# zju3dv/RelightableAvatar

Hardware: AMD Instinct MI355X
Metric: rays_per_sec (higher is better)
Workload: dtype f16

## Files before the change

### include/relightableavatar.h

```cpp
#ifndef RELIGHTABLEAVATAR_H
#define RELIGHTABLEAVATAR_H

#include <stddef.h>
#include <stdint.h>

#ifdef __cplusplus
extern "C" {
#endif

#define RA_ABI_VERSION 9
#define RA_N_LIGHTS_MAX 512

typedef struct ra_ctx ra_ctx;

const char* ra_last_error(void);
int ra_abi_version(void);

int ra_ctx_create(ra_ctx** out, int device);
int ra_ctx_destroy(ra_ctx* ctx);

typedef struct ra_config {
    int   xyz_res, sdf_res, view_res;
    int   n_bones;
    int   relight;
    float resd_limit;
    float blend_radius;
    float albedo_slope, albedo_bias;
    float roughness_slope, roughness_bias;
    float fresnel_f0;
    float shading_albedo;
    float albedo_multiplier;
    int   lambert_only, glossy_only;
    int   tonemapping;
    float bg_brightness;
    int   mlp_f16;
    int   query_skip;
    int   k4_batch_slots;
    int   trace_precision;
    float clip_near, clip_far;
    int   only_visibility;
    int   vis_shade_map;
    int   use_geodesic_filter;
    float key_light_share;
} ra_config;
int ra_default_config(ra_config* out);
int ra_set_config(ra_ctx* ctx, const ra_config* cfg);

int ra_set_weight(ra_ctx* ctx, const char* name, const float* host_data, size_t numel);
int ra_finalize_weights(ra_ctx* ctx, void* stream);
int ra_k3cc_enabled(const ra_ctx* ctx);

typedef struct ra_frame {
    const float* R;
    const float* Th;
    const float* poses;
    const float* cond_fix;
    const float* A;
    const float* big_A;
    const float* pverts;
    const float* pnorm;
    const float* tverts;
    const float* weights;
    int n_verts;
} ra_frame;
int ra_set_frame(ra_ctx* ctx, const ra_frame* frame, void* stream);

int ra_hdq_sdf(ra_ctx* ctx, const float* x_dev, int n, float dist_th, int smooth_transition,
               float* sdf_dev, void* stream);

int ra_observed_sdf(ra_ctx* ctx, const float* bpts_dev, int n, float* sdf_dev, void* stream);

int ra_bigpose_transform(ra_ctx* ctx, const float* x_dev, int n, const float* R_dev, const float* Th_dev, int invert,
                         float* out_dev, void* stream);

int ra_raw_channels(const ra_ctx* ctx);
int ra_forward(ra_ctx* ctx, const float* x_dev, const float* v_dev, int n, float dist_th,
               float* raw_dev, void* stream);

typedef struct ra_trace_params {
    int   iters;
    float tan_i;
    float tan_i_multiplier;
    float relax, offset, eps;
    int   shadow_skip_iter;
    int   clay_book;
    int   soft_shadow;
    float dist_th;
} ra_trace_params;
int ra_sphere_trace(ra_ctx* ctx, const float* ray_o, const float* ray_d, const float* near_,
                    const float* far_, const float* tan_i_dev, int n, const ra_trace_params* p,
                    float* surf, float* occ, float* st, float* ot, void* stream);

typedef struct ra_render_out {
    float* rgb;
    float* acc;
    float* depth;
    float* surf;
    float* norm;
    float* albedo;
    float* roughness;
    float* shade;
    float* spec;
    float* cpts;
    float* bpts;
    float* resd;
    float* ray_o;
    float* lvis;
    float* ldot;
    float* raw;
    float* volume_albedo;
    float* volume_roughness;
} ra_render_out;

typedef struct ra_sphere_params {
    ra_trace_params surface;
    ra_trace_params shadow;
    float shadow_near_offset;
    float dist_th;
    float surf_sample_range;
    int   n_samples;
    int   relighting;
    int   no_visibility, local_visibility;
    int   premultiply;
    int   n_boxes;
    const float* boxes;
    const int*   box_start;
} ra_sphere_params;

int ra_render_sphere_chunk(ra_ctx* ctx, const float* ray_o, const float* ray_d, const float* near_,
                           const float* far_, int P, const float* bbox_host6,
                           const float* probe_dev, int probe_h, int probe_w,
                           const ra_sphere_params* p, const ra_render_out* out, void* stream);

int ra_gather_rays(int device, const long long* idx_dev, int n, const float* ray_o, const float* ray_d, const float* near_, const float* far_,
                   float* out_o, float* out_d, float* out_near, float* out_far, void* stream);

int ra_scatter_rows(int device, const float* src_dev, const long long* src_idx_dev, const long long* dst_idx_dev, long long n, int C,
                    float* dst_dev, void* stream);

int ra_begin_render(ra_ctx* ctx);

int ra_set_key_probes(ra_ctx* ctx, const float* probes_dev, int n, int probe_h, int probe_w, int accumulate, void* stream);

int ra_set_light_xyz(ra_ctx* ctx, const float* xyz_dev, void* stream);

int ra_light_visibility(ra_ctx* ctx, const float* surf, const float* norm, const float* acc, int n, const int* rows_dev, int n_rows,
                        const float* bbox_host6, const float* probe_dev, int probe_h, int probe_w, const ra_sphere_params* params,
                        float* lvis, float* ldot, void* stream);

int ra_render_volume_chunk(ra_ctx* ctx, const float* ray_o, const float* ray_d, const float* near_,
                           const float* far_, int P, int n_samples, float dist_th,
                           const ra_render_out* out, void* stream);

int ra_reshade(ra_ctx* ctx, const float* ray_o, const float* surf, const float* norm,
               const float* albedo, const float* roughness, const float* lvis, const float* ldot,
               int P, const float* probes_dev, int n_probes, int probe_h, int probe_w,
               float* rgb, float* shade, float* spec, void* stream);

int ra_reshade_backward(ra_ctx* ctx, const float* ray_o, const float* surf, const float* norm,
                        const float* albedo, const float* roughness, const float* lvis, const float* ldot, int P,
                        const float* probes_dev, int n_probes, int probe_h, int probe_w,
                        const float* d_rgb, float* d_albedo, float* d_roughness, float* d_probes, void* stream);

size_t ra_heads_param_count(const ra_ctx* ctx);
int ra_heads_get_params(ra_ctx* ctx, float* theta_dev, void* stream);
int ra_heads_forward(ra_ctx* ctx, const float* theta_dev, const float* feat_dev, int n, float* albedo_dev, float* rough_dev, void* stream);
int ra_heads_backward(ra_ctx* ctx, const float* theta_dev, const float* feat_dev, int n,
                      const float* d_albedo_dev, const float* d_rough_dev, float* d_theta_dev, void* stream);
int ra_bigpose_features(ra_ctx* ctx, const float* bpts_dev, int n, float* feat_dev, void* stream);

int ra_canonical_features(ra_ctx* ctx, const float* cpts_dev, int n, float* feat_dev, void* stream);
int ra_gaussian_entropy(ra_ctx* ctx, const float* x_dev, int n, const float* d_value_dev, float* value_dev, float* d_x_dev, void* stream);

int ra_reshade_ground(ra_ctx* ctx, const float* ray_d, const float* albedo_map, const float* lvis, const float* ldot, int P,
                      const float* probes_dev, int n_probes, int probe_h, int probe_w, const float* images_dev, int image_h, int image_w,
                      int attach_envmap, float* rgb, float* albedo, float* shade, float* spec, void* stream);

typedef struct ra_counters {
    uint64_t n_coarse;
    uint64_t n_fine_sdf;
    uint64_t n_fine_full;
    uint64_t n_shadow_rays;
    uint64_t n_hit_pixels;
    uint64_t n_shaded;
    uint64_t n_fine_sdf_wide;
    uint64_t n_fine_sdf_comp;
} ra_counters;
int ra_get_counters(ra_ctx* ctx, ra_counters* out, void* stream);
int ra_reset_counters(ra_ctx* ctx, void* stream);

int ra_get_mlp_time(ra_ctx* ctx, float* ms, int* n_launches, void* stream);
int ra_get_kernel_time(ra_ctx* ctx, int kind, float* ms, int* n_launches, void* stream);
int ra_enable_timing(ra_ctx* ctx, int on);
typedef struct ra_gate ra_gate;
int ra_gate_create(ra_gate** out, int device);
int ra_gate_destroy(ra_gate* gate);
// ... 196 lines not shown
```

### relightableavatar_amd/_lib.py

```python
import ctypes as C
import os
import subprocess

_HERE = os.path.dirname(os.path.abspath(__file__))
LIB_PATH = os.environ.get('RA_LIB_PATH') or os.path.join(_HERE, 'librelightableavatar_hip.so')
_lib = None
ABI_VERSION = 9
RA_MESH_BRUTE, RA_MESH_UNSORTED = 1, 2
RA_WINDING_ONE_PASS, RA_WINDING_SPLIT = 1, 2
RA_RAYCAST_BRUTE, RA_RAYCAST_UNSORTED = 1, 2
RA_TOPO_ARRAYS = ('vert', 'twin', 'edge', 'edges', 'edge_counts', 'edge_he_start', 'edge_he', 'nbr_start', 'nbr', 'out_start', 'out_he')
RA_CLOTH_STRETCH, RA_CLOTH_BENDING, RA_CLOTH_GRAVITY = 1, 2, 4
CLOTH_MATERIAL_DEFAULTS = (('density', 426 * 0.00047), ('thickness', 0.00047), ('young_modulus', 0.7e5), ('poisson_ratio', 0.485),
                           ('bending_multiplier', 50.0), ('stretch_multiplier', 1.0), ('material_multiplier', 1.0))
RA_VOLUME_MODES = {'canonical': 0, 'tpose': 1, 'posed': 2}


class RaError(RuntimeError):
    pass


class ra_config(C.Structure):
    _fields_ = [('xyz_res', C.c_int), ('sdf_res', C.c_int), ('view_res', C.c_int), ('n_bones', C.c_int), ('relight', C.c_int),
                ('resd_limit', C.c_float), ('blend_radius', C.c_float), ('albedo_slope', C.c_float), ('albedo_bias', C.c_float),
                ('roughness_slope', C.c_float), ('roughness_bias', C.c_float), ('fresnel_f0', C.c_float),
                ('shading_albedo', C.c_float), ('albedo_multiplier', C.c_float), ('lambert_only', C.c_int),
                ('glossy_only', C.c_int), ('tonemapping', C.c_int), ('bg_brightness', C.c_float), ('mlp_f16', C.c_int), ('query_skip', C.c_int),
                ('k4_batch_slots', C.c_int), ('trace_precision', C.c_int), ('clip_near', C.c_float), ('clip_far', C.c_float),
                ('only_visibility', C.c_int), ('vis_shade_map', C.c_int), ('use_geodesic_filter', C.c_int), ('key_light_share', C.c_float)]


class ra_frame(C.Structure):
    _fields_ = [(k, C.c_void_p) for k in ('R', 'Th', 'poses', 'cond_fix', 'A', 'big_A', 'pverts', 'pnorm', 'tverts', 'weights')] + \
               [('n_verts', C.c_int)]


class ra_trace_params(C.Structure):
    _fields_ = [('iters', C.c_int), ('tan_i', C.c_float), ('tan_i_multiplier', C.c_float), ('relax', C.c_float),
                ('offset', C.c_float), ('eps', C.c_float), ('shadow_skip_iter', C.c_int), ('clay_book', C.c_int),
                ('soft_shadow', C.c_int), ('dist_th', C.c_float)]


RENDER_OUT_KEYS = ('rgb', 'acc', 'depth', 'surf', 'norm', 'albedo', 'roughness', 'shade', 'spec', 'cpts', 'bpts', 'resd',
                   'ray_o', 'lvis', 'ldot', 'raw', 'volume_albedo', 'volume_roughness')


class ra_render_out(C.Structure):
    _fields_ = [(k, C.c_void_p) for k in RENDER_OUT_KEYS]


class ra_sphere_params(C.Structure):
    _fields_ = [('surface', ra_trace_params), ('shadow', ra_trace_params), ('shadow_near_offset', C.c_float),
                ('dist_th', C.c_float), ('surf_sample_range', C.c_float), ('n_samples', C.c_int), ('relighting', C.c_int),
                ('no_visibility', C.c_int), ('local_visibility', C.c_int), ('premultiply', C.c_int),
                ('n_boxes', C.c_int), ('boxes', C.POINTER(C.c_float)), ('box_start', C.POINTER(C.c_int))]


class ra_ground_params(C.Structure):
    _fields_ = [('normal', C.c_float * 3), ('origin', C.c_float * 3), ('albedo', C.c_float * 3), ('attach_envmap', C.c_int),
                ('env_r', C.c_float), ('shading_multiplier', C.c_float), ('shadow', ra_trace_params), ('shadow_near_offset', C.c_float),
                ('no_visibility', C.c_int), ('local_visibility', C.c_int), ('n_boxes', C.c_int), ('boxes', C.POINTER(C.c_float)),
                ('box_start', C.POINTER(C.c_int))]


GROUND_OUT_KEYS = ('rgb', 'surf', 'albedo', 'shade', 'spec', 'depth', 'lvis', 'ldot')


class ra_ground_out(C.Structure):
    _fields_ = [(k, C.c_void_p) for k in GROUND_OUT_KEYS]


class ra_pose_in(C.Structure):
    _fields_ = [(k, C.POINTER(C.c_float)) for k in ('poses', 'tjoints', 'big_A', 'Rh', 'Th')] + \
               [('parents', C.POINTER(C.c_int)), ('faces', C.POINTER(C.c_int)), ('n_bones', C.c_int), ('n_faces', C.c_int), ('n_verts', C.c_int),
                ('tverts', C.c_void_p), ('weights', C.c_void_p), ('bounds_padding', C.c_float)]


POSE_OUT_KEYS = ('A', 'joints', 'tpose', 'pverts', 'wverts', 'pnorm', 'R', 'pbounds', 'wbounds', 'poses', 'Th')


class ra_pose_out(C.Structure):
    _fields_ = [(k, C.c_void_p) for k in POSE_OUT_KEYS]


class ra_image_params(C.Structure):
    _fields_ = [('type', C.c_int), ('H', C.c_int), ('W', C.c_int), ('bg_brightness', C.c_float), ('normalize', C.c_int), ('tonemap', C.c_int),
                ('min_clip', C.c_float), ('cam_R', C.c_float * 9), ('tbounds', C.c_float * 6)]


class ra_metrics_params(C.Structure):
    _fields_ = [('H', C.c_int), ('W', C.c_int), ('bg_brightness', C.c_float), ('data_range', C.c_float), ('mse_over_rays', C.c_int),
                ('crop_to_mask', C.c_int)]


class ra_lpips_weights(C.Structure):
    _fields_ = [('conv_w', C.c_void_p * 5), ('conv_b', C.c_void_p * 5), ('lin', C.c_void_p * 5), ('shift', C.c_float * 3), ('scale', C.c_float * 3)]


class ra_cloth_material(C.Structure):
    _fields_ = [(k, C.c_double) for k, _ in CLOTH_MATERIAL_DEFAULTS]


class ra_counters(C.Structure):
    _fields_ = [(k, C.c_uint64) for k in ('n_coarse', 'n_fine_sdf', 'n_fine_full', 'n_shadow_rays', 'n_hit_pixels', 'n_shaded', 'n_fine_sdf_wide', 'n_fine_sdf_comp')]


SYMBOLS = {
    'ra_last_error': (C.c_char_p, []),
    'ra_abi_version': (C.c_int, []),
    'ra_default_config': (C.c_int, [C.POINTER(ra_config)]),
    'ra_shard_plan': (C.c_int, [C.c_void_p, C.c_int, C.c_int, C.c_int, C.c_int, C.c_longlong] + [C.c_void_p] * 2 + [C.c_int] + [C.c_void_p] * 7),
    'ra_ctx_create': (C.c_int, [C.POINTER(C.c_void_p), C.c_int]),
    'ra_ctx_destroy': (C.c_int, [C.c_void_p]),
    'ra_set_config': (C.c_int, [C.c_void_p, C.POINTER(ra_config)]),
    'ra_set_weight': (C.c_int, [C.c_void_p, C.c_char_p, C.c_void_p, C.c_size_t]),
    'ra_finalize_weights': (C.c_int, [C.c_void_p, C.c_void_p]),
    'ra_set_frame': (C.c_int, [C.c_void_p, C.POINTER(ra_frame), C.c_void_p]),
    'ra_hdq_sdf': (C.c_int, [C.c_void_p, C.c_void_p, C.c_int, C.c_float, C.c_int, C.c_void_p, C.c_void_p]),
    'ra_observed_sdf': (C.c_int, [C.c_void_p, C.c_void_p, C.c_int, C.c_void_p, C.c_void_p]),
    'ra_bigpose_transform': (C.c_int, [C.c_void_p, C.c_void_p, C.c_int, C.c_void_p, C.c_void_p, C.c_int, C.c_void_p, C.c_void_p]),
    'ra_raw_channels': (C.c_int, [C.c_void_p]),
    'ra_forward': (C.c_int, [C.c_void_p, C.c_void_p, C.c_void_p, C.c_int, C.c_float, C.c_void_p, C.c_void_p]),
    'ra_sphere_trace': (C.c_int, [C.c_void_p] + [C.c_void_p] * 5 + [C.c_int, C.POINTER(ra_trace_params)] + [C.c_void_p] * 5),
    'ra_render_sphere_chunk': (C.c_int, [C.c_void_p] + [C.c_void_p] * 4 + [C.c_int, C.POINTER(C.c_float), C.c_void_p, C.c_int, C.c_int,
                                         C.POINTER(ra_sphere_params), C.POINTER(ra_render_out), C.c_void_p]),
    'ra_render_volume_chunk': (C.c_int, [C.c_void_p] + [C.c_void_p] * 4 + [C.c_int, C.c_int, C.c_float, C.POINTER(ra_render_out), C.c_void_p]),
    'ra_render_ground_chunk': (C.c_int, [C.c_void_p] + [C.c_void_p] * 3 + [C.c_int, C.POINTER(C.c_float), C.c_void_p, C.c_int, C.c_int,
                                         C.POINTER(ra_ground_params), C.POINTER(ra_ground_out), C.c_void_p]),
    'ra_blend_ground': (C.c_int, [C.c_void_p] + [C.c_void_p] * 4 + [C.c_int, C.c_int, C.c_int, C.c_void_p, C.c_void_p]),
    'ra_reshade': (C.c_int, [C.c_void_p] + [C.c_void_p] * 7 + [C.c_int, C.c_void_p, C.c_int, C.c_int, C.c_int] + [C.c_void_p] * 4),
    'ra_reshade_backward': (C.c_int, [C.c_void_p] + [C.c_void_p] * 7 + [C.c_int, C.c_void_p, C.c_int, C.c_int, C.c_int] + [C.c_void_p] * 5),
    'ra_heads_get_params': (C.c_int, [C.c_void_p, C.c_void_p, C.c_void_p]),
    'ra_heads_forward': (C.c_int, [C.c_void_p, C.c_void_p, C.c_void_p, C.c_int, C.c_void_p, C.c_void_p, C.c_void_p]),
    'ra_heads_backward': (C.c_int, [C.c_void_p, C.c_void_p, C.c_void_p, C.c_int, C.c_void_p, C.c_void_p, C.c_void_p, C.c_void_p]),
    'ra_bigpose_features': (C.c_int, [C.c_void_p, C.c_void_p, C.c_int, C.c_void_p, C.c_void_p]),
    'ra_canonical_features': (C.c_int, [C.c_void_p, C.c_void_p, C.c_int, C.c_void_p, C.c_void_p]),
    'ra_gaussian_entropy': (C.c_int, [C.c_void_p, C.c_void_p, C.c_int, C.c_void_p, C.c_void_p, C.c_void_p, C.c_void_p]),
    'ra_k3cc_enabled': (C.c_int, [C.c_void_p]),
    'ra_begin_render': (C.c_int, [C.c_void_p]),
    'ra_debug_key_lights': (C.c_int, [C.c_void_p, C.c_void_p, C.c_void_p, C.c_void_p]),
    'ra_scatter_rows': (C.c_int, [C.c_int, C.c_void_p, C.c_void_p, C.c_void_p, C.c_longlong, C.c_int, C.c_void_p, C.c_void_p]),
    'ra_gather_rays': (C.c_int, [C.c_int, C.c_void_p, C.c_int] + [C.c_void_p] * 9),
    'ra_set_key_probes': (C.c_int, [C.c_void_p, C.c_void_p, C.c_int, C.c_int, C.c_int, C.c_int, C.c_void_p]),
    'ra_set_light_xyz': (C.c_int, [C.c_void_p, C.c_void_p, C.c_void_p]),
    'ra_light_visibility': (C.c_int, [C.c_void_p, C.c_void_p, C.c_void_p, C.c_void_p, C.c_int, C.c_void_p, C.c_int, C.POINTER(C.c_float), C.c_void_p,
                                      C.c_int, C.c_int, C.POINTER(ra_sphere_params), C.c_void_p, C.c_void_p, C.c_void_p]),
    'ra_reshade_ground': (C.c_int, [C.c_void_p] + [C.c_void_p] * 4 + [C.c_int, C.c_void_p, C.c_int, C.c_int, C.c_int, C.c_void_p, C.c_int, C.c_int, C.c_int] +
                          [C.c_void_p] * 5),
    'ra_get_counters': (C.c_int, [C.c_void_p, C.POINTER(ra_counters), C.c_void_p]),
    'ra_reset_counters': (C.c_int, [C.c_void_p, C.c_void_p]),
    'ra_get_mlp_time': (C.c_int, [C.c_void_p, C.POINTER(C.c_float), C.POINTER(C.c_int), C.c_void_p]),
    'ra_get_kernel_time': (C.c_int, [C.c_void_p, C.c_int, C.POINTER(C.c_float), C.POINTER(C.c_int), C.c_void_p]),
    'ra_enable_timing': (C.c_int, [C.c_void_p, C.c_int]),
    'ra_set_knn_mode': (C.c_int, [C.c_void_p, C.c_int]),
    'ra_gate_create': (C.c_int, [C.POINTER(C.c_void_p), C.c_int]),
    'ra_gate_destroy': (C.c_int, [C.c_void_p]),
    'ra_set_gate': (C.c_int, [C.c_void_p, C.c_void_p]),
    'ra_pose_frame': (C.c_int, [C.c_void_p, C.POINTER(ra_pose_in), C.POINTER(ra_pose_out), C.c_void_p]),
    'ra_grow_bounds': (C.c_int, [C.c_void_p, C.c_void_p, C.c_float, C.c_void_p]),
    'ra_shift_envmap': (C.c_int, [C.c_void_p, C.c_void_p, C.c_int, C.c_int, C.c_int, C.c_float, C.c_void_p, C.c_void_p]),
    'ra_add_light_probe': (C.c_int, [C.c_void_p, C.c_void_p, C.c_int, C.c_int, C.c_void_p, C.c_int, C.c_int, C.POINTER(C.c_float), C.c_int, C.c_int, C.c_void_p]),
    'ra_map_to_image': (C.c_int, [C.c_void_p, C.POINTER(ra_image_params)] + [C.c_void_p] * 4 + [C.c_int, C.c_void_p, C.c_void_p, C.c_void_p]),
    'ra_image_metrics': (C.c_int, [C.c_void_p, C.POINTER(ra_metrics_params), C.c_void_p, C.c_void_p, C.c_void_p, C.c_int, C.c_void_p, C.c_void_p,
                                   C.c_void_p]),
    'ra_lpips_load': (C.c_int, [C.c_void_p, C.POINTER(ra_lpips_weights), C.c_void_p]),
    'ra_lpips_loaded': (C.c_int, [C.c_void_p]),
    'ra_lpips': (C.c_int, [C.c_void_p, C.POINTER(ra_metrics_params), C.c_void_p, C.c_void_p, C.c_void_p, C.c_int, C.c_void_p, C.c_void_p, C.c_void_p]),
    'ra_lpips_features': (C.c_int, [C.c_void_p, C.c_void_p, C.c_int, C.c_int, C.c_int, C.c_void_p, C.c_void_p]),
    'ra_lpips_tile_m': (C.c_int, []),
    'ra_mesh_create': (C.c_int, [C.c_void_p, C.c_void_p, C.c_int, C.c_void_p, C.c_int, C.POINTER(C.c_void_p), C.c_void_p]),
    'ra_mesh_destroy': (C.c_int, [C.c_void_p, C.c_void_p]),
    'ra_mesh_closest': (C.c_int, [C.c_void_p, C.c_void_p, C.c_void_p, C.c_int, C.c_int] + [C.c_void_p] * 5),
    'ra_mesh_tile': (C.c_int, [C.c_int]),
    'ra_mesh_winding': (C.c_int, [C.c_void_p, C.c_void_p, C.c_void_p, C.c_int, C.c_int, C.c_void_p, C.c_void_p]),
    'ra_winding_tile': (C.c_int, [C.c_int]),
    'ra_mesh_winding_grad': (C.c_int, [C.c_void_p, C.c_void_p, C.c_void_p, C.c_int, C.c_int, C.c_void_p, C.c_void_p, C.c_void_p]),
    'ra_mesh_raycast': (C.c_int, [C.c_void_p, C.c_void_p, C.c_void_p, C.c_void_p, C.c_int, C.c_int] + [C.c_void_p] * 5),
    'ra_raycast_tile': (C.c_int, [C.c_int]),
    'ra_topo_create': (C.c_int, [C.c_void_p, C.c_void_p, C.c_int, C.c_int, C.POINTER(C.c_void_p), C.c_void_p]),
    'ra_topo_destroy': (C.c_int, [C.c_void_p, C.c_void_p]),
    'ra_topo_sizes': (C.c_int, [C.c_void_p, C.c_void_p, C.POINTER(C.c_int)]),
    'ra_topo_array': (C.c_int, [C.c_void_p, C.c_void_p, C.c_int, C.c_void_p, C.c_void_p]),
# ... 80 lines not shown
```

### relightableavatar_amd/config.py

```python
from .base_utils import dotdict

_ACTIVE = None


def set_active_cfg(cfg):
    global _ACTIVE
    _ACTIVE = cfg


def active_cfg():
    global _ACTIVE
    if _ACTIVE is None:
        _ACTIVE = default_cfg()
    return _ACTIVE


UNSUPPORTED = {
    'bruteforce_st': (False, 'render_bruteforce_human (sphere_tracing_renderer.py:787-940) needs lib/networks/relight/nerfactor_network.py, '
                             'which the reference release does not contain'),
    'smpl_distance': (False, 'the SMPL mesh distance (base_network.py:417-427) needs the bvh_distance_queries CUDA extension'),
    'ablate_hdq_mode': ('hdq', "the world / can / curve tracing modes (sphere_tracing_renderer.py:141-151) call world_to_bigpose_transform, "
                               "which raises on the dataset's Th of shape (B, 1, 3); the operators exist: ra_observed_sdf, ra_bigpose_transform"),
    'check_bound_sdf': (False, 'debug colour map of |sdf| at termination (sphere_tracing_renderer.py:577-587, needs easyvolcap)'),
    'geometry_normal': (False, 'part of render_bruteforce_human'),
    'geometry_visibility': (False, 'part of render_bruteforce_human'),
    'zero_roughness': (False, 'part of render_bruteforce_human'),
    'mesh_simp_face': (-1, 'quadric decimation of the extracted mesh (mesh_renderer.py:95-96) needs open3d / trimesh'),
    'track_tpose_mesh': (False, 'mesh tracking (lib/networks/renderer/mesh_tracker.py) is not mirrored'),
}


def check_supported(cfg):
    for k, (default, why) in UNSUPPORTED.items():
        if k in cfg and cfg[k] != default:
            raise NotImplementedError(f'cfg.{k} = {cfg[k]!r} is not supported: {why}')


def default_cfg() -> dotdict:
    c = dotdict()
    c.network_module = 'relightableavatar_amd.networks.deform.base_network'
    c.renderer_module = 'relightableavatar_amd.renderer.base_renderer'
    c.n_bones = 52
    c.cond_dim = 156
    c.xyz_res = 10
    c.sdf_res = 8
    c.view_res = 4
    c.feat_dim = 256
    c.resd_limit = 0.05
    c.sdf_beta_init_value = 0.1
    c.blend_radius = 0.075
    c.sample_vert_cnt = 3
    c.use_geodesic_filter = True
    c.lambertian = False
    c.dist_th = 0.1
    c.n_samples = 128
    c.perturb = 1.0
    c.clip_near = 0.02
    c.clip_far = 10.0
    c.bg_brightness = 0.0
    c.render_chunk_size = 8192
    c.volume_chunk_rays = 65536
    c.sphere_chunk_rays = 262144
    c.ground_chunk_rays = 262144
    c.network_chunk_size = 262144
    c.fix_material = 0
    c.always_fix_material = True
    c.sphere_tracing = dotdict(iter=16, tan_i=1000.0, relax=0.0, offset=0.02, eps=1e-8,
                               near_offset=0.01, shadow_skip_iter=1, tan_i_multiplier=1.0)
    c.obj_lvis = dotdict(iter=4, offset=0.01, relax=0.0, near_offset=0.02, dist_th=0.05)
    c.env_lvis = dotdict(iter=16, offset=0.01, relax=0.0, near_offset=0.02, bbox_margin=0.25, dist_th=0.005)
    c.no_claybook = False
    c.no_dfss = False
    c.no_visibility = False
    c.local_visibility = False
    c.surf_sample_range = 0.005
    c.relighting = False
    c.achro_light = False
    c.envmap_upscale = 2
    c.envmap_init_intensity = 0.2
    c.env_h = 16
    c.env_w = 32
    c.env_r = 10.0
    c.fresnel_f0 = 0.02
    c.lambert_only = False
    c.glossy_only = False
    c.albedo_slope = 1.0
    c.albedo_bias = 0.0
    c.roughness_slope = 0.90
    c.roughness_bias = 0.09
    c.relight_network_width = 128
    c.relight_network_depth = 2
    c.albedo_multiplier = 1.0
    c.shading_albedo = 0.8
    c.tonemapping_rendering = True
    c.only_visibility = False
    c.rgb_as_albedo = False
    c.img_loss_weight = 1.0
    c.albedo_sparsity = 5e-4
    c.albedo_smooth_weight = 5e-3
    c.roughness_smooth_weight = 5e-3
    c.xyz_noise_std = 0.02
    c.light_xyz_noise_std = 1.0
    c.vis_rendering_map = True
    c.vis_shading_map = False
    c.vis_specular_map = False
    c.vis_novel_light = False
    c.vis_ground_shading = False
    c.voxel_size = [0.005, 0.005, 0.005]
    c.mesh_th = 0.5
    c.mesh_th_to_sdf = False
    c.mesh_simp_face = -1
    c.surface_blend_weight = False
    c.vis_tpose_mesh = False
    c.vis_posed_mesh = False
    c.vis_can_mesh = False
    c.track_tpose_mesh = False
    c.ground_normal = [0.0, 0.0, 1.0]
    c.ground_origin = [0.0, 0.0, 0.0]
    c.ground_albedo = [0.05, 0.05, 0.05]
    c.ground_attach_envmap = True
    c.ground_shading_multiplier = 1.0
    c.vis_lvis_map = False
    c.vis_ldot_map = False
    c.replace_light = ''
    c.test_light = ['main']
    c.vis_rotate_light = False
    c.rotate_ratio = 4
    c.probe_size_ratio = 0.2
    c.env_image_w = 2048
    c.normalize_shading = False
    c.normalize_specular = True
    c.min_clip = 1.0
    c.vis_median_depth = False
    c.store_alpha_channel = True
    c.tonemapping_albedo = True
    c.mlp_dtype = 'f16'
    c.ret_raw = True
    c.novel_light_timing = True
    c.query_skip = True
    c.trace_precision = 1
    c.key_light_share = 0.0078
    c.k4_batch_slots = 0
    return c


def make_cfg(mode: str = 'anisdf', **overrides) -> dotdict:
    c = default_cfg()
    if mode in ('sphere_tracing', 'relight', 'novel_light'):
        c.n_samples = 3
        c.render_chunk_size = 65536
        c.network_chunk_size = 1048576
        c.renderer_module = 'relightableavatar_amd.renderer.sphere_tracing_renderer'
    if mode in ('relight', 'novel_light'):
        c.relighting = True
        c.dist_th = 0.125
        c.obj_lvis.dist_th = 0.125
        c.achro_light = True
        c.network_module = 'relightableavatar_amd.networks.relight.relight_network'
    if mode == 'novel_light':
        c.vis_novel_light = True
        c.renderer_module = 'relightableavatar_amd.renderer.novel_light_sphere_tracing'
    elif mode not in ('anisdf', 'sphere_tracing', 'relight'):
        raise ValueError(f'unknown mode {mode}')
    for k, v in overrides.items():
        if isinstance(v, dict) and isinstance(c.get(k), dict):
            c[k].update(v)
        else:
            c[k] = v
    return c
```

### relightableavatar_amd/csrc/ra_api.cpp

```cpp
#include "ra_api_impl.hpp"
#include <cmath>

int check_ready(ra_ctx* c, const char* who) {
    if (!c) { ra_set_error(std::string(who) + ": null ctx"); return 1; }
    if (!c->have_weights) { ra_set_error(std::string(who) + ": weights not finalized"); return 1; }
    if (!c->have_frame) { ra_set_error(std::string(who) + ": no frame set (ra_set_frame)"); return 1; }
    if (hipSetDevice(c->device) != hipSuccess) { ra_set_error(std::string(who) + ": hipSetDevice failed"); return 1; }
    return 0;
}

static void zero_chunk_counters(ra_ctx* c, hipStream_t s) {
    hipMemsetAsync(icnt(c, 0), 0, CNT_ALL * sizeof(int), s);
    c->fc_next = 0;
    c->fc_wrapped = false;
    c->cnt_zero = true;
}
int* next_fine_counter(ra_ctx* c, hipStream_t s) {
    if (c->fc_next >= CNT_FC_SLOTS) {
        hipMemsetAsync(icnt(c, CNT_FC0), 0, CNT_FC_SLOTS * sizeof(int), s);
        c->fc_next = 0;
        c->fc_wrapped = true;
    }
    return icnt(c, CNT_FC0 + c->fc_next++);
}

namespace {

struct Timer {
    ra_ctx* c; hipStream_t s; TimerKind kind; hipEvent_t a = nullptr, b = nullptr;
    Timer(ra_ctx* c_, hipStream_t s_, TimerKind kind_) : c(c_), s(s_), kind(kind_) {
        if (!c->timing) return;
        if (c->ev_used == c->ev_pool.size()) {
            hipEvent_t x, y;
            hipEventCreate(&x); hipEventCreate(&y);
            c->ev_pool.push_back({x, y});
            c->ev_kind.push_back(kind);
        }
        c->ev_kind[c->ev_used] = kind;
        a = c->ev_pool[c->ev_used].first; b = c->ev_pool[c->ev_used].second;
        c->ev_used++;
        hipEventRecord(a, s);
    }
    ~Timer() { if (a) hipEventRecord(b, s); }
};

struct HintScope {
    ra_ctx* c; hipStream_t s;
    HintScope(ra_ctx* c_, hipStream_t s_) : c(c_), s(s_) {
        const int k = c->call_no++;
        if (k >= 64) { c->cur_hint = nullptr; return; }
        if ((int)c->hints.size() <= k) c->hints.resize(k + 1);
        HintSlot& h = c->hints[k];
        if (!h.ev) {
            if (hipEventCreateWithFlags(&h.ev, hipEventDisableTiming) != hipSuccess || hipHostMalloc((void**)&h.host, CNT_FC_SLOTS * sizeof(int)) != hipSuccess) {
                h.ev = nullptr; h.host = nullptr; c->cur_hint = nullptr; (void)hipGetLastError(); return;
            }
        }
        if (h.pending && hipEventQuery(h.ev) == hipSuccess) {
            h.vals.assign(h.host, h.host + h.n_pending);
            h.n_valid = h.n_pending;
            h.pending = false;
        }
        (void)hipGetLastError();
        c->cur_hint = &h;
    }
    ~HintScope() {
        HintSlot* h = c->cur_hint;
        c->cur_hint = nullptr;
        if (!h || h->pending || c->fc_next <= 0 || c->fc_wrapped) return;
        if (hipMemcpyAsync(h->host, icnt(c, CNT_FC0), (size_t)c->fc_next * sizeof(int), hipMemcpyDeviceToHost, s) != hipSuccess) return;
        if (hipEventRecord(h->ev, s) != hipSuccess) return;
        h->n_pending = c->fc_next;
        h->pending = true;
    }
};

int fine_hint(const ra_ctx* c, int k) {
    const HintSlot* h = c->cur_hint;
    return (h && !c->fc_wrapped && k < h->n_valid) ? h->vals[k] : -1;
}
int variant_size(int n, int hint) {
    if (hint < 0) return n;
    const long long v = (long long)hint + hint / 4 + 1024;
    return v < n ? (int)v : n;
}
int grid_size(int n, int nv) { return nv > n / 8 ? nv : n / 8; }

void k3_launch(ra_ctx* c, const MlpIO& io, int n, hipStream_t s, int grid_slots = 0) {
    if (c->cfg.mlp_f16) launch_mlp_sdf_stream_f16(c->host.geo, c->sarena.p, c->sarena_pairs.p, c->barena.as<float>(), c->fr, io, n, s, grid_slots);
    else launch_mlp_sdf_stream_bf16(c->host.geo, c->sarena.p, c->sarena_pairs.p, c->barena.as<float>(), c->fr, io, n, s, grid_slots);
}

}

void k4_fwd_launch(ra_ctx* c, const FullIO& io, char* tape, hipStream_t s) {
    if (c->cfg.mlp_f16) launch_mlp_fwd_tape_f16(c->host.geo, c->fwd_arena.p, c->barena.as<float>(), c->fr, io, tape, s);
    else launch_mlp_fwd_tape_bf16(c->host.geo, c->fwd_arena.p, c->barena.as<float>(), c->fr, io, tape, s);
}

FullIO full_io(ra_ctx* c) {
    FullIO io{};
    io.C = raw_channels(c);
    io.beta = c->host.beta; io.resd_limit = c->cfg.resd_limit;
    io.albedo_slope = c->cfg.albedo_slope; io.albedo_bias = c->cfg.albedo_bias;
    io.rough_slope = c->cfg.roughness_slope; io.rough_bias = c->cfg.roughness_bias;
    io.relight = c->cfg.relight;
    io.counters = dcnt(c);
    return io;
}

enum { Q_OTHER = 0, Q_SURFACE = 1, Q_PRECISE = 2 };
static bool precise(const ra_ctx* c, int what) { return what == Q_PRECISE || c->cfg.trace_precision >= 2 || (c->cfg.trace_precision == 1 && what == Q_SURFACE); }
static constexpr int KEY_LIGHTS_MAX = 48;
static bool key_tier(const ra_ctx* c) { return c->cfg.trace_precision == 1 && c->cfg.key_light_share > 0.f && c->n_lights > 0; }
static int key_mask_from(ra_ctx* c, const float* probe, int ph, int pw, hipStream_t s) {
    if (c->key_external) return 0;
    c->key_valid = false;
    if (!key_tier(c) || !probe) return 0;
    if (c->key_mask.ensure((size_t)c->n_lights) || c->key_share.ensure((size_t)c->n_lights * sizeof(float))) return 1;
    launch_key_lights(probe, 1, ph, pw, c->light_dir.as<float>(), c->light_area.as<float>(), c->n_lights, c->cfg.key_light_share, KEY_LIGHTS_MAX, 0,
                      c->key_share.as<float>(), c->key_mask.as<unsigned char>(), s);
    c->key_valid = true;
    return 0;
}

static void fine_level(ra_ctx* c, const MlpIO& io, int n, bool comp, hipStream_t s, int hint = -1) {
    const int nv = variant_size(n, hint);
    if (comp) {
        Timer t(c, s, T_K3C);
        launch_mlp_sdf_comp(c->host.geo, c->sarena_c.p, c->barena.as<float>(), c->fr, io, nv, s, c->k3cc_ok, grid_size(n, nv));
    } else {
        Timer t(c, s, k3_waves(nv) == 8 ? T_K3_WIDE : T_K3_NARROW);
        k3_launch(c, io, nv, s, grid_size(n, nv));
    }
}

static int hdq_pass(ra_ctx* c, const RaySet& rs, int n, float th, int smooth, float* sdf, hipStream_t s, int what = Q_OTHER,
                    const unsigned char* key = nullptr, int n_key = 0) {
    if (n <= 0) return 0;
    int err = 0;
    int* fine_idx = c->buf<int>("fine_idx", n, &err);
    float* bpts = c->buf<float>("fine_bpts", (size_t)n * 3, &err);
    if (err) return 1;
    HdqOut out{};
    out.sdf = sdf; out.fine_count = next_fine_counter(c, s); out.fine_idx = fine_idx; out.bpts = bpts;
    const int hint = fine_hint(c, c->fc_next - 1);
    int hint2 = -1;
    if (key && n_key > 0) {
        out.key = key;
        out.fine_idx2 = c->buf<int>("fine_idx_k", n_key, &err);
        out.bpts2 = c->buf<float>("fine_bpts_k", (size_t)n_key * 3, &err);
        if (err) return 1;
        out.fine_count2 = next_fine_counter(c, s);
        hint2 = fine_hint(c, c->fc_next - 1);
    }
    out.counters = dcnt(c);
    launch_hdq_coarse(c->fr, rs, n, th, c->cfg.blend_radius, out, s, c->cfg.use_geodesic_filter != 0);
    MlpIO io{};
    io.bpts = bpts; io.idx = fine_idx; io.count = out.fine_count; io.sdf = sdf; io.dist_th = th; io.smooth = smooth;
    io.resd_limit = c->cfg.resd_limit; io.counters = dcnt(c);
    fine_level(c, io, n, precise(c, what), s, hint);
    if (out.key) {
        io.bpts = out.bpts2; io.idx = out.fine_idx2; io.count = out.fine_count2;
        fine_level(c, io, n_key, true, s, hint2);
    }
    return 0;
}

int full_query(ra_ctx* c, FullIO io, int n, hipStream_t s) {
    const bool gated = c->gate && n > 65536;
    if (gated && c->gate->armed) RA_HIP(hipStreamWaitEvent(s, c->gate->done, 0));
    struct Release {
        ra_ctx* c; hipStream_t s; bool on;
        ~Release() { if (on) { hipEventRecord(c->gate->done, s); c->gate->armed = true; } }
    } release{c, s, gated};
    Timer t(c, s, T_K4);
    const int batch = c->cfg.k4_batch_slots > 0 ? c->cfg.k4_batch_slots : (1 << 20);
    const int cap = n < batch ? n : batch;
    int err = 0;
    char* tape = c->buf<char>("k4_tape", mlp_full_rev_tape_bytes(cap), &err);
    if (err) {
        ra_set_error("full query: no device memory for the activation tape (" + std::to_string(mlp_full_rev_tape_bytes(cap) >> 20) +
                     " MB): lower cfg.k4_batch_slots / cfg.volume_chunk_rays");
        return 1;
    }
    for (int s0 = 0; s0 < n; s0 += cap) {
        io.slot0 = s0;
        io.slot_cap = n - s0 < cap ? n - s0 : cap;
        k4_fwd_launch(c, io, tape, s);
        if (c->cfg.mlp_f16) launch_mlp_bwd_heads_f16(c->host.mat, c->host.col, c->bwd_arena.p, c->barena.as<float>(), c->shead_row.as<float>(), c->fr, io, tape, s);
        else launch_mlp_bwd_heads_bf16(c->host.mat, c->host.col, c->bwd_arena.p, c->barena.as<float>(), c->shead_row.as<float>(), c->fr, io, tape, s);
    }
    return 0;
}

static int forward_pass(ra_ctx* c, const float* x, const float* v, int n, const int* n_dev, float th, float* raw, hipStream_t s) {
    if (n <= 0) return 0;
    int err = 0;
    const int C = raw_channels(c);
    int* fine_idx = c->buf<int>("fine_idx", n, &err);
    float* bpts = c->buf<float>("fine_bpts", (size_t)n * 3, &err);
    float* mats = c->buf<float>("fine_mats", (size_t)n * 24, &err);
    float* sdf = c->buf<float>("fwd_sdf", n, &err);
    if (err) return 1;
    RaySet rs{};
    rs.mode = 0; rs.x = x; rs.n_dev = n_dev;
    HdqOut out{};
    out.sdf = sdf; out.fine_count = next_fine_counter(c, s); out.fine_idx = fine_idx; out.bpts = bpts; out.mats = mats;
    out.raw_zero = raw; out.raw_C = C;
    out.counters = dcnt(c);
    launch_hdq_coarse(c->fr, rs, n, th, c->cfg.blend_radius, out, s, c->cfg.use_geodesic_filter != 0);
    FullIO io = full_io(c);
    io.bpts = bpts; io.mats = mats; io.view = v; io.idx = fine_idx; io.count = out.fine_count; io.raw = raw;
    return full_query(c, io, n, s);
}

static TraceState alloc_trace(ra_ctx* c, const std::string& p, int n, bool soft, int* err) {
    TraceState ts{};
    ts.t = c->buf<float>(p + "t", n, err);
    ts.d0 = c->buf<float>(p + "d0", n, err);
    ts.occ = c->buf<float>(p + "occ", n, err);
    ts.ot = c->buf<float>(p + "ot", n, err);
    ts.stuck = c->buf<unsigned char>(p + "stuck", n, err);
    if (!soft) {
        ts.dt = c->buf<float>(p + "dt", n, err);
        ts.st = c->buf<float>(p + "st", n, err);
        ts.cd = c->buf<float>(p + "cd", n, err);
        ts.off = c->buf<float>(p + "off", n, err);
        ts.rlx = c->buf<float>(p + "rlx", n, err);
    }
    return ts;
}

int sdf_points_precise(ra_ctx* c, int mode, const float* pts, int n, float dist_th, float* sdf, hipStream_t s) {
    if (n <= 0) return 0;
    if (mode == 2) {
        RaySet rs{};
        rs.mode = 0; rs.x = pts;
        return hdq_pass(c, rs, n, dist_th, 0, sdf, s, Q_PRECISE);
    }
    int err = 0;
    int* idx = c->buf<int>("fine_idx", n, &err);
    if (err) return 1;
    int* cnt = next_fine_counter(c, s);
    launch_iota(idx, n, cnt, s);
    MlpIO io{};
    io.bpts = pts; io.idx = idx; io.count = cnt; io.sdf = sdf; io.dist_th = 1.f; io.smooth = 0;
    io.resd_limit = mode == 0 ? 0.f : c->cfg.resd_limit; io.counters = dcnt(c);
    fine_level(c, io, n, true, s);
    return 0;
}

extern "C" {

int ra_raw_channels(const ra_ctx* c) { return c ? raw_channels(c) : 16; }

int ra_hdq_sdf(ra_ctx* c, const float* x, int n, float dist_th, int smooth, float* sdf, void* stream) {
    if (check_ready(c, "ra_hdq_sdf")) return 1;
    RA_CHECK(n >= 0 && (n == 0 || (x && sdf)), "ra_hdq_sdf: bad arguments");
    RaySet rs{};
    rs.mode = 0; rs.x = x;
    if (hdq_pass(c, rs, n, dist_th, smooth, sdf, (hipStream_t)stream)) return 1;
    RA_HIP(hipGetLastError());
    return 0;
}

int ra_observed_sdf(ra_ctx* c, const float* bpts, int n, float* sdf, void* stream) {
    if (check_ready(c, "ra_observed_sdf")) return 1;
    RA_CHECK(n >= 0 && (n == 0 || (bpts && sdf)), "ra_observed_sdf: bad arguments");
    if (n == 0) return 0;
    hipStream_t s = (hipStream_t)stream;
    int err = 0;
    int* idx = c->buf<int>("fine_idx", n, &err);
    if (err) return 1;
    int* cnt = next_fine_counter(c, s);
    launch_iota(idx, n, cnt, s);
    MlpIO io{};
    io.bpts = bpts; io.idx = idx; io.count = cnt; io.sdf = sdf; io.dist_th = 1.f; io.smooth = 0;
    io.resd_limit = c->cfg.resd_limit; io.counters = dcnt(c);
    fine_level(c, io, n, precise(c, Q_OTHER), s);
    RA_HIP(hipGetLastError());
    return 0;
}

int ra_bigpose_transform(ra_ctx* c, const float* x, int n, const float* R, const float* Th, int invert, float* out, void* stream) {
    if (check_ready(c, "ra_bigpose_transform")) return 1;
    RA_CHECK(n >= 0 && (n == 0 || (x && out && R && Th)), "ra_bigpose_transform: bad arguments");
    if (n == 0) return 0;
    hipStream_t s = (hipStream_t)stream;
    int err = 0;
    int* fine_idx = c->buf<int>("fine_idx", n, &err);
    float* fb = c->buf<float>("fine_bpts", (size_t)n * 3, &err);
    float* sdfc = c->buf<float>("bt_sdf", n, &err);
    float* sb = c->buf<float>("bt_sdf_batch", (size_t)n * 3, &err);
    int* nb = c->buf<int>("bt_nn", (size_t)n * 3, &err);
    float* d2 = c->buf<float>("bt_d2", (size_t)n * 3, &err);
    float* bp = c->buf<float>("bt_bpts", (size_t)n * 3, &err);
    float* tp = c->buf<float>("bt_tpts", (size_t)n * 3, &err);
    float* mats = c->buf<float>("bt_mats", (size_t)n * 24, &err);
    if (err) return 1;
    RaySet rs{};
    rs.mode = 0; rs.x = x;
    HdqOut o{};
    o.sdf = sdfc; o.fine_count = next_fine_counter(c, s); o.fine_idx = fine_idx; o.bpts = fb;
    o.dbg_sdf_batch = sb; o.dbg_nn_batch = nb; o.dbg_d2 = d2; o.dbg_bpts = bp; o.dbg_tpts = tp; o.dbg_mats = mats;
    o.counters = dcnt(c);
    launch_hdq_coarse(c->fr, rs, n, 1e9f, c->cfg.blend_radius, o, s, c->cfg.use_geodesic_filter != 0);
    launch_bigpose_compose(mats, d2, n, c->cfg.blend_radius, R, Th, invert, out, s);
    RA_HIP(hipGetLastError());
    return 0;
}

int ra_forward(ra_ctx* c, const float* x, const float* v, int n, float dist_th, float* raw, void* stream) {
    if (check_ready(c, "ra_forward")) return 1;
    RA_CHECK(n >= 0 && (n == 0 || (x && raw)), "ra_forward: bad arguments");
    RA_CHECK(c->cfg.relight || v || n == 0, "ra_forward: the AniSDF colour net needs view directions");
    if (forward_pass(c, x, v, n, nullptr, dist_th, raw, (hipStream_t)stream)) return 1;
    RA_HIP(hipGetLastError());
    return 0;
}

int ra_sphere_trace(ra_ctx* c, const float* ray_o, const float* ray_d, const float* near_, const float* far_, const float* tan_i,
                    int n, const ra_trace_params* p, float* surf, float* occ, float* st, float* ot, void* stream) {
    if (check_ready(c, "ra_sphere_trace")) return 1;
    RA_CHECK(p && n >= 0 && (n == 0 || (ray_o && ray_d && near_ && far_)), "ra_sphere_trace: bad arguments");
    if (n == 0) return 0;
    hipStream_t s = (hipStream_t)stream;
    int err = 0;
    TraceState ts = alloc_trace(c, "tr_", n, false, &err);
    float* sdf = c->buf<float>("tr_sdf", n, &err);
    if (err) return 1;
    ts.near_ = near_; ts.far_ = far_; ts.tan_i = tan_i; ts.light = nullptr;
    launch_trace_init(ts, n, nullptr, *p, s);
    RaySet rs{};
    rs.mode = 1; rs.o = ray_o; rs.d = ray_d; rs.t = ts.t;
    rs.nn_hint = c->buf<int>("tr_nn", (size_t)n * 3, &err);
    if (err) return 1;
    for (int it = 0; it < p->iters; ++it) {
        rs.hint_valid = it > 0;
        if (hdq_pass(c, rs, n, p->dist_th, 1, sdf, s, p->soft_shadow ? Q_OTHER : Q_SURFACE)) return 1;
        launch_trace_update(ts, sdf, n, nullptr, it, *p, s);
    }
    if (occ) RA_HIP(hipMemcpyAsync(occ, ts.occ, (size_t)n * 4, hipMemcpyDeviceToDevice, s));
    if (st) RA_HIP(hipMemcpyAsync(st, ts.st, (size_t)n * 4, hipMemcpyDeviceToDevice, s));
    if (ot) RA_HIP(hipMemcpyAsync(ot, ts.ot, (size_t)n * 4, hipMemcpyDeviceToDevice, s));
    if (surf) {
        float* depth = c->buf<float>("tr_depth", n, &err);
        float* acc = c->buf<float>("tr_acc", n, &err);
        int* hidx = c->buf<int>("tr_hidx", n, &err);
        if (err) return 1;
        launch_surface_finish(ray_o, ray_d, ts.st, ts.occ, n, surf, depth, acc, hidx, icnt(c, CNT_HIT), s);
    }
    RA_HIP(hipGetLastError());
    return 0;
}

struct LvisStage {
    const float *surf, *norm_slots, *acc, *bbox;
    const int *hit_idx, *hit_count;
    int P, no_visibility, local_visibility;
    float near_offset;
    const ra_trace_params* shadow;
    int n_boxes;
    const float* boxes;
    const int *box_start, *pix_nn, *perm;
    bool split_wide_groups;
    float *lvis, *ldot;
};
static int light_visibility_stage(ra_ctx* c, LvisStage& st, hipStream_t s) {
    const int P = st.P;
    const ra_trace_params& shadow = *st.shadow;
    int err = 0;
    const int L = c->n_lights;
    const size_t NR = (size_t)P * L;
    st.lvis = c->buf<float>("lv_lvis", NR, &err);
    st.ldot = c->buf<float>("lv_ldot", NR, &err);
    ShadowGen g{};
    g.surf = st.surf; g.norm = st.norm_slots; g.acc = st.acc; g.hit_idx = st.hit_idx; g.hit_count = st.hit_count; g.ldir = c->light_dir.as<float>();
    for (int k = 0; k < 6; ++k) g.bbox[k] = st.bbox[k];
    g.n_boxes = st.n_boxes > 1 ? st.n_boxes : 0;
    for (int j = 0; j < g.n_boxes; ++j) {
        for (int k = 0; k < 6; ++k) g.boxes[j][k] = st.boxes[6 * j + k];
        g.box_start[j] = st.box_start[j];
    }
    if (g.n_boxes) g.box_start[g.n_boxes] = st.box_start[g.n_boxes];
    g.perm = g.n_boxes ? st.perm : nullptr;
    g.near_offset = st.near_offset; g.L = L; g.no_visibility = st.no_visibility; g.local_visibility = st.local_visibility;
    g.split_wide_groups = st.split_wide_groups ? 1 : 0;
    g.lvis = st.lvis; g.ldot = st.ldot;
    g.ray_count = icnt(c, CNT_RAYS);
    const bool traced = !(st.no_visibility || st.local_visibility);
    TraceState sh{};
    float* ssdf = nullptr;
    if (traced) {
        g.ray_pix = c->buf<int>("lv_pix", NR, &err);
        g.ray_light = c->buf<int>("lv_light", NR, &err);
        g.ray_slot = c->buf<int>("lv_slot", NR, &err);
        g.near_ = c->buf<float>("lv_near", NR, &err);
        g.far_ = c->buf<float>("lv_far", NR, &err);
        sh = alloc_trace(c, "sh_", (int)NR, shadow.soft_shadow != 0, &err);
        ssdf = c->buf<float>("sh_sdf", NR, &err);
    }
    const bool keyed = traced && key_tier(c) && c->key_valid;
    const size_t NK = keyed ? (size_t)P * (size_t)(L < KEY_LIGHTS_MAX ? L : KEY_LIGHTS_MAX) : 0;
    if (err) return 1;
    if (c->gate && c->gate->armed) RA_HIP(hipStreamWaitEvent(s, c->gate->done, 0));
    launch_shadow_gen(g, P, s, c->cnt_zero);
    c->cnt_zero = false;
    if (traced) {
        sh.near_ = g.near_; sh.far_ = g.far_; sh.tan_i = c->light_sharp.as<float>(); sh.light = g.ray_light;
        launch_trace_init(sh, (int)NR, g.ray_count, shadow, s);
        RaySet r2{};
        r2.mode = 2; r2.o = st.surf; r2.t = sh.t; r2.pix = g.ray_pix; r2.light = g.ray_light; r2.ldir = c->light_dir.as<float>();
        r2.n_dev = g.ray_count;
        r2.skip = c->cfg.query_skip ? sh.stuck : nullptr;
        r2.nn_hint = c->buf<int>("lv_nn", NR * 3, &err);
        if (err) return 1;
        for (int it = 0; it < shadow.iters; ++it) {
            r2.hint_valid = it > 0;
            r2.hint_src = it == 0 ? st.pix_nn : nullptr;
            r2.hint_src_index = it == 0 ? g.ray_pix : nullptr;
            if (hdq_pass(c, r2, (int)NR, shadow.dist_th, 1, ssdf, s, Q_OTHER, keyed ? c->key_mask.as<unsigned char>() : nullptr, (int)NK)) return 1;
            launch_trace_update(sh, ssdf, (int)NR, g.ray_count, it, shadow, s);
        }
        launch_shadow_scatter(sh.occ, g.ray_slot, g.ray_count, (int)NR, st.lvis, s);
        launch_accumulate(g.ray_count, &dcnt(c)->n_shadow_rays, s);
    }
    if (c->gate) { RA_HIP(hipEventRecord(c->gate->done, s)); c->gate->armed = true; }
    return 0;
}

int ra_begin_render(ra_ctx* c) {
    RA_CHECK(c, "ra_begin_render: null ctx");
    c->call_no = 0;
    return 0;
}

int ra_set_key_probes(ra_ctx* c, const float* probes, int n, int ph, int pw, int accumulate, void* stream) {
    RA_CHECK(c && n >= 0 && (n == 0 || (probes && ph > 0 && pw > 0)), "ra_set_key_probes: bad arguments");
    if (n == 0) { c->key_external = false; c->key_valid = false; return 0; }
    RA_CHECK(c->have_weights && c->n_lights > 0, "ra_set_key_probes: needs the relight network's light set (ra_finalize_weights)");
    RA_HIP(hipSetDevice(c->device));
    const bool acc = accumulate && c->key_external && c->key_valid;
    c->key_external = true;
    if (!key_tier(c)) { c->key_valid = false; return 0; }
    if (c->key_mask.ensure((size_t)c->n_lights) || c->key_share.ensure((size_t)c->n_lights * sizeof(float))) return 1;
    launch_key_lights(probes, n, ph, pw, c->light_dir.as<float>(), c->light_area.as<float>(), c->n_lights, c->cfg.key_light_share, KEY_LIGHTS_MAX,
                      acc ? 1 : 0, c->key_share.as<float>(), c->key_mask.as<unsigned char>(), (hipStream_t)stream);
    c->key_valid = true;
    RA_HIP(hipGetLastError());
    return 0;
}

static int sort_hits(ra_ctx* c, const char* who, const float* surf, const float* acc, int P, const float* bbox, int* hit_idx, hipStream_t s) {
    int err = 0;
    const size_t tb = sort_hits_temp_bytes(P);
    unsigned* k0 = c->buf<unsigned>("hs_k0", P, &err);
    unsigned* k1 = c->buf<unsigned>("hs_k1", P, &err);
    int* v0 = c->buf<int>("hs_v0", P, &err);
    char* tmp = c->buf<char>("hs_tmp", tb + 16, &err);
    if (err) return 1;
    if (launch_sort_hits(surf, acc, P, bbox, k0, k1, v0, hit_idx, tmp, tb, s)) { ra_set_error(std::string(who) + ": radix sort failed"); return 1; }
    return 0;
}
static int sort_rays(ra_ctx* c, const char* who, const float** ray_o, const float** ray_d, const float** near_, const float** far_, int P,
                     const float* bbox, const int** perm, hipStream_t s) {
    int err = 0;
    const size_t tb = sort_hits_temp_bytes(P);
    unsigned* k0 = c->buf<unsigned>("hs_k0", P, &err);
    unsigned* k1 = c->buf<unsigned>("hs_k1", P, &err);
    int* v0 = c->buf<int>("hs_v0", P, &err);
    int* pm = c->buf<int>("rs_perm", P, &err);
    char* tmp = c->buf<char>("hs_tmp", tb + 16, &err);
    float* so = c->buf<float>("rs_o", (size_t)P * 3, &err);
    float* sd = c->buf<float>("rs_d", (size_t)P * 3, &err);
    float* sn = c->buf<float>("rs_n", P, &err);
    float* sf = c->buf<float>("rs_f", P, &err);
    if (err) return 1;
    const int rc = bbox ? launch_sort_rays(*ray_o, *ray_d, *near_, *far_, P, bbox, k0, k1, v0, pm, tmp, tb, so, sd, sn, sf, s)
                        : launch_sort_rays(*ray_o, *ray_d, *near_, *far_, P, nullptr, k0, k1, v0, pm, tmp, tb, so, sd, sn, sf, s, c->cfg.clip_near, c->cfg.clip_far);
    if (rc) { ra_set_error(std::string(who) + ": radix sort failed"); return 1; }
    *ray_o = so; *ray_d = sd; *near_ = sn; *far_ = sf; *perm = pm;
    return 0;
}

static int check_box_table(const std::string& w, int n_boxes, const float* boxes, const int* box_start, const float* bbox, int P) {
    if (n_boxes <= 1) return 0;
    RA_CHECK(n_boxes <= RA_MAX_BOXES && boxes && box_start && bbox, w + ": at most 32 boxes per call, with their tables");
    RA_CHECK(box_start[0] == 0 && box_start[n_boxes] == P, w + ": box_start must run from 0 to P");
    for (int j = 0; j < n_boxes; ++j) RA_CHECK(box_start[j] <= box_start[j + 1], w + ": box_start must ascend");
    return 0;
}

int ra_render_sphere_chunk(ra_ctx* c, const float* ray_o, const float* ray_d, const float* near_, const float* far_, int P,
                           const float* bbox, const float* probe, int ph, int pw, const ra_sphere_params* p,
                           const ra_render_out* out, void* stream) {
    if (check_ready(c, "ra_render_sphere_chunk")) return 1;
    RA_CHECK(p && out && P >= 0, "ra_render_sphere_chunk: bad arguments");
    if (P == 0) return 0;
    RA_CHECK(ray_o && ray_d && near_ && far_, "ra_render_sphere_chunk: null ray arrays");
    const bool relit = p->relighting != 0;
    RA_CHECK(!relit || (c->cfg.relight && probe && bbox && c->n_lights > 0), "ra_render_sphere_chunk: relighting needs the relight network, a probe and a bbox");
    RA_CHECK(p->n_samples >= 1 && p->n_samples <= 16, "ra_render_sphere_chunk: n_samples out of range");
    RA_CHECK(!relit || (long long)P * c->n_lights < (1ll << 31), "ra_render_sphere_chunk: chunk too large (rays x lights must fit an int): lower cfg.render_chunk_size / cfg.sphere_chunk_rays");
    if (check_box_table("ra_render_sphere_chunk", p->n_boxes, p->boxes, p->box_start, bbox, P)) return 1;
    hipStream_t s = (hipStream_t)stream;
    int err = 0;
    const int S = p->n_samples, C = raw_channels(c), L = c->n_lights;
    zero_chunk_counters(c, s);
    HintScope hints(c, s);
    const int* perm = nullptr;
    if (bbox && sort_rays(c, "ra_render_sphere_chunk", &ray_o, &ray_d, &near_, &far_, P, bbox, &perm, s)) return 1;
    TraceState ts = alloc_trace(c, "sf_", P, false, &err);
    float* sdf = c->buf<float>("sf_sdf", P, &err);
    float* surf = c->buf<float>("sf_surf", (size_t)P * 3, &err);
    float* depth = c->buf<float>("sf_depth", P, &err);
    float* acc = c->buf<float>("sf_acc", P, &err);
    int* hit_idx = c->buf<int>("sf_hit", P, &err);
    int* slot_of_ray = c->buf<int>("sf_slot", P, &err);
    if (err) return 1;
    ts.near_ = near_; ts.far_ = far_;
    launch_trace_init(ts, P, nullptr, p->surface, s);
    RaySet rs{};
    rs.mode = 1; rs.o = ray_o; rs.d = ray_d; rs.t = ts.t; rs.skip = c->cfg.query_skip ? ts.stuck : nullptr;
    rs.nn_hint = c->buf<int>("sf_nn", (size_t)P * 3, &err);
    if (err) return 1;
    for (int it = 0; it < p->surface.iters; ++it) {
        rs.hint_valid = it > 0;
        if (hdq_pass(c, rs, P, p->surface.dist_th, 1, sdf, s, Q_SURFACE)) return 1;
        launch_trace_update(ts, sdf, P, nullptr, it, p->surface, s);
    }
    int* hit_count = icnt(c, CNT_HIT);
    launch_surface_finish(ray_o, ray_d, ts.st, ts.occ, P, surf, depth, acc, hit_idx, hit_count, s, slot_of_ray, true);
    launch_accumulate(hit_count, &dcnt(c)->n_hit_pixels, s);
    if (relit && sort_hits(c, "ra_render_sphere_chunk", surf, acc, P, bbox, hit_idx, s)) return 1;
    launch_slot_index(hit_idx, hit_count, P, slot_of_ray, s);
    float* xs = c->buf<float>("mt_x", (size_t)P * S * 3, &err);
    float* vs = c->buf<float>("mt_v", (size_t)P * S * 3, &err);
    float* raw = c->buf<float>("mt_raw", (size_t)P * S * C, &err);
    SurfaceMaps m{};
    m.cpts = c->buf<float>("mp_cpts", (size_t)P * 3, &err);
    m.bpts = c->buf<float>("mp_bpts", (size_t)P * 3, &err);
    m.resd = c->buf<float>("mp_resd", (size_t)P * 3, &err);
    m.norm = c->buf<float>("mp_norm", (size_t)P * 3, &err);
    m.albedo = c->buf<float>("mp_albedo", (size_t)P * 3, &err);
    m.rough = c->buf<float>("mp_rough", P, &err);
    m.rgb = c->buf<float>("mp_rgb", (size_t)P * 3, &err);
    m.valbedo = (out->volume_albedo && c->cfg.relight) ? c->buf<float>("mp_valbedo", (size_t)P * 3, &err) : nullptr;
    if (err) return 1;
    launch_surface_samples(surf, ray_d, hit_idx, hit_count, P, S, p->surf_sample_range, xs, vs, icnt(c, CNT_SAMP), s);
    if (forward_pass(c, xs, vs, P * S, icnt(c, CNT_SAMP), p->dist_th, raw, s)) return 1;
    launch_surface_composite(raw, C, S, hit_count, P, c->cfg.relight, c->cfg, m, s);
    float *shade = nullptr, *spec = nullptr;
    LvisStage st{};
    if (relit) {
        if (key_mask_from(c, probe, ph, pw, s)) return 1;
        st.surf = surf; st.norm_slots = m.norm; st.acc = acc; st.hit_idx = hit_idx; st.hit_count = hit_count; st.P = P; st.bbox = bbox;
        st.near_offset = p->shadow_near_offset; st.shadow = &p->shadow; st.no_visibility = p->no_visibility; st.local_visibility = p->local_visibility;
        st.n_boxes = p->n_boxes; st.boxes = p->boxes; st.box_start = p->box_start; st.pix_nn = rs.nn_hint; st.perm = perm; st.split_wide_groups = true;
        if (light_visibility_stage(c, st, s)) return 1;
        m.rgb = c->buf<float>("mp_rgb", (size_t)P * 3, &err);
        shade = c->buf<float>("mp_shade", (size_t)P * 3, &err);
        spec = c->buf<float>("mp_spec", (size_t)P * 3, &err);
        if (err) return 1;
        ShadeIn in{};
        in.ray_o = ray_o; in.surf = surf; in.idx = hit_idx; in.count = hit_count; in.n = P;
        in.norm = m.norm; in.albedo = m.albedo; in.rough = m.rough; in.lvis = st.lvis; in.ldot = st.ldot;
        in.light_xyz = c->light_xyz.as<float>(); in.light_area = c->light_area.as<float>(); in.L = L;
        in.probes = probe; in.n_probes = 1; in.ph = ph; in.pw = pw; in.want_spec = out->spec != nullptr;
        in.rgb = m.rgb; in.shade = shade; in.spec = spec;
        launch_shade(in, c->cfg, s);
    }
    const int pm = p->premultiply;
    EmitMaps em{};
    em.slot_of_ray = slot_of_ray; em.acc = acc; em.perm = perm; em.P = P;
    long long total = 0;
    auto scat = [&](float* dst, const float* src, int Cc, bool premul, bool src_full) {
        if (!dst) return;
        if (em.n_jobs == RA_MAX_MAP_JOBS) { launch_emit_maps(em, s); em.n_jobs = 0; total = 0; }
// ... 161 lines not shown
```

### relightableavatar_amd/csrc/ra_api_ctx.cpp

```cpp
#include "ra_api_impl.hpp"
#include <cstdio>
#include <memory>
#include <mutex>

static thread_local std::string g_err;
void ra_set_error(const std::string& msg) { g_err = msg; }

int DevBuf::ensure(size_t need) {
    if (need <= bytes && p) return 0;
    if (need == 0) need = 16;
    if (p) { hipDeviceSynchronize(); hipFree(p); p = nullptr; bytes = 0; }
    size_t want = need + need / 8 + 256;
    hipError_t e = hipMalloc(&p, want);
    if (e != hipSuccess) { ra_set_error(std::string("hipMalloc(") + std::to_string(want) + "): " + hipGetErrorString(e)); p = nullptr; return 1; }
    bytes = want;
    return 0;
}
void DevBuf::release() { if (p) hipFree(p); p = nullptr; bytes = 0; }

ra_ctx::~ra_ctx() {
    for (auto& e : ev_pool) { hipEventDestroy(e.first); hipEventDestroy(e.second); }
    for (int k = 0; k < PinRing::n; ++k) if (pin.ev[k]) hipEventDestroy(pin.ev[k]);
    for (HintSlot& h : hints) { if (h.ev) hipEventDestroy(h.ev); if (h.host) hipHostFree(h.host); }
    if (pin.base) hipHostFree(pin.base);
}

extern "C" {

const char* ra_last_error(void) { return g_err.c_str(); }
int ra_abi_version(void) { return RA_ABI_VERSION; }

int ra_ctx_create(ra_ctx** out, int device) {
    RA_CHECK(out, "ra_ctx_create: null out");
    int n = 0;
    RA_HIP(hipGetDeviceCount(&n));
    RA_CHECK(n > 0, "ra_ctx_create: no HIP device visible (the render path has no CPU fallback)");
    RA_CHECK(device >= 0 && device < n, "ra_ctx_create: bad device index");
    RA_HIP(hipSetDevice(device));
    std::unique_ptr<ra_ctx> c(new ra_ctx());
    c->device = device;
    if (c->dcounters.ensure(1024)) return 1;
    RA_HIP(hipMemset(c->dcounters.p, 0, 1024));
    *out = c.release();
    return 0;
}

int ra_gate_create(ra_gate** out, int device) {
    RA_CHECK(out, "ra_gate_create: null out");
    RA_HIP(hipSetDevice(device));
    std::unique_ptr<ra_gate> g(new ra_gate());
    g->device = device;
    if (hipEventCreateWithFlags(&g->done, hipEventDisableTiming) != hipSuccess) { g->done = nullptr; ra_set_error("ra_gate_create: hipEventCreate failed"); return 1; }
    *out = g.release();
    return 0;
}
int ra_gate_destroy(ra_gate* g) {
    if (!g) return 0;
    hipSetDevice(g->device);
    hipDeviceSynchronize();
    delete g;
    return 0;
}
int ra_set_gate(ra_ctx* c, ra_gate* g) {
    RA_CHECK(c, "ra_set_gate: null context");
    RA_CHECK(!g || g->device == c->device, "ra_set_gate: gate and context live on different devices");
    c->gate = g;
    return 0;
}

int ra_ctx_destroy(ra_ctx* c) {
    if (!c) return 0;
    hipSetDevice(c->device);
    hipDeviceSynchronize();
    delete c;
    return 0;
}

int ra_default_config(ra_config* o) {
    RA_CHECK(o, "ra_default_config: null argument");
    *o = ra_config{};
    o->xyz_res = 10; o->sdf_res = 8; o->view_res = 4; o->n_bones = 52; o->relight = 1;
    o->resd_limit = 0.05f; o->blend_radius = 0.075f;
    o->albedo_slope = 1.f; o->albedo_bias = 0.f; o->roughness_slope = 0.9f; o->roughness_bias = 0.09f;
    o->fresnel_f0 = 0.02f; o->shading_albedo = 0.8f; o->albedo_multiplier = 1.f;
    o->tonemapping = 1; o->bg_brightness = 0.f; o->mlp_f16 = 1; o->query_skip = 1; o->k4_batch_slots = 0;
    o->trace_precision = 1; o->clip_near = 0.02f; o->clip_far = 10.f;
    o->only_visibility = 0; o->vis_shade_map = 0; o->use_geodesic_filter = 1;
    o->key_light_share = 0.0078f;
    return 0;
}

int ra_set_config(ra_ctx* c, const ra_config* cfg) {
    RA_CHECK(c && cfg, "ra_set_config: null argument");
    RA_CHECK(cfg->n_bones > 0 && cfg->n_bones <= 256, "ra_set_config: bad n_bones");
    RA_CHECK(cfg->trace_precision >= 0 && cfg->trace_precision <= 2, "ra_set_config: trace_precision must be 0, 1 or 2 (a zero-initialised ra_config is not the default: ra_default_config)");
    RA_CHECK(cfg->clip_far > cfg->clip_near, "ra_set_config: clip_far must exceed clip_near (a zero-initialised ra_config is not the default: ra_default_config)");
    RA_CHECK(cfg->vis_shade_map >= 0 && cfg->vis_shade_map <= 2, "ra_set_config: vis_shade_map must be 0, 1 or 2");
    RA_CHECK(cfg->key_light_share >= 0.f && cfg->key_light_share <= 1.f, "ra_set_config: key_light_share must be a fraction in [0, 1] (0 = no key-light tier)");
    c->cfg = *cfg;
    c->have_cfg = true;
    return 0;
}

int ra_set_weight(ra_ctx* c, const char* name, const float* data, size_t numel) {
    RA_CHECK(c && name && (data || numel == 0), "ra_set_weight: null argument");
    c->state_dict[name] = std::vector<float>(data, data + numel);
    c->have_weights = false;
    return 0;
}

static int upload(DevBuf& b, const void* src, size_t bytes, hipStream_t s) {
    if (b.ensure(bytes)) return 1;
    if (bytes) RA_HIP(hipMemcpyAsync(b.p, src, bytes, hipMemcpyHostToDevice, s));
    return 0;
}

static std::mutex k3cc_mu;
static std::map<int, bool> k3cc_result;
static int k3cc_self_test(ra_ctx* c, hipStream_t s) {
    {
        std::lock_guard<std::mutex> lk(k3cc_mu);
        auto it = k3cc_result.find(c->device);
        if (it != k3cc_result.end()) { c->k3cc_ok = it->second; return 0; }
    }
    constexpr int N = 400;
    std::vector<float> x(3 * N);
    unsigned u = 12345u;
    for (float& v : x) { u = u * 1664525u + 1013904223u; v = ((u >> 8) * (1.f / 16777216.f) - 0.5f) * 0.9f; }
    std::vector<int> idx(N);
    for (int i = 0; i < N; ++i) idx[i] = i;
    DevBuf bx, bi, bc, ba, bb, bz;
    if (bx.ensure(x.size() * 4) || bi.ensure(N * 4) || bc.ensure(4) || ba.ensure(N * 4) || bb.ensure(N * 4) || bz.ensure(2048)) return 1;
    RA_HIP(hipMemcpyAsync(bx.p, x.data(), x.size() * 4, hipMemcpyHostToDevice, s));
    RA_HIP(hipMemcpyAsync(bi.p, idx.data(), N * 4, hipMemcpyHostToDevice, s));
    const int n = N;
    RA_HIP(hipMemcpyAsync(bc.p, &n, 4, hipMemcpyHostToDevice, s));
    RA_HIP(hipMemsetAsync(ba.p, 0xff, N * 4, s));
    RA_HIP(hipMemsetAsync(bb.p, 0, N * 4, s));
    RA_HIP(hipMemsetAsync(bz.p, 0, 2048, s));
    FrameState f{};
    f.bias_r0 = bz.as<float>(); f.bias_r4 = bz.as<float>() + 256;
    MlpIO io{};
    io.bpts = bx.as<float>(); io.idx = bi.as<int>(); io.count = bc.as<int>(); io.dist_th = 1.f; io.smooth = 0; io.resd_limit = c->cfg.resd_limit;
    io.sdf = ba.as<float>();
    launch_mlp_sdf_comp(c->host.geo, c->sarena_c.p, c->barena.as<float>(), f, io, N, s, true);
    io.sdf = bb.as<float>();
    launch_mlp_sdf_comp(c->host.geo, c->sarena_c.p, c->barena.as<float>(), f, io, N, s, false);
    std::vector<unsigned> a(N), b(N);
    RA_HIP(hipMemcpyAsync(a.data(), ba.p, N * 4, hipMemcpyDeviceToHost, s));
    RA_HIP(hipMemcpyAsync(b.data(), bb.p, N * 4, hipMemcpyDeviceToHost, s));
    RA_HIP(hipStreamSynchronize(s));
    RA_HIP(hipGetLastError());
    c->k3cc_ok = a == b;
    if (!c->k3cc_ok)
        fprintf(stderr, "relightableavatar: K3CC self-test failed (its distances differ from K3C's): the cooperative small-launch kernel is disabled on device %d (ra_k3cc_enabled)\n", c->device);
    std::lock_guard<std::mutex> lk(k3cc_mu);
    k3cc_result[c->device] = c->k3cc_ok;
    return 0;
}

int ra_k3cc_enabled(const ra_ctx* c) { return c && c->have_weights && c->k3cc_ok ? 1 : 0; }

int ra_finalize_weights(ra_ctx* c, void* stream) {
    RA_CHECK(c && c->have_cfg, "ra_finalize_weights: call ra_set_config first");
    hipStream_t s = (hipStream_t)stream;
    RA_HIP(hipSetDevice(c->device));
    std::string err;
    if (ra_pack_weights(c, err)) { ra_set_error("ra_finalize_weights: " + err); return 1; }
    HostNets& H = c->host;
    if (upload(c->sarena, H.sarena_trim.data(), H.sarena_trim.size() * 2, s)) return 1;
    if (upload(c->sarena_pairs, H.sarena_pairs.data(), H.sarena_pairs.size() * 2, s)) return 1;
    if (upload(c->sarena_c, H.sarena_c.data(), H.sarena_c.size() * 2, s)) return 1;
    if (upload(c->fwd_arena, H.fwd_arena.data(), H.fwd_arena.size() * 2, s)) return 1;
    if (upload(c->bwd_arena, H.bwd_arena.data(), H.bwd_arena.size() * 2, s)) return 1;
    if (upload(c->shead_row, H.shead_row.data(), H.shead_row.size() * 4, s)) return 1;
    if (upload(c->barena, H.barena.data(), H.barena.size() * 4, s)) return 1;
    if (upload(c->cond_r0, H.cond_r0.data(), H.cond_r0.size() * 4, s)) return 1;
    if (upload(c->cond_r4, H.cond_r4.data(), H.cond_r4.size() * 4, s)) return 1;
    if (upload(c->b_r0, H.b_r0.data(), H.b_r0.size() * 4, s)) return 1;
    if (upload(c->b_r4, H.b_r4.data(), H.b_r4.size() * 4, s)) return 1;
    if (H.has_color) {
        if (upload(c->cond_c3, H.cond_c3.data(), H.cond_c3.size() * 4, s)) return 1;
        if (upload(c->b_c3, H.b_c3.data(), H.b_c3.size() * 4, s)) return 1;
    }
    if (c->cfg.relight) {
        c->n_lights = (int)H.light_area.size();
        if (upload(c->light_xyz, H.light_xyz.data(), H.light_xyz.size() * 4, s)) return 1;
        if (upload(c->light_xyz_loaded, H.light_xyz.data(), H.light_xyz.size() * 4, s)) return 1;
        if (upload(c->light_area, H.light_area.data(), H.light_area.size() * 4, s)) return 1;
        if (upload(c->light_sharp, H.light_sharp.data(), H.light_sharp.size() * 4, s)) return 1;
        if (c->light_dir.ensure(H.light_xyz.size() * 4)) return 1;
        launch_light_dirs(c->light_xyz.as<float>(), c->n_lights, c->light_dir.as<float>(), s);
    }
    RA_HIP(hipStreamSynchronize(s));
    if (k3cc_self_test(c, s)) return 1;
    c->have_weights = true;
    return 0;
}

int ra_set_frame(ra_ctx* c, const ra_frame* f, void* stream) {
    RA_CHECK(c && f, "ra_set_frame: null argument");
    RA_CHECK(c->have_weights, "ra_set_frame: weights not finalized");
    RA_CHECK(f->R && f->Th && f->poses && f->A && f->big_A && f->pverts && f->pnorm && f->tverts && f->weights, "ra_set_frame: null frame array");
    RA_CHECK(f->n_verts >= 3, "ra_set_frame: need at least 3 vertices (K=3 neighbours)");
    hipStream_t s = (hipStream_t)stream;
    RA_HIP(hipSetDevice(c->device));
    const int nv = f->n_verts, nb = c->cfg.n_bones, cond = nb * 3;
    if (c->fvertA.ensure((size_t)nv * 24 * 4) || c->fpverts4.ensure((size_t)nv * 16) || c->fbias_r0.ensure(1024) || c->fbias_r4.ensure(1024) ||
        c->fbias_c3.ensure(1024))
        return 1;
    launch_pack_verts(f->pverts, nv, c->fpverts4.as<float4>(), s);
    launch_vert_blend(f->weights, f->A, f->big_A, nv, nb, c->fvertA.as<float>(), s);
    const int nleaf = c->use_bvh ? bvh_leaf_count(nv) : 0;
    const int nsuper = bvh_super_count(nleaf);
    if (nleaf > 0) {
        if (c->fbvh_pts.ensure((size_t)nleaf * 32 * 16) || c->fbvh_pairs.ensure((size_t)nsuper * (32 + 192)) || c->fbvh_order.ensure((size_t)nv * 4)) return 1;
        launch_bvh_build(c->fpverts4.as<float4>(), nv, c->fbvh_order.as<int>(), c->fbvh_pts.as<float>(), c->fbvh_pairs.as<float4>(), nleaf, nsuper, s);
        RA_HIP(hipGetLastError());
    }
    launch_fold_bias(c->cond_r0.as<float>(), cond, 0, cond, f->poses, c->b_r0.as<float>(), c->fbias_r0.as<float>(), s);
    launch_fold_bias(c->cond_r4.as<float>(), cond, 0, cond, f->poses, c->b_r4.as<float>(), c->fbias_r4.as<float>(), s);
    if (c->host.has_color && f->cond_fix)
        launch_fold_bias(c->cond_c3.as<float>(), cond, 0, cond, f->cond_fix, c->b_c3.as<float>(), c->fbias_c3.as<float>(), s);
    FrameState& fr = c->fr;
    fr.R = (float*)f->R; fr.Th = (float*)f->Th; fr.vertA = c->fvertA.as<float>(); fr.pverts4 = c->fpverts4.as<float4>();
    fr.pnorm = (float*)f->pnorm; fr.tverts = (float*)f->tverts; fr.bias_r0 = c->fbias_r0.as<float>();
    fr.bias_r4 = c->fbias_r4.as<float>(); fr.bias_c3 = c->fbias_c3.as<float>(); fr.n_verts = nv;
    fr.bvh_soa = c->fbvh_pts.as<float>();
    fr.bvh_sbox = c->fbvh_pairs.as<float4>(); fr.bvh_lpair = reinterpret_cast<const float*>(fr.bvh_sbox + (size_t)2 * nsuper); fr.bvh_leaves = nleaf; fr.bvh_supers = nsuper;
    c->have_frame = true;
    c->call_no = 0;
    RA_HIP(hipGetLastError());
    return 0;
}

int ra_get_counters(ra_ctx* c, ra_counters* out, void* stream) {
    RA_CHECK(c && out, "ra_get_counters: null argument");
    RA_HIP(hipSetDevice(c->device));
    RA_HIP(hipStreamSynchronize((hipStream_t)stream));
    unsigned long long h[8];
    RA_HIP(hipMemcpy(h, c->dcounters.p, sizeof(h), hipMemcpyDeviceToHost));
// ... 60 lines not shown
```

### relightableavatar_amd/csrc/ra_hdq.hip

```cpp
#include "ra_kernels.hpp"
#include <type_traits>
#include <cstdlib>

namespace {

constexpr int KNN_THREADS = 256;

#ifdef RA_COARSE_TS
__device__ long long ra_coarse_ts[64 * 64 * 16 * 8];
extern "C" int ra_coarse_read_timestamps(long long* out) { return (int)hipMemcpyFromSymbol(out, HIP_SYMBOL(ra_coarse_ts), sizeof(ra_coarse_ts)); }
#define RA_CSTAMP(k) do { if (tsp) { __builtin_amdgcn_sched_barrier(0); if ((threadIdx.x & 63) == 0) tsp[k] = __builtin_readcyclecounter(); __builtin_amdgcn_sched_barrier(0); } } while (0)
#else
#define RA_CSTAMP(k) do { } while (0)
#endif
constexpr int VT = 2048;

__device__ __forceinline__ void inv3d(const float R[9], float M[9]) {
    M[0] = R[4] * R[8] - R[7] * R[5];
    M[3] = -R[3] * R[8] + R[6] * R[5];
    M[6] = R[3] * R[7] - R[6] * R[4];
    M[1] = -R[1] * R[8] + R[7] * R[2];
    M[4] = R[0] * R[8] - R[6] * R[2];
    M[7] = -R[0] * R[7] + R[6] * R[1];
    M[2] = R[1] * R[5] - R[4] * R[2];
    M[5] = -R[0] * R[5] + R[3] * R[2];
    M[8] = R[0] * R[4] - R[3] * R[1];
    const float D = R[0] * M[0] + R[1] * M[3] + R[2] * M[6];
    const float inv = 1.f / (D + 1e-8f);
#pragma unroll
    for (int i = 0; i < 9; ++i) M[i] *= inv;
}

__device__ __forceinline__ float sgn(float x) { return (x > 0.f) ? 1.f : ((x < 0.f) ? -1.f : 0.f); }

__global__ void vert_blend_kernel(const float* __restrict__ weights, const float* __restrict__ A, const float* __restrict__ big_A,
                                  int n_verts, int n_bones, float* __restrict__ vertA) {
    const int v = blockIdx.x * blockDim.x + threadIdx.x;
    if (v >= n_verts) return;
    float acc[24];
#pragma unroll
    for (int e = 0; e < 24; ++e) acc[e] = 0.f;
    for (int j = 0; j < n_bones; ++j) {
        const float w = weights[(size_t)v * n_bones + j];
#pragma unroll
        for (int e = 0; e < 12; ++e) {
            acc[e] += w * A[j * 16 + e];
            acc[12 + e] += w * big_A[j * 16 + e];
        }
    }
#pragma unroll
    for (int e = 0; e < 24; ++e) vertA[(size_t)v * 24 + e] = acc[e];
}

__global__ void pack_verts_kernel(const float* __restrict__ pv, int n, float4* __restrict__ out) {
    const int v = blockIdx.x * blockDim.x + threadIdx.x;
    if (v < n) out[v] = make_float4(pv[3 * v], pv[3 * v + 1], pv[3 * v + 2], 0.f);
}

__global__ __launch_bounds__(256) void fold_bias_kernel(const float* __restrict__ W, int ld, int col0, int ncond, const float* __restrict__ cond,
                                                        const float* __restrict__ bias, float* __restrict__ out) {
    const int r = blockIdx.x * 4 + (threadIdx.x >> 6), lane = threadIdx.x & 63;
    if (r >= 256) return;
    const float* row = W + (size_t)r * ld + col0;
    float a = 0.f;
    for (int c = lane; c < ncond; c += 64) a = fmaf(row[c], cond[c], a);
#pragma unroll
    for (int o = 32; o > 0; o >>= 1) a += __shfl_xor(a, o);
    if (lane == 0) out[r] = bias[r] + a;
}

constexpr int BVH_THREADS = 1024;
constexpr int BVH_LEAF = 32;
constexpr int BVH_FAN = 8;
constexpr int BVH_MAXN = 16384;
constexpr int BVH_MAXL = BVH_MAXN / BVH_LEAF;
constexpr int BVH_MAXS = BVH_MAXL / BVH_FAN;

__device__ __forceinline__ unsigned expand10(unsigned v) {
    v = (v * 0x00010001u) & 0xFF0000FFu;
    v = (v * 0x00000101u) & 0x0F00F00Fu;
    v = (v * 0x00000011u) & 0xC30C30C3u;
    v = (v * 0x00000005u) & 0x49249249u;
    return v;
}

constexpr int RANK_WAVES = BVH_THREADS / 64;

__global__ __launch_bounds__(BVH_THREADS) void bvh_rank_kernel(const float4* __restrict__ pv, int n, int* __restrict__ order) {
    __shared__ unsigned long long keys[BVH_MAXN];
    __shared__ float red[6][BVH_THREADS / 64];
    __shared__ float bb[6];
    __shared__ int cnt[RANK_WAVES][64];
    const int tid = threadIdx.x;
    float mn[3] = {3e38f, 3e38f, 3e38f}, mx[3] = {-3e38f, -3e38f, -3e38f};
    for (int i = tid; i < n; i += BVH_THREADS) {
        const float4 v = pv[i];
        mn[0] = fminf(mn[0], v.x); mn[1] = fminf(mn[1], v.y); mn[2] = fminf(mn[2], v.z);
        mx[0] = fmaxf(mx[0], v.x); mx[1] = fmaxf(mx[1], v.y); mx[2] = fmaxf(mx[2], v.z);
    }
#pragma unroll
    for (int c = 0; c < 3; ++c)
#pragma unroll
        for (int o = 32; o > 0; o >>= 1) { mn[c] = fminf(mn[c], __shfl_xor(mn[c], o)); mx[c] = fmaxf(mx[c], __shfl_xor(mx[c], o)); }
    if ((tid & 63) == 0) for (int c = 0; c < 3; ++c) { red[c][tid >> 6] = mn[c]; red[3 + c][tid >> 6] = mx[c]; }
    __syncthreads();
    if (tid < 6) {
        float a = red[tid][0];
        for (int w = 1; w < BVH_THREADS / 64; ++w) a = tid < 3 ? fminf(a, red[tid][w]) : fmaxf(a, red[tid][w]);
        bb[tid] = a;
    }
    __syncthreads();
    const int n4 = (n + 3) & ~3;
    for (int i = tid; i < n4; i += BVH_THREADS) {
        unsigned long long k = ~0ull;
        if (i < n) {
            const float4 v = pv[i];
            const float p[3] = {v.x, v.y, v.z};
            unsigned q[3];
#pragma unroll
            for (int c = 0; c < 3; ++c) {
                const float e = fmaxf(bb[3 + c] - bb[c], 1e-12f);
                q[c] = (unsigned)fminf(fmaxf((p[c] - bb[c]) / e * 1023.f, 0.f), 1023.f);
            }
            const unsigned code = (expand10(q[0]) << 2) | (expand10(q[1]) << 1) | expand10(q[2]);
            k = ((unsigned long long)code << 32) | (unsigned)i;
        }
        keys[i] = k;
    }
    __syncthreads();
    const int lane = tid & 63, g = tid >> 6;
    const int e = blockIdx.x * 64 + lane;
    const unsigned long long mine = e < n ? keys[e] : 0ull;
    const int chunk = ((n4 / 4 + RANK_WAVES - 1) / RANK_WAVES) * 4;
    const int j0 = g * chunk, j1 = min(n4, j0 + chunk);
    int c = 0;
    for (int j = j0; j < j1; j += 4) {
        const ulonglong2 a = *reinterpret_cast<const ulonglong2*>(&keys[j]);
        const ulonglong2 b = *reinterpret_cast<const ulonglong2*>(&keys[j + 2]);
        c += (a.x < mine) + (a.y < mine) + (b.x < mine) + (b.y < mine);
    }
    cnt[g][lane] = c;
    __syncthreads();
    if (g == 0 && e < n) {
        int r = 0;
#pragma unroll
        for (int w = 0; w < RANK_WAVES; ++w) r += cnt[w][lane];
        order[r] = e;
    }
}

__global__ __launch_bounds__(BVH_THREADS) void bvh_boxes_kernel(const float4* __restrict__ pv, const int* __restrict__ order, int n,
                                                                float* __restrict__ leaves, float4* __restrict__ sbox, int nl, int ns) {
    __shared__ float lb[BVH_MAXL][6];
    const int tid = threadIdx.x, e = tid & 31;
    for (int l = tid >> 5; l < nl; l += BVH_THREADS / 32) {
        const int i = l * BVH_LEAF + e;
        float4 v = make_float4(__int_as_float(0x7f800000), __int_as_float(0x7f800000), __int_as_float(0x7f800000), __int_as_float(0x7fffffff));
        float lo[3] = {3e38f, 3e38f, 3e38f}, hi[3] = {-3e38f, -3e38f, -3e38f};
        if (i < n) {
            const int id = order[i];
            v = pv[id];
            v.w = __int_as_float(id);
            lo[0] = hi[0] = v.x; lo[1] = hi[1] = v.y; lo[2] = hi[2] = v.z;
        }
        float* soa = leaves + (size_t)l * (4 * BVH_LEAF) + e;
        soa[0] = v.x; soa[BVH_LEAF] = v.y; soa[2 * BVH_LEAF] = v.z; soa[3 * BVH_LEAF] = v.w;
#pragma unroll
        for (int c = 0; c < 3; ++c)
#pragma unroll
            for (int o = 16; o > 0; o >>= 1) { lo[c] = fminf(lo[c], __shfl_xor(lo[c], o)); hi[c] = fmaxf(hi[c], __shfl_xor(hi[c], o)); }
        if (e == 0) {
#pragma unroll
            for (int c = 0; c < 3; ++c) { lb[l][c] = lo[c]; lb[l][3 + c] = hi[c]; }
        }
    }
    __syncthreads();
    for (int sidx = tid; sidx < ns; sidx += BVH_THREADS) {
        float lo[3] = {3e38f, 3e38f, 3e38f}, hi[3] = {-3e38f, -3e38f, -3e38f};
        for (int k = 0; k < BVH_FAN; ++k) {
            const int l = sidx * BVH_FAN + k;
            if (l < nl)
#pragma unroll
                for (int c = 0; c < 3; ++c) { lo[c] = fminf(lo[c], lb[l][c]); hi[c] = fmaxf(hi[c], lb[l][3 + c]); }
        }
        sbox[2 * sidx] = make_float4(lo[0], lo[1], lo[2], 0.f);
        sbox[2 * sidx + 1] = make_float4(hi[0], hi[1], hi[2], 0.f);
        float* rec = reinterpret_cast<float*>(sbox + 2 * (size_t)ns) + (size_t)sidx * (6 * BVH_FAN);
        for (int k = 0; k < BVH_FAN; ++k) {
            const int l = sidx * BVH_FAN + k;
#pragma unroll
            for (int c = 0; c < 6; ++c) rec[12 * (k >> 1) + 2 * c + (k & 1)] = l < nl ? lb[l][c] : (c < 3 ? 3e38f : -3e38f);
        }
    }
}

template <int I, int N, typename F>
__device__ __forceinline__ void static_for(F&& f) {
    if constexpr (I < N) {
        f(std::integral_constant<int, I>{});
        static_for<I + 1, N>(f);
    }
}

template <int K>
__device__ __forceinline__ float row_bcast(float v) {
    return __int_as_float(__builtin_amdgcn_update_dpp(0, __float_as_int(v), 0x150 + K, 0xf, 0xf, false));
}

__device__ __forceinline__ float box_dist2(const float p[3], float lx, float ly, float lz, float hx, float hy, float hz) {
    const float dx = fmaxf(fmaxf(lx - p[0], p[0] - hx), 0.f);
    const float dy = fmaxf(fmaxf(ly - p[1], p[1] - hy), 0.f);
    const float dz = fmaxf(fmaxf(lz - p[2], p[2] - hz), 0.f);
    return dx * dx + dy * dy + dz * dz;
}

__device__ __forceinline__ float dist2(float dx, float dy, float dz) { return __fmaf_rn(dz, dz, __fmaf_rn(dx, dx, dy * dy)); }

__device__ __forceinline__ void knn_insert(float d, int id, float& d0, float& d1, float& d2, int& i0, int& i1, int& i2, bool dedup = false) {
    if (__builtin_expect(__ballot(d <= d2) == 0ull, 1)) return;
    bool fresh = true;
    if (dedup) fresh = (id != i0) & (id != i1) & (id != i2);
    const bool c2 = fresh && (d < d2 || (d == d2 && id < i2));
    const bool c1 = fresh && (d < d1 || (d == d1 && id < i1));
    const bool c0 = fresh && (d < d0 || (d == d0 && id < i0));
    const float nd2 = c1 ? d1 : (c2 ? d : d2);
    const int ni2 = c1 ? i1 : (c2 ? id : i2);
    const float nd1 = c0 ? d0 : (c1 ? d : d1);
    const int ni1 = c0 ? i0 : (c1 ? id : i1);
    d0 = c0 ? d : d0;
    i0 = c0 ? id : i0;
    d1 = nd1; i1 = ni1; d2 = nd2; i2 = ni2;
}

__device__ __forceinline__ void ray_point(const RaySet& rs, int i, float x[3]) {
    if (rs.mode == 0) {
        x[0] = rs.x[3 * i]; x[1] = rs.x[3 * i + 1]; x[2] = rs.x[3 * i + 2];
    } else if (rs.mode == 1) {
        const float t = rs.t[i];
        x[0] = rs.o[3 * i] + t * rs.d[3 * i];
        x[1] = rs.o[3 * i + 1] + t * rs.d[3 * i + 1];
        x[2] = rs.o[3 * i + 2] + t * rs.d[3 * i + 2];
    } else {
        const float t = rs.t[i];
        const int p = rs.pix[i], l = rs.light[i];
        x[0] = rs.o[3 * p] + t * rs.ldir[3 * l];
        x[1] = rs.o[3 * p + 1] + t * rs.ldir[3 * l + 1];
        x[2] = rs.o[3 * p + 2] + t * rs.ldir[3 * l + 2];
    }
}

template <bool BVH, int SPLIT, bool HINT = false>
__global__ __launch_bounds__(SPLIT == 1 ? KNN_THREADS : 64 * SPLIT) void hdq_coarse_kernel(FrameState fr, RaySet rs, int n_launch, float th, float inv2r2,
                                                                  HdqOut out, int dbg) {
    static_assert(SPLIT == 1 || (BVH && SPLIT >= 2 && SPLIT <= 16), "SPLIT > 1: the workgroup is SPLIT waves on the same 64 queries");
    constexpr int NT = SPLIT == 1 ? KNN_THREADS : 64 * SPLIT;
    __shared__ __attribute__((aligned(16))) unsigned char smem[BVH ? 16 : VT * 16];
#ifdef RA_COARSE_TS
    long long* tsp = blockIdx.x < 64 ? ra_coarse_ts + ((((dbg >> 8) & 63) * 64 + blockIdx.x) * 16 + (threadIdx.x >> 6)) * 8 : nullptr;
    dbg &= 255;
    if (tsp && (threadIdx.x & 63) == 0) { tsp[1] = tsp[2] = tsp[3] = tsp[4] = tsp[5] = tsp[6] = tsp[7] = 0; }
    RA_CSTAMP(0);
#endif
    const int n = rs.n_dev ? min(*rs.n_dev, n_launch) : n_launch;
    const int base = blockIdx.x * (SPLIT == 1 ? KNN_THREADS : 64);
    if (base >= n) return;
    if (blockIdx.x == 0 && threadIdx.x == 0 && out.counters) atomicAdd(&out.counters->n_coarse, (unsigned long long)n);
    const int i = base + (SPLIT == 1 ? threadIdx.x : (threadIdx.x & 63));
    const bool live_q = i < n && !(rs.skip && rs.skip[i < n ? i : 0]);
    bool live = live_q;
    if (__syncthreads_count(live_q) == 0) return;
    float x[3] = {0.f, 0.f, 0.f};
    if (live) ray_point(rs, i, x);
    const float xt[3] = {x[0] - fr.Th[0], x[1] - fr.Th[1], x[2] - fr.Th[2]};
    float p[3];
#pragma unroll
    for (int c = 0; c < 3; ++c) p[c] = xt[0] * fr.R[c] + xt[1] * fr.R[3 + c] + xt[2] * fr.R[6 + c];

    RA_CSTAMP(1);
    float d0 = 3.0e38f, d1 = 3.0e38f, d2 = 3.0e38f;
    int i0 = 0, i1 = 0, i2 = 0;
    if (dbg & 1) { d0 = 1e-4f; d1 = 2e-4f; d2 = 3e-4f; i0 = 0; i1 = 1; i2 = 2; }
    else if (BVH) {
        const int nl = fr.bvh_leaves, ns = fr.bvh_supers;
        if (!live) { d0 = d1 = d2 = -1.f; }
        const unsigned long long lm = __ballot(live);
        const int first = lm ? __ffsll((long long)lm) - 1 : 0;
        const int lane = threadIdx.x & 63;
        typedef float f2 __attribute__((ext_vector_type(2)));
        const f2 px2 = {p[0], p[0]}, py2 = {p[1], p[1]}, pz2 = {p[2], p[2]};
        constexpr bool hinted = HINT;
#ifdef RA_COARSE_TS
        int n_rare = 0;
#endif
        typedef float f8 __attribute__((ext_vector_type(8)));
        typedef float f4 __attribute__((ext_vector_type(4)));
        typedef int i4 __attribute__((ext_vector_type(4)));
        auto soa8 = [&](int off) __attribute__((always_inline)) { return *(const f8 __attribute__((address_space(4)))*)(fr.bvh_soa + off); };
        auto soa_id4 = [&](int off) __attribute__((always_inline)) { return *(const i4 __attribute__((address_space(4)))*)(fr.bvh_soa + off); };
        auto box4 = [&](int off) __attribute__((always_inline)) {
            return *(const f4 __attribute__((address_space(4)))*)(reinterpret_cast<const float*>(fr.bvh_sbox) + off);
        };
        auto box1 = [&](int off) __attribute__((always_inline)) { return reinterpret_cast<const float*>(fr.bvh_sbox)[off]; };
        auto scan_leaf = [&](int l) __attribute__((always_inline)) {
            const int L = l * (4 * BVH_LEAF);
            f8 cx = soa8(L), cy = soa8(L + BVH_LEAF), cz = soa8(L + 2 * BVH_LEAF), nx = cx, ny = cy, nz = cz;
            static_for<0, 4>([&](auto q_) {
                constexpr int q = decltype(q_)::value;
                static_for<0, 2>([&](auto g_) {
                    constexpr int g = decltype(g_)::value;
                    const f2 ax = {cx[4 * g], cx[4 * g + 1]}, ay = {cy[4 * g], cy[4 * g + 1]}, az = {cz[4 * g], cz[4 * g + 1]};
                    const f2 bx = {cx[4 * g + 2], cx[4 * g + 3]}, by = {cy[4 * g + 2], cy[4 * g + 3]}, bz = {cz[4 * g + 2], cz[4 * g + 3]};
                    const f2 dxa = px2 - ax, dya = py2 - ay, dza = pz2 - az, dxb = px2 - bx, dyb = py2 - by, dzb = pz2 - bz;
                    f2 da = dya * dya, db = dyb * dyb;
                    da = __builtin_elementwise_fma(dxa, dxa, da);
                    db = __builtin_elementwise_fma(dxb, dxb, db);
                    da = __builtin_elementwise_fma(dza, dza, da);
                    db = __builtin_elementwise_fma(dzb, dzb, db);
                    if (__builtin_expect(__ballot(fminf(fminf(da.x, da.y), fminf(db.x, db.y)) <= d2) != 0ull, 0)) {
#ifdef RA_COARSE_TS
                        ++n_rare;
#endif
                        const i4 id = soa_id4(L + 3 * BVH_LEAF + 8 * q + 4 * g);
                        knn_insert(da.x, id.x, d0, d1, d2, i0, i1, i2, hinted);
                        knn_insert(da.y, id.y, d0, d1, d2, i0, i1, i2, hinted);
                        knn_insert(db.x, id.z, d0, d1, d2, i0, i1, i2, hinted);
                        knn_insert(db.y, id.w, d0, d1, d2, i0, i1, i2, hinted);
                    }
                    if constexpr (g == 0 && q < 3) { nx = soa8(L + 8 * (q + 1)); ny = soa8(L + BVH_LEAF + 8 * (q + 1)); nz = soa8(L + 2 * BVH_LEAF + 8 * (q + 1)); }
                });
                cx = nx; cy = ny; cz = nz;
            });
        };
        int n_scan = 0, n_open = 0;
        if (lm != 0ull) {
            int seed = -1;
            if (hinted) {
                if (live) {
                    float e[3]; int h[3];
#pragma unroll
                    for (int k = 0; k < 3; ++k) {
                        h[k] = rs.hint_src ? rs.hint_src[3 * (size_t)rs.hint_src_index[i] + k] : rs.nn_hint[3 * (size_t)i + k];
                        const float4 v = fr.pverts4[h[k]];
                        e[k] = dist2(p[0] - v.x, p[1] - v.y, p[2] - v.z);
                    }
                    auto before = [&](int a, int b) { return e[a] < e[b] || (e[a] == e[b] && h[a] < h[b]); };
                    auto swap = [&](int a, int b) { const float te = e[a]; e[a] = e[b]; e[b] = te; const int th_ = h[a]; h[a] = h[b]; h[b] = th_; };
                    if (before(1, 0)) swap(0, 1);
                    if (before(2, 1)) swap(1, 2);
                    if (before(1, 0)) swap(0, 1);
                    d0 = e[0]; d1 = e[1]; d2 = e[2]; i0 = h[0]; i1 = h[1]; i2 = h[2];
                }
            } else {
                auto bc = [&](float v) __attribute__((always_inline)) { return __int_as_float(__builtin_amdgcn_readlane(__float_as_int(v), first)); };
                const float q[3] = {bc(p[0]), bc(p[1]), bc(p[2])};
                auto wave_argmin = [&](float d) __attribute__((always_inline)) {
                    float m = d;
#pragma unroll
                    for (int o = 32; o > 0; o >>= 1) m = fminf(m, __shfl_xor(m, o));
                    return __ffsll((long long)__ballot(d == m)) - 1;
                };
                float d = 3.4e38f;
                if (lane < ns) { const int o = 8 * lane; d = box_dist2(q, box1(o), box1(o + 1), box1(o + 2), box1(o + 4), box1(o + 5), box1(o + 6)); }
                const int bi = wave_argmin(d);
                d = 3.4e38f;
                if (lane < BVH_FAN) { const int o = 8 * ns + bi * (6 * BVH_FAN) + 12 * (lane >> 1) + (lane & 1); d = box_dist2(q, box1(o), box1(o + 2), box1(o + 4), box1(o + 6), box1(o + 8), box1(o + 10)); }
                seed = bi * BVH_FAN + wave_argmin(d);
            }
            RA_CSTAMP(2);
            if (!hinted) {
                n_scan = 1;
                scan_leaf(seed);
            }
            RA_CSTAMP(3);
#pragma unroll 1
            for (int j = SPLIT > 1 ? (int)(threadIdx.x >> 6) : 0; j < ns; j += SPLIT) {
                const f4 slo = box4(8 * j), shi = box4(8 * j + 4);
                if (__ballot(box_dist2(p, slo.x, slo.y, slo.z, shi.x, shi.y, shi.z) * 0.99999f <= d2) == 0ull) continue;
                ++n_open;
#pragma unroll 1
                for (int pr = 0; pr < BVH_FAN / 2; ++pr) {
                    const int ro = 8 * ns + j * (6 * BVH_FAN) + 12 * pr;
                    const f4 ra = box4(ro), rb = box4(ro + 4), rc = box4(ro + 8);
                    const f2 ax = f2{ra.x, ra.y} - px2, ay = f2{ra.z, ra.w} - py2, az = f2{rb.x, rb.y} - pz2;
                    const f2 bx = px2 - f2{rb.z, rb.w}, by = py2 - f2{rc.x, rc.y}, bz = pz2 - f2{rc.z, rc.w};
                    const f2 ex = {__builtin_fmaxf(__builtin_fmaxf(ax.x, bx.x), 0.f), __builtin_fmaxf(__builtin_fmaxf(ax.y, bx.y), 0.f)};
                    const f2 ey = {__builtin_fmaxf(__builtin_fmaxf(ay.x, by.x), 0.f), __builtin_fmaxf(__builtin_fmaxf(ay.y, by.y), 0.f)};
                    const f2 ez = {__builtin_fmaxf(__builtin_fmaxf(az.x, bz.x), 0.f), __builtin_fmaxf(__builtin_fmaxf(az.y, bz.y), 0.f)};
                    f2 dd = ex * ex;
                    dd = __builtin_elementwise_fma(ey, ey, dd);
                    dd = __builtin_elementwise_fma(ez, ez, dd);
                    dd *= 0.99999f;
                    const int l = j * BVH_FAN + 2 * pr;
                    if (l != seed && __ballot(dd.x <= d2) != 0ull) { scan_leaf(l); ++n_scan; }
                    if (l + 1 != seed && __ballot(dd.y <= d2) != 0ull) { scan_leaf(l + 1); ++n_scan; }
                }
            }
        }
        RA_CSTAMP(4);
#ifdef RA_COARSE_TS
        if (tsp && (threadIdx.x & 63) == 0) tsp[7] = ((long long)n_scan << 32) | ((long long)n_rare << 12) | n_open;
#endif
        if (SPLIT > 1) {
            __shared__ float md[SPLIT > 1 ? SPLIT - 1 : 1][3][64];
            __shared__ int mi[SPLIT > 1 ? SPLIT - 1 : 1][3][64];
            const int wv = threadIdx.x >> 6;
            if (wv > 0) {
                md[wv - 1][0][lane] = d0; md[wv - 1][1][lane] = d1; md[wv - 1][2][lane] = d2;
                mi[wv - 1][0][lane] = i0; mi[wv - 1][1][lane] = i1; mi[wv - 1][2][lane] = i2;
            }
            __syncthreads();
            if (wv == 0) {
#pragma unroll
                for (int w = 0; w < SPLIT - 1; ++w)
#pragma unroll
                    for (int k = 0; k < 3; ++k) {
                        const int id = mi[w][k][lane];
                        const bool dup = id == i0 || id == i1 || id == i2;
                        knn_insert(dup ? 3.4e38f : md[w][k][lane], id, d0, d1, d2, i0, i1, i2);
                    }
            } else {
                live = false;
            }
        }
        RA_CSTAMP(5);
        if ((dbg & 4) && out.counters && lane == 0) {
// ... 2 lines not shown
        }
    } else {
        float4* sv = reinterpret_cast<float4*>(smem);
        for (int v0 = 0; v0 < fr.n_verts; v0 += VT) {
            const int nv = min(VT, fr.n_verts - v0);
            __syncthreads();
            for (int j = threadIdx.x; j < nv; j += KNN_THREADS) sv[j] = fr.pverts4[v0 + j];
            __syncthreads();
#pragma unroll 4
            for (int j = 0; j < nv; ++j) {
                const float4 v = sv[j];
                const float dx = p[0] - v.x, dy = p[1] - v.y, dz = p[2] - v.z;
                const float d = dist2(dx, dy, dz);
                knn_insert(d, v0 + j, d0, d1, d2, i0, i1, i2);
            }
        }
    }
    if (rs.nn_hint && live) {
        int* hw = rs.nn_hint + 3 * (size_t)i;
        hw[0] = i0; hw[1] = i1; hw[2] = i2;
    }
    if (dbg & 2) { if (live) out.sdf[i] = d0 + d1 + d2 + (float)(i0 + i1 + i2); return; }
    float dk[3] = {d0, d1, d2};
    int ik[3] = {i0, i1, i2};
    float sk[3];
#pragma unroll
    for (int k = 0; k < 3; ++k) {
        const float4 v = fr.pverts4[ik[k]];
        const float* nn = fr.pnorm + 3 * (size_t)ik[k];
        const float dot = (p[0] - v.x) * nn[0] + (p[1] - v.y) * nn[1] + (p[2] - v.z) * nn[2];
        sk[k] = sqrtf(dk[k]) * sgn(dot);
    }
    const float th2 = th * th;
    if (!(dbg & 32)) {
        const float* t0 = fr.tverts + 3 * (size_t)ik[0];
#pragma unroll
        for (int k = 1; k < 3; ++k) {
            const float* tk = fr.tverts + 3 * (size_t)ik[k];
            const float ex = tk[0] - t0[0], ey = tk[1] - t0[1], ez = tk[2] - t0[2];
            if (!(ex * ex + ey * ey + ez * ez < th2)) { dk[k] = dk[0]; ik[k] = ik[0]; sk[k] = sk[0]; }
        }
    }
    float smpl = (sk[0] + sk[1] + sk[2]) / 3.f;
    if (dbg & 32) {
        const float sg = fmaxf(fmaxf(sgn(sk[0]), sgn(sk[1])), sgn(sk[2]));
        smpl = sqrtf((dk[0] + dk[1] + dk[2]) / 3.f) * sg;
        sk[0] = sk[1] = sk[2] = smpl;
    }
    smpl = (smpl < -th) ? smpl : fabsf(smpl);
    const bool fine = live && (d0 < th2);
    if (live) {
        out.sdf[i] = smpl;
        if (out.raw_zero && !fine) {
            float* rz = out.raw_zero + (size_t)i * out.raw_C;
            for (int c = 0; c < out.raw_C; ++c) rz[c] = 0.f;
        }
        if (out.dbg_sdf_batch) {
#pragma unroll
            for (int k = 0; k < 3; ++k) { out.dbg_sdf_batch[3 * i + k] = sk[k]; out.dbg_nn_batch[3 * i + k] = ik[k]; out.dbg_d2[3 * i + k] = dk[k]; }
        }
    }
    __shared__ int wcount[NT / 64 + 1], wcount2[NT / 64 + 1];
    const bool fine2 = fine && out.key != nullptr && out.key[rs.light[i]] != 0;
    const unsigned long long m = __ballot(fine && !fine2), m2 = out.key ? __ballot(fine2) : 0ull;
    const int lane = threadIdx.x & 63, wv = threadIdx.x >> 6;
    if (lane == 0) { wcount[wv] = __popcll(m); wcount2[wv] = __popcll(m2); }
    __syncthreads();
    if (threadIdx.x == 0) {
        int tot = 0, tot2 = 0;
#pragma unroll
        for (int w = 0; w < NT / 64; ++w) { const int cnt = wcount[w]; wcount[w] = tot; tot += cnt; const int c2 = wcount2[w]; wcount2[w] = tot2; tot2 += c2; }
        wcount[NT / 64] = (dbg & 8) ? base : (tot ? atomicAdd(out.fine_count, tot) : 0);
        wcount2[NT / 64] = tot2 ? atomicAdd(out.fine_count2, tot2) : 0;
    }
    __syncthreads();
    RA_CSTAMP(6);
    if (!fine || (dbg & 16)) return;
    const int slot = fine2 ? wcount2[NT / 64] + wcount2[wv] + __popcll(m2 & ((1ull << lane) - 1ull))
                           : wcount[NT / 64] + wcount[wv] + __popcll(m & ((1ull << lane) - 1ull));
    float w[3], ws = 0.f;
#pragma unroll
    for (int k = 0; k < 3; ++k) { w[k] = expf(-dk[k] * inv2r2); ws += w[k]; }
    ws += 1.1920928955078125e-07f;
    float M[24];
#pragma unroll
    for (int e = 0; e < 24; ++e) M[e] = 0.f;
#pragma unroll
    for (int k = 0; k < 3; ++k) {
        const float wk = w[k] / ws;
        const float4* src = reinterpret_cast<const float4*>(fr.vertA + (size_t)ik[k] * 24);
#pragma unroll
        for (int q = 0; q < 6; ++q) {
            const float4 a = src[q];
            M[4 * q] += wk * a.x; M[4 * q + 1] += wk * a.y; M[4 * q + 2] += wk * a.z; M[4 * q + 3] += wk * a.w;
        }
    }
    const float AR[9] = {M[0], M[1], M[2], M[4], M[5], M[6], M[8], M[9], M[10]};
    float Ai[9];
    inv3d(AR, Ai);
    const float q[3] = {p[0] - M[3], p[1] - M[7], p[2] - M[11]};
    float tp[3], bp[3];
#pragma unroll
    for (int r = 0; r < 3; ++r) tp[r] = Ai[3 * r] * q[0] + Ai[3 * r + 1] * q[1] + Ai[3 * r + 2] * q[2];
#pragma unroll
    for (int r = 0; r < 3; ++r) bp[r] = M[12 + 4 * r] * tp[0] + M[12 + 4 * r + 1] * tp[1] + M[12 + 4 * r + 2] * tp[2] + M[12 + 4 * r + 3];
    if (fine2) {
        out.fine_idx2[slot] = i;
        out.bpts2[3 * slot] = bp[0]; out.bpts2[3 * slot + 1] = bp[1]; out.bpts2[3 * slot + 2] = bp[2];
        return;
    }
    out.fine_idx[slot] = i;
    out.bpts[3 * slot] = bp[0]; out.bpts[3 * slot + 1] = bp[1]; out.bpts[3 * slot + 2] = bp[2];
    if (out.mats) {
        float4* dst = reinterpret_cast<float4*>(out.mats + (size_t)slot * 24);
#pragma unroll
        for (int qd = 0; qd < 6; ++qd) dst[qd] = make_float4(M[4 * qd], M[4 * qd + 1], M[4 * qd + 2], M[4 * qd + 3]);
    }
    if (out.dbg_bpts) {
#pragma unroll
        for (int c = 0; c < 3; ++c) { out.dbg_bpts[3 * i + c] = bp[c]; out.dbg_tpts[3 * i + c] = tp[c]; }
#pragma unroll
        for (int e = 0; e < 24; ++e) out.dbg_mats[(size_t)i * 24 + e] = M[e];
    }
}

}

void launch_vert_blend(const float* weights, const float* A, const float* big_A, int n_verts, int n_bones, float* vertA,
                       hipStream_t s) {
    hipLaunchKernelGGL(vert_blend_kernel, dim3((n_verts + 255) / 256), dim3(256), 0, s, weights, A, big_A, n_verts, n_bones, vertA);
}

void launch_pack_verts(const float* pverts, int n_verts, float4* out, hipStream_t s) {
    hipLaunchKernelGGL(pack_verts_kernel, dim3((n_verts + 255) / 256), dim3(256), 0, s, pverts, n_verts, out);
}

void launch_fold_bias(const float* W, int ld, int col0, int ncond, const float* cond, const float* bias, float* out,
                      hipStream_t s) {
    hipLaunchKernelGGL(fold_bias_kernel, dim3(64), dim3(256), 0, s, W, ld, col0, ncond, cond, bias, out);
}

int bvh_leaf_count(int n_verts) {
    if (n_verts > BVH_MAXN) return 0;
    return (n_verts + BVH_LEAF - 1) / BVH_LEAF;
}
int bvh_super_count(int n_leaves) { return (n_leaves + BVH_FAN - 1) / BVH_FAN; }

void launch_bvh_build(const float4* pverts4, int n_verts, int* order, float* leaves, float4* sbox, int n_leaves, int n_supers, hipStream_t s) {
    hipLaunchKernelGGL(bvh_rank_kernel, dim3((n_verts + 63) / 64), dim3(BVH_THREADS), 0, s, pverts4, n_verts, order);
    hipLaunchKernelGGL(bvh_boxes_kernel, dim3(1), dim3(BVH_THREADS), 0, s, pverts4, order, n_verts, leaves, sbox, n_leaves, n_supers);
}

void launch_hdq_coarse(const FrameState& fr, const RaySet& rs, int n, float th, float blend_radius, const HdqOut& out,
                       hipStream_t s, bool geodesic) {
    if (n <= 0) return;
    const float inv2r2 = 1.f / (2.f * blend_radius * blend_radius);
    const dim3 grid((n + KNN_THREADS - 1) / KNN_THREADS);
    int dbg = 0, probe = 0, split_max = 196608;
#ifdef RA_TESTING
    static const int e_dbg = getenv("RA_COARSE_DBG") ? atoi(getenv("RA_COARSE_DBG")) : 0;
    static const int e_probe = getenv("RA_COARSE_PROBE") ? atoi(getenv("RA_COARSE_PROBE")) : 0;
    static const int e_split = getenv("RA_COARSE_SPLIT_MAX") ? atoi(getenv("RA_COARSE_SPLIT_MAX")) : 196608;
    dbg = e_dbg; probe = e_probe; split_max = e_split;
#endif
    if (!geodesic) dbg |= 32;
#ifdef RA_COARSE_TS
    static int launch_no = 0;
    dbg |= (launch_no++ & 63) << 8;
#endif
    const bool hint = (rs.nn_hint != nullptr && rs.hint_valid != 0) || rs.hint_src != nullptr;
    for (int pass = probe ? 0 : 1; pass < 2; ++pass) {
        const int d = pass == 0 ? probe : dbg;
        if (fr.bvh_leaves > 0 && n <= split_max)
        {
            const int groups = (n + 63) / 64;
            if (hint) {
                if (n <= split_max / 8) hipLaunchKernelGGL((hdq_coarse_kernel<true, 16, true>), dim3(groups), dim3(1024), 0, s, fr, rs, n, th, inv2r2, out, d);
                else if (n <= split_max / 2) hipLaunchKernelGGL((hdq_coarse_kernel<true, 8, true>), dim3(groups), dim3(512), 0, s, fr, rs, n, th, inv2r2, out, d);
                else hipLaunchKernelGGL((hdq_coarse_kernel<true, 4, true>), dim3(groups), dim3(256), 0, s, fr, rs, n, th, inv2r2, out, d);
            } else {
                if (n <= split_max / 8) hipLaunchKernelGGL((hdq_coarse_kernel<true, 16>), dim3(groups), dim3(1024), 0, s, fr, rs, n, th, inv2r2, out, d);
                else if (n <= split_max / 2) hipLaunchKernelGGL((hdq_coarse_kernel<true, 8>), dim3(groups), dim3(512), 0, s, fr, rs, n, th, inv2r2, out, d);
                else hipLaunchKernelGGL((hdq_coarse_kernel<true, 4>), dim3(groups), dim3(256), 0, s, fr, rs, n, th, inv2r2, out, d);
            }
        }
        else if (fr.bvh_leaves > 0 && hint) hipLaunchKernelGGL((hdq_coarse_kernel<true, 1, true>), grid, dim3(KNN_THREADS), 0, s, fr, rs, n, th, inv2r2, out, d);
        else if (fr.bvh_leaves > 0) hipLaunchKernelGGL((hdq_coarse_kernel<true, 1>), grid, dim3(KNN_THREADS), 0, s, fr, rs, n, th, inv2r2, out, d);
        else hipLaunchKernelGGL((hdq_coarse_kernel<false, 1>), grid, dim3(KNN_THREADS), 0, s, fr, rs, n, th, inv2r2, out, d);
        if (pass == 0) hipMemsetAsync(out.fine_count, 0, sizeof(int), s);
    }
}
```

### relightableavatar_amd/csrc/ra_kernels.hpp

```cpp
#pragma once
#include "ra_common.hpp"
#include "ra_lpips_pack.hpp"

struct RaySet {
    int mode;
    const float* x;
    const float* o;
    const float* d;
    const float* t;
    const int* pix;
    const int* light;
    const float* ldir;
    const int* n_dev;
    const unsigned char* skip;
    int* nn_hint;
    int hint_valid;
    const int* hint_src;
    const int* hint_src_index;
};

struct HdqOut {
    float* sdf;
    int* fine_count;
    int* fine_idx;
    float* bpts;
    float* mats;
    const unsigned char* key;
    int* fine_count2;
    int* fine_idx2;
    float* bpts2;
    float* raw_zero;
    int raw_C;
    float* dbg_sdf_batch;
    int* dbg_nn_batch;
    float* dbg_d2;
    float* dbg_tpts;
    float* dbg_bpts;
    float* dbg_mats;
    DevCounters* counters;
};

void launch_vert_blend(const float* weights, const float* A, const float* big_A, int n_verts, int n_bones, float* vertA,
                       hipStream_t s);
void launch_pack_verts(const float* pverts, int n_verts, float4* out, hipStream_t s);
void launch_fold_bias(const float* W, int ld, int col0, int ncond, const float* cond, const float* bias, float* out,
                      hipStream_t s);
void launch_bvh_build(const float4* pverts4, int n_verts, int* order, float* leaves, float4* sbox, int n_leaves, int n_supers, hipStream_t s);
int bvh_leaf_count(int n_verts);
int bvh_super_count(int n_leaves);
void launch_hdq_coarse(const FrameState& fr, const RaySet& rs, int n, float th, float blend_radius, const HdqOut& out,
                       hipStream_t s, bool geodesic = true);

struct TraceState {
    float *t, *d0, *dt, *st, *ot, *cd, *occ, *off, *rlx;
    const float *near_, *far_;
    const float* tan_i;
    const int* light;
    unsigned char* stuck;
};
void launch_trace_init(const TraceState& ts, int n, const int* n_dev, const ra_trace_params& p, hipStream_t s);

void launch_trace_update(const TraceState& ts, const float* sdf, int n, const int* n_dev, int iter,
                         const ra_trace_params& p, hipStream_t s);

void launch_surface_finish(const float* ray_o, const float* ray_d, const float* st, const float* occ, int P, float* surf,
                           float* depth, float* acc, int* hit_idx, int* hit_count, hipStream_t s, int* slot_of_ray = nullptr,
                           bool counter_is_zero = false);
void launch_slot_index(const int* hit_idx, const int* hit_count, int P, int* slot_of_ray, hipStream_t s);
struct MapJob { const float* src; float* dst; int C; int premul; int src_full; };
constexpr int RA_MAX_MAP_JOBS = 16;
struct EmitMaps { MapJob job[RA_MAX_MAP_JOBS]; long long end[RA_MAX_MAP_JOBS]; int n_jobs; const int* slot_of_ray; const float* acc; const int* perm; int P; };
void launch_emit_maps(const EmitMaps& m, hipStream_t s);
void launch_surface_samples(const float* surf, const float* ray_d, const int* hit_idx, const int* hit_count, int P, int S,
                            float range, float* x, float* v, int* n_out, hipStream_t s);
struct SurfaceMaps {
    float *cpts, *bpts, *resd, *norm, *albedo, *rough, *rgb;
    float* valbedo;
};
void launch_surface_composite(const float* raw, int C, int S, const int* hit_count, int P, int relight, const ra_config& cfg,
                              const SurfaceMaps& m, hipStream_t s);

constexpr int RA_MAX_BOXES = 32;
struct ShadowGen {
    const float* surf;
    const float* norm;
    const float* acc;
    const int* hit_idx;
    const int* hit_count;
    const float* ldir;
    float bbox[6];
    int n_boxes;
    float boxes[RA_MAX_BOXES][6];
    int box_start[RA_MAX_BOXES + 1];
    const int* perm;
    float near_offset;
    int L;
    int no_visibility, local_visibility;
    int split_wide_groups;
    float* lvis;
    float* ldot;
    int* ray_pix;
    int* ray_light;
    int* ray_slot;
    float *near_, *far_;
    int* ray_count;
};
void launch_key_lights(const float* probes, int n, int ph, int pw, const float* ldir, const float* area, int L, float share, int kmax,
                       int accumulate, float* smax, unsigned char* key, hipStream_t s);
void launch_gather_shard_rays(const long long* idx, int n, const float* ro, const float* rd, const float* nr, const float* fr, float* so, float* sd,
                              float* sn, float* sf, hipStream_t s);
void launch_scatter_rows(const float* src, const long long* src_idx, const long long* dst_idx, long long n, int C, float* dst, hipStream_t s);
void launch_shadow_gen(const ShadowGen& g, int P, hipStream_t s, bool counter_is_zero = false);
void launch_debug_aabb(const float* o, const float* d, int n, const float* bbox6, float* nr, float* fr, hipStream_t s);
void launch_debug_brdf(const float* p2l, const float* p2c, const float* nrm, const float* alb, const float* rough, int L, int N, const ra_config& cfg,
                       float* out, hipStream_t s);
size_t sort_hits_temp_bytes(int P);
int launch_sort_hits(const float* surf, const float* acc, int P, const float* bbox_min, unsigned* keys_in, unsigned* keys_out,
                     int* vals_in, int* hit_idx_out, void* temp, size_t temp_bytes, hipStream_t s);
void launch_shadow_scatter(const float* occ, const int* ray_slot, const int* ray_count, int max_rays, float* lvis, hipStream_t s);

struct ShadeIn {
    const float* ray_o;
    const float* surf;
    const int* idx;
    const int* count;
    int n;
    const float *norm, *albedo, *rough;
    const float *lvis, *ldot;
    const float *light_xyz, *light_area;
    int L;
    const float* probes;
    int n_probes, ph, pw;
    int want_spec;
    float *rgb, *shade, *spec;
};
void launch_shade(const ShadeIn& in, const ra_config& cfg, hipStream_t s);

constexpr int SHADE_BWD_MAX_GRID = 768;
constexpr size_t SHADE_BWD_LDS_BYTES = 65536;
struct ShadeBwd {
    const float *ray_o, *surf, *norm, *albedo, *rough;
    const float* lvis;
    const float *light_xyz, *light_area; int L;
    const float* probes; int n_probes, ph, pw;
    const float* d_rgb;
    int P;
    float *d_albedo, *d_rough, *d_probes;
    float* slabs;
};
int shade_bwd_grid(int P);
int shade_bwd_probes_per_launch(int ph, int pw);
void launch_shade_bwd(const ShadeBwd& a, const ra_config& cfg, hipStream_t s);

constexpr int HEADS_PARAMS = 99332;
constexpr int HEADS_MAX_GRID = 128;
constexpr int HEADS_CHUNK = 32768;
constexpr size_t HEADS_TAPE_BYTES_PER_TILE = 163840;
constexpr size_t HEADS_W16_BYTES = 2 * 66048 * 2;
struct HeadsIO {
    const float *theta, *feat;
    int n;
    float *albedo, *rough;
    const float *d_albedo, *d_rough;
    float* d_theta;
    void* w16;
    unsigned* amax;
    void* tape;
    float* slabs;
};
int heads_grid(int n);
void launch_heads_forward(const HeadsIO& io, const ra_config& cfg, hipStream_t s);
void launch_heads_backward(const HeadsIO& io, const ra_config& cfg, hipStream_t s);

constexpr int ENTROPY_MAX_GRID = 256;
int entropy_grid(int n);
size_t entropy_scratch_doubles(int n);
void launch_gaussian_entropy(const float* x, int n, const float* d_value, float* value, float* d_x, double* scratch, hipStream_t s);

struct MetricsIO {
    const float *pred, *gt;
    const long long* pix;
    int P;
    const unsigned char* mask;
    int H, W;
    float bg, data_range;
    int mse_over_rays, crop_to_mask;
    double* out;
    void* scratch;
};
size_t metrics_scratch_bytes(int H, int W, bool ray_list);
void launch_image_metrics(const MetricsIO& io, hipStream_t s);

struct LpipsIO {
    const float *pred, *gt;
    const long long* pix;
    int P;
    const unsigned char* mask;
    int H, W;
    float bg;
    int crop_to_mask;
    double* out;
    void* scratch;
    const float* arena;
    LpipsArena off;
};
size_t lpips_scratch_bytes(int H, int W, bool ray_list);
void launch_lpips(const LpipsIO& io, hipStream_t s);
void launch_lpips_features(const LpipsIO& io, int tap, float* out, hipStream_t s);
void lpips_feature_shape(int H, int W, int tap, int* C, int* h, int* w);

constexpr int MESH_LEAF = 32;
constexpr int MESH_FAN = 8;
constexpr int MESH_REC = 12;
constexpr int MESH_MAX_FACES = 1 << 24;
constexpr int MESH_SORT_MIN = 64;
struct MeshView {
    const float* recs;
    const float* lbox;
    const float* gbox;
    int n_faces, n_leaves, n_groups;
};
struct MeshBuild {
    int* faces;
    unsigned* bb;
    unsigned *keys, *keys_sorted;
    int *vals, *vals_sorted;
    void* temp;
    size_t temp_bytes;
};
struct MeshQuery {
    const float* pts;
    int n, brute;
    const int* perm;
    float *d2, *closest, *bary;
    int* face;
};
inline int mesh_leaf_count(int n_faces) { return (n_faces + MESH_LEAF - 1) / MESH_LEAF; }
inline int mesh_group_count(int n_leaves) { return (n_leaves + MESH_FAN - 1) / MESH_FAN; }
size_t mesh_sort_temp_bytes(int n);
int launch_mesh_build(const float* verts, const MeshBuild& b, const MeshView& m, float* recs, float* lbox, float* gbox, hipStream_t s);
int launch_mesh_sort_points(const float* pts, int n, const MeshBuild& b, hipStream_t s);
void launch_mesh_closest(const MeshView& m, const MeshQuery& q, hipStream_t s);

constexpr int WIND_BLOCK = 64;
constexpr int WIND_CHUNK = 1024;
constexpr int WIND_SPLIT_TILES = 2048;
constexpr long long WIND_SPLIT_MAX = 1ll << 24;
inline int wind_chunk_count(int n_leaves) { return (int)(((long long)n_leaves * MESH_LEAF + WIND_CHUNK - 1) / WIND_CHUNK); }
void launch_mesh_winding(const MeshView& m, const float* pts, int n, double* partial, float* out, hipStream_t s);
void launch_mesh_winding_grad(const MeshView& m, const float* pts, int n, double* partial, float* winding, float* grad, hipStream_t s);

constexpr int RAY_BLOCK = 64;
constexpr int RAY_PAIR_BLOCK = 256;
constexpr long long RAY_MAX_PAIRS = 1ll << 31;
struct RayQuery {
    const float *o, *d;
    int n, brute;
    const int* perm;
    float *t, *uv;
    int *face, *count;
};
void launch_mesh_raycast(const MeshView& m, const RayQuery& q, hipStream_t s);
void launch_ray_tri_pairs(const float* o, const float* d, int n, const float* tris, int f, float* u, float* v, float* t, hipStream_t s);

constexpr int TOPO_BLOCK = 256;
constexpr int TOPO_SMOOTH_BLOCK = 256;
constexpr int TOPO_MAX_FACES = (1 << 29) / 3;
constexpr int TOPO_MAX_CHANNELS = 64;
enum { TOPO_BAD = 0, TOPO_E = 1, TOPO_MAX_NBR = 2, TOPO_MAX_OUT = 3, TOPO_MAX_COUNT = 4, TOPO_STAT_INTS = 5 };
struct TopoView {
    int n_faces, n_verts, n_edges;
    const int *vert, *twin, *edge;
// ... 178 lines not shown
```

### relightableavatar_amd/csrc/ra_trace.hip

```cpp
#include "ra_kernels.hpp"
#include "ra_shade_dev.hpp"
#include <hipcub/hipcub.hpp>

namespace {

constexpr int TPB = 256;

__device__ __forceinline__ int live_count(const int* n_dev, int n) { return n_dev ? min(*n_dev, n) : n; }

__device__ __forceinline__ float linspace01(int s, int S) {
    if (S == 1) return 0.f;
    const float step = 1.f / (float)(S - 1);
    return (s < S / 2) ? (float)s * step : 1.f - (float)(S - 1 - s) * step;
}

__global__ void trace_init_kernel(TraceState ts, int n_launch, const int* n_dev, float offset, float relax) {
    const int i = blockIdx.x * TPB + threadIdx.x;
    if (i >= live_count(n_dev, n_launch)) return;
    const float nr = ts.near_[i], fr = ts.far_[i];
    ts.t[i] = nr;
    ts.d0[i] = 1e9f;
    ts.occ[i] = 1.f;
    if (ts.stuck) ts.stuck[i] = 0;
    if (ts.dt) ts.dt[i] = 1e9f;
    if (ts.st) ts.st[i] = fr;
    if (ts.ot) ts.ot[i] = fr;
    if (ts.cd) ts.cd[i] = 1e9f;
    if (ts.off) ts.off[i] = offset;
    if (ts.rlx) ts.rlx[i] = relax;
}

template <bool SOFT>
__global__ void trace_update_kernel(TraceState ts, const float* __restrict__ sdf, int n_launch, const int* n_dev, int iter,
                                    ra_trace_params p) {
    const int i = blockIdx.x * TPB + threadIdx.x;
    if (i >= live_count(n_dev, n_launch)) return;
    const float d1 = sdf[i];
    const float d0 = ts.d0[i];
    float t = ts.t[i];
    const float t_prev = t;
    float occ = ts.occ[i];
    const float nr = ts.near_[i], fr = ts.far_[i];
    float tan_i = p.tan_i;
    if (SOFT) {
        const float ti = ts.tan_i ? (ts.light ? ts.tan_i[ts.light[i]] : ts.tan_i[i]) : p.tan_i;
        tan_i = p.tan_i_multiplier * ti;
    }
    const float tan2 = (1.f / tan_i) * 2.f;
    float off = ts.off ? ts.off[i] : p.offset;
    float rlx = ts.rlx ? ts.rlx[i] : p.relax;
    float ot = ts.ot ? ts.ot[i] : 0.f;
    if (SOFT && p.clay_book && iter >= p.shadow_skip_iter) {
        const float dx0 = d0 + rlx * d0 + off;
        const float dx1 = d1 + rlx * d1 + off;
        const float dy = (dx1 * dx1) / (2.f * dx0);
        const float dx = (sqrtf(dx1 * dx1 - dy * dy) - off) / (1.f + rlx);
        const float den = fmaxf(fmaxf(t - dy, nr), p.eps);
        const float cls = fmaxf(dx, 0.f) / den / tan2;
        const bool msk = (cls < occ) && (dy < t) && (dx1 > 0.f) && (dx0 > 0.f) && (dx > 0.f) && (dy > 0.f) && (dy < dx0);
        if (msk) { ot = t - dy; occ = cls; }
    }
    if (iter >= p.shadow_skip_iter) {
        const float cls = fmaxf(d1, 0.f) / fmaxf(fmaxf(t, nr), p.eps) / tan2;
        if (cls < occ) { ot = t; occ = cls; }
    }
    if (!SOFT) {
        const float d1u = fabsf(d1), d0u = fabsf(d0);
        float st = ts.st[i], cd = ts.cd[i];
        const float dt = ts.dt[i];
        const float s0 = (d0 > 0.f) ? 1.f : ((d0 < 0.f) ? -1.f : 0.f);
        const float s1 = (d1 > 0.f) ? 1.f : ((d1 < 0.f) ? -1.f : 0.f);
        if (s0 != s1) {
            st = t - dt * fminf(fmaxf(d1u / (d0u + d1u + p.eps), 0.f), 1.f);
            off = 0.f;
            rlx = 0.f;
        }
        if (d1u < cd) { cd = d1u; st = t; }
        ts.st[i] = st;
        ts.cd[i] = cd;
        ts.off[i] = off;
        ts.rlx[i] = rlx;
    }
    const float dtn = d1 + rlx * d1 + off;
    t = t + dtn;
    t = fminf(t, fr);
    t = fmaxf(t, nr);
    if (ts.dt) ts.dt[i] = dtn;
    ts.t[i] = t;
    if (ts.stuck) ts.stuck[i] = (t == t_prev || (SOFT && occ == 0.f)) ? 1 : 0;
    ts.d0[i] = d1;
    ts.occ[i] = occ;
    if (ts.ot) ts.ot[i] = ot;
}

__global__ void surface_finish_kernel(const float* __restrict__ ro, const float* __restrict__ rd, const float* __restrict__ st,
                                      const float* __restrict__ occ, int P, float* __restrict__ surf, float* __restrict__ depth,
                                      float* __restrict__ acc, int* __restrict__ hit_idx, int* __restrict__ hit_count, int* __restrict__ slot_of_ray) {
    const int i = blockIdx.x * TPB + threadIdx.x;
    bool hit = false;
    if (i < P) {
        if (slot_of_ray) slot_of_ray[i] = -1;
        const float s = st[i];
        const float sx = ro[3 * i] + s * rd[3 * i], sy = ro[3 * i + 1] + s * rd[3 * i + 1], sz = ro[3 * i + 2] + s * rd[3 * i + 2];
        surf[3 * i] = sx; surf[3 * i + 1] = sy; surf[3 * i + 2] = sz;
        depth[i] = (sx - ro[3 * i]) / rd[3 * i];
        const float a = 1.f - occ[i];
        acc[i] = a;
        hit = a > 0.f;
    }
    const unsigned long long m = __ballot(hit);
    if (m == 0ull) return;
    const int lane = threadIdx.x & 63;
    int base = 0;
    if (lane == 0) base = atomicAdd(hit_count, __popcll(m));
    base = __shfl(base, 0);
    if (hit) hit_idx[base + __popcll(m & ((1ull << lane) - 1ull))] = i;
}

__device__ __forceinline__ unsigned expand10t(unsigned v) {
    v = (v * 0x00010001u) & 0xFF0000FFu;
    v = (v * 0x00000101u) & 0x0F00F00Fu;
    v = (v * 0x00000011u) & 0xC30C30C3u;
    v = (v * 0x00000005u) & 0x49249249u;
    return v;
}

__global__ void hit_keys_kernel(const float* __restrict__ surf, const float* __restrict__ acc, int P, float bx, float by, float bz,
                                unsigned* __restrict__ keys, int* __restrict__ vals) {
    const int i = blockIdx.x * TPB + threadIdx.x;
    if (i >= P) return;
    unsigned k = 0xffffffffu;
    if (acc[i] > 0.f) {
        const unsigned qx = (unsigned)fminf(fmaxf((surf[3 * i] - bx) * 256.f, 0.f), 1023.f);
        const unsigned qy = (unsigned)fminf(fmaxf((surf[3 * i + 1] - by) * 256.f, 0.f), 1023.f);
        const unsigned qz = (unsigned)fminf(fmaxf((surf[3 * i + 2] - bz) * 256.f, 0.f), 1023.f);
        k = (expand10t(qx) << 2) | (expand10t(qy) << 1) | expand10t(qz);
    }
    keys[i] = k;
    vals[i] = i;
}

__global__ void ray_keys_kernel(const float* __restrict__ ro, const float* __restrict__ rd, const float* __restrict__ nr, int P,
                                float bx, float by, float bz, const float* __restrict__ origin_dev, unsigned* __restrict__ keys,
                                int* __restrict__ vals) {
    const int i = blockIdx.x * TPB + threadIdx.x;
    if (i >= P) return;
    if (origin_dev) { bx = origin_dev[0]; by = origin_dev[1]; bz = origin_dev[2]; }
    const float t = nr[i];
    const unsigned qx = (unsigned)fminf(fmaxf((ro[3 * i] + t * rd[3 * i] - bx) * 256.f, 0.f), 1023.f);
    const unsigned qy = (unsigned)fminf(fmaxf((ro[3 * i + 1] + t * rd[3 * i + 1] - by) * 256.f, 0.f), 1023.f);
    const unsigned qz = (unsigned)fminf(fmaxf((ro[3 * i + 2] + t * rd[3 * i + 2] - bz) * 256.f, 0.f), 1023.f);
    keys[i] = (expand10t(qx) << 2) | (expand10t(qy) << 1) | expand10t(qz);
    vals[i] = i;
}

__global__ __launch_bounds__(1024) void entry_min_kernel(const float* __restrict__ ro, const float* __restrict__ rd, const float* __restrict__ nr,
                                                         int P, float* __restrict__ out) {
    __shared__ float sm_[16][3];
    float lo[3] = {3.4e38f, 3.4e38f, 3.4e38f};
    for (int i = threadIdx.x; i < P; i += 1024)
#pragma unroll
        for (int c = 0; c < 3; ++c) lo[c] = fminf(lo[c], ro[3 * i + c] + nr[i] * rd[3 * i + c]);
#pragma unroll
    for (int c = 0; c < 3; ++c)
#pragma unroll
        for (int o = 32; o > 0; o >>= 1) lo[c] = fminf(lo[c], __shfl_xor(lo[c], o));
    if ((threadIdx.x & 63) == 0)
#pragma unroll
        for (int c = 0; c < 3; ++c) sm_[threadIdx.x >> 6][c] = lo[c];
    __syncthreads();
    if (threadIdx.x < 3) {
        float a = sm_[0][threadIdx.x];
        for (int w = 1; w < 16; ++w) a = fminf(a, sm_[w][threadIdx.x]);
        out[threadIdx.x] = a;
    }
}

__global__ void gather_rays_kernel(const int* __restrict__ perm, int P, const float* __restrict__ ro, const float* __restrict__ rd,
                                   const float* __restrict__ nr, const float* __restrict__ fr, float* __restrict__ so, float* __restrict__ sd,
                                   float* __restrict__ sn, float* __restrict__ sf, float near_min, float far_max) {
    const int i = blockIdx.x * TPB + threadIdx.x;
    if (i >= P) return;
    const int r = perm[i];
#pragma unroll
    for (int c = 0; c < 3; ++c) { so[3 * i + c] = ro[3 * r + c]; sd[3 * i + c] = rd[3 * r + c]; }
    sn[i] = fmaxf(nr[r], near_min);
    sf[i] = fminf(fr[r], far_max);
}

__global__ void gather_shard_rays_kernel(const long long* __restrict__ idx, int n, const float* __restrict__ ro, const float* __restrict__ rd,
                                         const float* __restrict__ nr, const float* __restrict__ fr, float* __restrict__ so, float* __restrict__ sd,
                                         float* __restrict__ sn, float* __restrict__ sf) {
    const int i = blockIdx.x * TPB + threadIdx.x;
    if (i >= n) return;
    const long long r = idx[i];
#pragma unroll
    for (int c = 0; c < 3; ++c) { so[3 * i + c] = ro[3 * r + c]; sd[3 * i + c] = rd[3 * r + c]; }
    sn[i] = nr[r];
    sf[i] = fr[r];
}

__global__ void scatter_rows_kernel(const float* __restrict__ src, const long long* __restrict__ src_idx, const long long* __restrict__ dst_idx,
                                    long long n, int C, float* __restrict__ dst) {
    const long long k = (long long)blockIdx.x * TPB + threadIdx.x;
    if (k >= n * C) return;
    const long long i = k / C;
    const int c = (int)(k - i * C);
    dst[dst_idx[i] * C + c] = src[src_idx[i] * C + c];
}

__global__ void surface_samples_kernel(const float* __restrict__ surf, const float* __restrict__ rd, const int* __restrict__ hit_idx,
                                       const int* __restrict__ hit_count, int S, float range, float* __restrict__ x,
                                       float* __restrict__ v, int* __restrict__ n_out) {
    const int nh = *hit_count;
    const int k = blockIdx.x * TPB + threadIdx.x;
    if (k == 0) *n_out = nh * S;
    if (k >= nh * S) return;
    const int h = k / S, s = k - h * S;
    const int r = hit_idx[h];
    const float zv = (S == 1) ? 0.5f : linspace01(s, S);
    const float z = zv * (2.f * range) - range;
#pragma unroll
    for (int c = 0; c < 3; ++c) {
        const float d = rd[3 * r + c];
        x[3 * k + c] = surf[3 * r + c] + z * d;
        v[3 * k + c] = d;
    }
}

__global__ void surface_composite_kernel(const float* __restrict__ raw, int C, int S, const int* __restrict__ hit_count, int relight,
                                         ra_config cfg, SurfaceMaps m) {
    const int h = blockIdx.x * TPB + threadIdx.x;
    if (h >= *hit_count) return;
    float out[16];
    const int CC = C - 1;
#pragma unroll
    for (int c = 0; c < 16; ++c) out[c] = 0.f;
    float T = 1.f, accw = 0.f;
    for (int s = 0; s < S; ++s) {
        const float* r = raw + ((size_t)h * S + s) * C;
        const float a = r[CC];
        const float w = a * T;
// ... 31 lines not shown
__global__ void light_dirs_kernel(const float* __restrict__ xyz, int L, float* __restrict__ ldir) {
    const int l = blockIdx.x * TPB + threadIdx.x;
    if (l >= L) return;
    const float x = xyz[3 * l], y = xyz[3 * l + 1], z = xyz[3 * l + 2];
    const float n = sqrtf(x * x + y * y + z * z) + 1e-8f;
    ldir[3 * l] = x / n; ldir[3 * l + 1] = y / n; ldir[3 * l + 2] = z / n;
}

__device__ __forceinline__ void aabb_near_far(const float* bbox, const float o[3], const float dir[3], float& nr, float& fr) {
    float d[3] = {dir[0], dir[1], dir[2]};
    nr = -3.0e38f; fr = 3.0e38f;
#pragma unroll
    for (int c = 0; c < 3; ++c) {
        if (d[c] < 1e-8f && d[c] > -1e-16f) d[c] = 1e-8f;
        const float t0 = (bbox[c] - o[c]) / d[c], t1 = (bbox[3 + c] - o[c]) / d[c];
        nr = fmaxf(nr, fminf(t0, t1));
        fr = fminf(fr, fmaxf(t0, t1));
    }
}
struct Box6 { float v[6]; };
__global__ void debug_aabb_kernel(const float* __restrict__ o, const float* __restrict__ d, int n, Box6 b, float* __restrict__ nr, float* __restrict__ fr) {
    const int i = blockIdx.x * TPB + threadIdx.x;
    if (i >= n) return;
    const float oo[3] = {o[3 * i], o[3 * i + 1], o[3 * i + 2]}, dd[3] = {d[3 * i], d[3 * i + 1], d[3 * i + 2]};
    float a, f;
    aabb_near_far(b.v, oo, dd, a, f);
    nr[i] = a; fr[i] = f;
}

constexpr int SG_LIGHTS = 32;
constexpr float SG_SPLIT_EXTENT = 0.15f;
__global__ __launch_bounds__(TPB) void shadow_gen_kernel(ShadowGen g) {
    __shared__ float t_ldot[64][SG_LIGHTS + 1], t_lvis[64][SG_LIGHTS + 1];
    const int nh = *g.hit_count;
    const int lchunks = (g.L + SG_LIGHTS - 1) / SG_LIGHTS;
    const int grp = blockIdx.x / lchunks, lc = blockIdx.x - grp * lchunks;
    if (grp * 64 >= nh) return;
    const int lane = threadIdx.x & 63, wv = threadIdx.x >> 6;
    const int h = grp * 64 + lane;
    const bool hv = h < nh;
    int r = 0;
    float nrm[3] = {0.f, 0.f, 0.f}, o[3] = {0.f, 0.f, 0.f}, acc = 0.f;
    float box[6] = {g.bbox[0], g.bbox[1], g.bbox[2], g.bbox[3], g.bbox[4], g.bbox[5]};
    if (hv) {
        r = g.hit_idx[h];
        if (g.n_boxes > 1) {
            const int rc = g.perm ? g.perm[r] : r;
            int j = 0;
            for (int k = 1; k < g.n_boxes; ++k) j += rc >= g.box_start[k];
#pragma unroll
            for (int k = 0; k < 6; ++k) box[k] = g.boxes[j][k];
        }
        nrm[0] = g.norm[3 * h]; nrm[1] = g.norm[3 * h + 1]; nrm[2] = g.norm[3 * h + 2];
        o[0] = g.surf[3 * r]; o[1] = g.surf[3 * r + 1]; o[2] = g.surf[3 * r + 2];
        acc = g.acc[r];
    }
    constexpr int ROUNDS = SG_LIGHTS / (TPB / 64);
    constexpr int NL = ROUNDS * (TPB / 64);
    __shared__ int cnt[2][NL + 1];
    float nrv[ROUNDS], frv[ROUNDS];
    unsigned tmask = 0;
    float ext = 0.f;
    {
        float lo3[3], hi3[3];
#pragma unroll
        for (int k = 0; k < 3; ++k) { lo3[k] = hv ? o[k] : 3e38f; hi3[k] = hv ? o[k] : -3e38f; }
#pragma unroll
        for (int k = 0; k < 3; ++k)
#pragma unroll
            for (int sh = 32; sh > 0; sh >>= 1) { lo3[k] = fminf(lo3[k], __shfl_xor(lo3[k], sh)); hi3[k] = fmaxf(hi3[k], __shfl_xor(hi3[k], sh)); }
        ext = fmaxf(fmaxf(hi3[0] - lo3[0], hi3[1] - lo3[1]), hi3[2] - lo3[2]);
    }
    const bool halves = g.split_wide_groups && ext > SG_SPLIT_EXTENT;
#pragma unroll
    for (int round = 0; round < ROUNDS; ++round) {
        const int ll = round * (TPB / 64) + wv;
        const int l = lc * SG_LIGHTS + ll;
        bool trace = false;
        float nr = 0.f, fr = 0.f;
        if (hv && l < g.L) {
            const float dx = g.ldir[3 * l], dy = g.ldir[3 * l + 1], dz = g.ldir[3 * l + 2];
            const float ldot = dx * nrm[0] + dy * nrm[1] + dz * nrm[2];
            float lv;
            if (g.no_visibility) lv = 1.f;
            else if (g.local_visibility) lv = ldot > 0.f ? 1.f : 0.f;
            else {
                const bool front = (ldot > 0.f) && (acc > 0.f);
                lv = 0.f;
                if (front) {
                    const float d[3] = {dx, dy, dz};
                    aabb_near_far(box, o, d, nr, fr);
                    nr = fmaxf(nr, g.near_offset);
                    fr = fmaxf(fr, g.near_offset);
                    trace = nr < fr;
                    lv = 1.f;
                }
            }
            t_ldot[lane][ll] = ldot;
            t_lvis[lane][ll] = lv;
        }
        nrv[round] = nr; frv[round] = fr;
        if (trace) tmask |= 1u << round;
        const unsigned long long m = __ballot(trace);
        if (lane == 0) { cnt[0][ll] = __popcll(m & 0xffffffffull); cnt[1][ll] = __popcll(m >> 32); }
    }
    __syncthreads();
    if (threadIdx.x == 0) {
        int tot = 0;
        if (halves) {
            for (int hf = 0; hf < 2; ++hf)
                for (int k = 0; k < NL; ++k) { const int c = cnt[hf][k]; cnt[hf][k] = tot; tot += c; }
        } else {
            for (int k = 0; k < NL; ++k) {
                const int c0 = cnt[0][k], c1 = cnt[1][k];
                cnt[0][k] = tot; cnt[1][k] = tot + c0; tot += c0 + c1;
            }
        }
        cnt[0][NL] = tot ? atomicAdd(g.ray_count, tot) : 0;
    }
    __syncthreads();
    const int gbase = cnt[0][NL];
#pragma unroll
    for (int round = 0; round < ROUNDS; ++round) {
        const int ll = round * (TPB / 64) + wv;
        const bool trace = (tmask >> round) & 1u;
        const unsigned long long m = __ballot(trace);
        if (trace) {
            const int hf = lane >> 5;
            const unsigned mh = hf ? (unsigned)(m >> 32) : (unsigned)m;
            const int s = gbase + cnt[hf][ll] + __popc(mh & ((1u << (lane & 31)) - 1u));
            const int l = lc * SG_LIGHTS + ll;
            g.ray_pix[s] = r;
            g.ray_light[s] = l;
            g.ray_slot[s] = h * g.L + l;
            g.near_[s] = nrv[round];
            g.far_[s] = frv[round];
        }
    }
    const int col = threadIdx.x & (SG_LIGHTS - 1), l = lc * SG_LIGHTS + col;
    for (int row = threadIdx.x / SG_LIGHTS; row < 64; row += TPB / SG_LIGHTS) {
        const int hh = grp * 64 + row;
        if (hh < nh && l < g.L) {
            g.ldot[(size_t)hh * g.L + l] = t_ldot[row][col];
            g.lvis[(size_t)hh * g.L + l] = t_lvis[row][col];
        }
    }
}

__global__ void shadow_scatter_kernel(const float* __restrict__ occ, const int* __restrict__ ray_slot, const int* __restrict__ ray_count,
                                      int max_rays, float* __restrict__ lvis) {
    const int i = blockIdx.x * TPB + threadIdx.x;
    if (i >= min(*ray_count, max_rays)) return;
    lvis[ray_slot[i]] = occ[i];
}

__global__ __launch_bounds__(TPB) void key_lights_kernel(const float* __restrict__ probes, int n, int ph, int pw, const float* __restrict__ ldir,
                                                         const float* __restrict__ area, int L, float share, int kmax, int accumulate,
                                                         float* __restrict__ smax, unsigned char* __restrict__ key) {
    extern __shared__ float kl_w[];
    __shared__ float red[TPB / 64];
    for (int q = 0; q < n; ++q) {
        const float* img = probes + (size_t)q * ph * pw * 3;
        float part = 0.f;
        for (int l = threadIdx.x; l < L; l += TPB) {
            const float d[3] = {ldir[3 * l], ldir[3 * l + 1], ldir[3 * l + 2]};
            float c[3];
            sample_probe(img, ph, pw, d, c);
            float w = (c[0] + c[1] + c[2]) * (1.f / 3.f) * area[l];
            w = w > 0.f ? w : 0.f;
            kl_w[l] = w;
            part += w;
        }
#pragma unroll
        for (int sh = 32; sh > 0; sh >>= 1) part += __shfl_xor(part, sh);
        if ((threadIdx.x & 63) == 0) red[threadIdx.x >> 6] = part;
        __syncthreads();
        float total = 0.f;
#pragma unroll
        for (int k = 0; k < TPB / 64; ++k) total += red[k];
        for (int l = threadIdx.x; l < L; l += TPB) {
            const float sh_l = total > 0.f ? kl_w[l] / total : 0.f;
            smax[l] = (q == 0 && !accumulate) ? sh_l : fmaxf(smax[l], sh_l);
        }
        __syncthreads();
    }
    for (int l = threadIdx.x; l < L; l += TPB) kl_w[l] = smax[l];
    __syncthreads();
    const float thr = fmaxf(share, 4.f / (float)L);
    for (int l = threadIdx.x; l < L; l += TPB) {
        const float w = kl_w[l];
        bool cand = w >= thr;
        if (cand) {
            int rank = 0;
            for (int j = 0; j < L; ++j) rank += (kl_w[j] > w) || (kl_w[j] == w && j < l);
            cand = rank < kmax;
        }
        key[l] = (unsigned char)cand;
    }
}

__global__ void debug_brdf_kernel(const float* __restrict__ p2l, const float* __restrict__ p2c, const float* __restrict__ nrm, const float* __restrict__ alb,
                                  const float* __restrict__ rough, int L, int N, ra_config cfg, float* __restrict__ out) {
    const int i = blockIdx.x * TPB + threadIdx.x;
    if (i >= L * N) return;
    const int p = i % N;
    const float v[3] = {p2c[3 * p], p2c[3 * p + 1], p2c[3 * p + 2]}, n[3] = {nrm[3 * p], nrm[3 * p + 1], nrm[3 * p + 2]};
    const float a[3] = {alb[3 * p], alb[3 * p + 1], alb[3 * p + 2]}, l[3] = {p2l[3 * i], p2l[3 * i + 1], p2l[3 * i + 2]};
    const MfView mv = mf_view(v, n, rough[p]);
    float brdf[3], sb;
    mf_light(mv, l, a, cfg, brdf, sb);
    out[3 * i] = brdf[0]; out[3 * i + 1] = brdf[1]; out[3 * i + 2] = brdf[2];
}

constexpr int MAXP = 8;
__global__ __launch_bounds__(TPB) void shade_kernel(ShadeIn in, ra_config cfg) {
    const int n = in.count ? min(*in.count, in.n) : in.n;
    const int wave = (blockIdx.x * TPB + threadIdx.x) >> 6;
    const int lane = threadIdx.x & 63;
    if (wave >= n) return;
    const int h = wave;
    const int r = in.idx ? in.idx[h] : h;
    const float sp[3] = {in.surf[3 * r], in.surf[3 * r + 1], in.surf[3 * r + 2]};
    float v[3] = {in.ray_o[3 * r] - sp[0], in.ray_o[3 * r + 1] - sp[1], in.ray_o[3 * r + 2] - sp[2]};
    {
        const float nn = sqrtf(v[0] * v[0] + v[1] * v[1] + v[2] * v[2]) + 1e-8f;
        v[0] /= nn; v[1] /= nn; v[2] /= nn;
        fnormalize(v);
    }
    const float nraw[3] = {in.norm[3 * h], in.norm[3 * h + 1], in.norm[3 * h + 2]};
    const float alb[3] = {in.albedo[3 * h], in.albedo[3 * h + 1], in.albedo[3 * h + 2]};
    const MfView mv = mf_view(v, nraw, in.rough[h]);

    float rgb[MAXP][3], shd[MAXP][3], spc[MAXP][3];
#pragma unroll
    for (int q = 0; q < MAXP; ++q)
#pragma unroll
        for (int c = 0; c < 3; ++c) rgb[q][c] = shd[q][c] = spc[q][c] = 0.f;
    float vis_sum = 0.f;

    for (int l = lane; l < in.L; l += 64) {
        float s2l[3] = {in.light_xyz[3 * l] - sp[0], in.light_xyz[3 * l + 1] - sp[1], in.light_xyz[3 * l + 2] - sp[2]};
        {
            const float nn = sqrtf(s2l[0] * s2l[0] + s2l[1] * s2l[1] + s2l[2] * s2l[2]) + 1e-8f;
            s2l[0] /= nn; s2l[1] /= nn; s2l[2] /= nn;
        }
        float brdf[3], sbrdf;
        mf_light(mv, s2l, alb, cfg, brdf, sbrdf);
        const float area = in.light_area[l];
        const float lv = in.lvis[(size_t)h * in.L + l];
        const float ld = cfg.only_visibility ? 1.f : in.ldot[(size_t)h * in.L + l];
        const float spec_ld = 1.f / (fabsf(1.f) + 1e-8f);
        vis_sum += cfg.vis_shade_map == 1 ? lv : ld;
        for (int q = 0; q < in.n_probes; ++q) {
            float Lr[3];
            sample_probe(in.probes + (size_t)q * in.ph * in.pw * 3, in.ph, in.pw, s2l, Lr);
            if (cfg.only_visibility) Lr[0] = Lr[1] = Lr[2] = (Lr[0] + Lr[1] + Lr[2]) / 3.f;
#pragma unroll
            for (int c = 0; c < 3; ++c) {
                const float sh = lv * 1.f * area * Lr[c];
                rgb[q][c] += brdf[c] * sh;
                shd[q][c] += lv * ld * area * Lr[c];
                spc[q][c] += sbrdf * (1.f * spec_ld * area * Lr[c]);
            }
        }
    }
#pragma unroll
    for (int o = 32; o > 0; o >>= 1) vis_sum += __shfl_xor(vis_sum, o);
    for (int q = 0; q < in.n_probes; ++q) {
#pragma unroll
        for (int c = 0; c < 3; ++c) {
            float a = rgb[q][c], b = shd[q][c], d = spc[q][c];
#pragma unroll
            for (int o = 32; o > 0; o >>= 1) { a += __shfl_xor(a, o); b += __shfl_xor(b, o); d += __shfl_xor(d, o); }
            if (lane == 0) {
                const size_t k = ((size_t)q * in.n + h) * 3 + c;
                if (in.rgb) in.rgb[k] = cfg.tonemapping ? srgb(a) : a;
                if (in.shade) in.shade[k] = cfg.vis_shade_map ? vis_sum / (float)in.L : b * cfg.shading_albedo / PI_F;
                if (in.spec && in.want_spec) in.spec[k] = d;
            }
        }
    }
}

__global__ void slot_index_kernel(const int* __restrict__ hit_idx, const int* __restrict__ hit_count, int* __restrict__ slot_of_ray) {
    const int k = blockIdx.x * TPB + threadIdx.x;
    if (k < *hit_count) slot_of_ray[hit_idx[k]] = k;
}

__global__ void emit_maps_kernel(EmitMaps m) {
    long long k = (long long)blockIdx.x * TPB + threadIdx.x;
    int j = 0;
    long long start = 0;
    while (j < m.n_jobs && k >= m.end[j]) { start = m.end[j]; ++j; }
    if (j >= m.n_jobs) return;
    const MapJob& J = m.job[j];
    k -= start;
    const int r = (int)(k / J.C), c = (int)(k - (long long)r * J.C);
    const int slot = m.slot_of_ray[r];
    float v = 0.f;
    if (slot >= 0) {
        v = J.src_full ? J.src[(size_t)r * J.C + c] : J.src[(size_t)slot * J.C + c];
        if (J.premul) v *= m.acc[r];
    }
    J.dst[(size_t)(m.perm ? m.perm[r] : r) * J.C + c] = v;
}

// ... 545 lines not shown
__global__ void light_probe_kernel(ProbeInset p, const float* __restrict__ probe, float* __restrict__ rgb) {
    const int k = blockIdx.x * TPB + threadIdx.x;
    if (k >= p.uH * p.uW) return;
    const int y = k / p.uW, x = k - y * p.uW;
    const float lat_half = PI_F / p.uH / 2.f, lng_half = 2.f * PI_F / p.uW / 2.f;
    auto lin = [](float a, float b, int n, int i) { const float st = (b - a) / (float)(n - 1); return i < n / 2 ? a + i * st : b - (n - 1 - i) * st; };
    const float lat = p.uH > 1 ? lin(PI_F / 2.f - lat_half, -PI_F / 2.f + lat_half, p.uH, y) : PI_F / 2.f - lat_half;
    const float lng = p.uW > 1 ? lin(PI_F - lng_half, -PI_F + lng_half, p.uW, x) : PI_F - lng_half;
    float v[3] = {cosf(lat) * cosf(lng), cosf(lat) * sinf(lng), sinf(lat)};
    const float nn = sqrtf(v[0] * v[0] + v[1] * v[1] + v[2] * v[2]) + 1e-8f;
    float d[3];
#pragma unroll
    for (int r = 0; r < 3; ++r) d[r] = (v[0] * p.axes[3 * r] + v[1] * p.axes[3 * r + 1] + v[2] * p.axes[3 * r + 2]) / nn;
    float c[3];
    sample_probe(probe, p.ph, p.pw, d, c);
    float* o = rgb + ((size_t)y * p.W + x) * 3;
    o[0] = c[0]; o[1] = c[1]; o[2] = c[2];
}

__global__ void grow_bounds_kernel(float* __restrict__ wb, float m) {
    const int k = threadIdx.x;
    if (k < 6) wb[k] = k < 3 ? wb[k] - m : wb[k] + m;
}
void launch_grow_bounds(float* wbounds6, float margin, hipStream_t s) { hipLaunchKernelGGL(grow_bounds_kernel, dim3(1), dim3(64), 0, s, wbounds6, margin); }

void launch_shift_envmap(const float* img, int H, int W, int C, float shift, float* out, hipStream_t s) {
    if (H * W <= 0) return;
    hipLaunchKernelGGL(shift_envmap_kernel, grid_for(H * W), dim3(TPB), 0, s, img, H, W, C, shift, out);
}

void launch_light_probe(const ProbeInset& p, const float* probe, float* rgb, hipStream_t s) {
    if (p.uH * p.uW <= 0) return;
    hipLaunchKernelGGL(light_probe_kernel, grid_for(p.uH * p.uW), dim3(TPB), 0, s, p, probe, rgb);
}

__device__ __forceinline__ bool pixel_ray(const RayCam& c, int pix, float o[3], float d[3], float& nr, float& fr) {
    const double x = (double)(pix % c.W), y = (double)(pix / c.W);
    double pc[3], pw[3];
#pragma unroll
    for (int k = 0; k < 3; ++k) pc[k] = x * c.Kinv[3 * k] + y * c.Kinv[3 * k + 1] + c.Kinv[3 * k + 2] - c.T[k];
#pragma unroll
    for (int k = 0; k < 3; ++k) pw[k] = pc[0] * c.R[k] + pc[1] * c.R[3 + k] + pc[2] * c.R[6 + k] - c.o[k];
    const double inv = 1.0 / sqrt(pw[0] * pw[0] + pw[1] * pw[1] + pw[2] * pw[2]);
#pragma unroll
    for (int k = 0; k < 3; ++k) { d[k] = (float)(pw[k] * inv); o[k] = (float)c.o[k]; }
    const float nd = sqrtf(d[0] * d[0] + d[1] * d[1] + d[2] * d[2]);
    float t_near = -3.4e38f, t_far = 3.4e38f;
#pragma unroll
    for (int k = 0; k < 3; ++k) {
        float v = d[k] / nd;
        if (v < 1e-5f && v > -1e-10f) v = 1e-5f;
        if (v > -1e-5f && v < 1e-10f) v = -1e-5f;
        const float lo = c.bdev ? c.bdev[k] : c.bmin[k], hi = c.bdev ? c.bdev[3 + k] : c.bmax[k];
        const float t0 = (lo - o[k]) / v, t1 = (hi - o[k]) / v;
        t_near = fmaxf(t_near, fminf(t0, t1));
        t_far = fminf(t_far, fmaxf(t0, t1));
    }
    nr = t_near / nd / nd;
    fr = t_far / nd / nd;
    return t_near < t_far;
}

__global__ void ray_mask_kernel(RayCam c, unsigned char* __restrict__ mask) {
    const int i = blockIdx.x * TPB + threadIdx.x;
    if (i >= c.H * c.W) return;
    float o[3], d[3], nr, fr;
    mask[i] = pixel_ray(c, i, o, d, nr, fr) ? 1 : 0;
}

__global__ void ray_emit_kernel(RayCam c, const int* __restrict__ pix_idx, const int* __restrict__ count, float* __restrict__ ro,
                                float* __restrict__ rd, float* __restrict__ near_, float* __restrict__ far_) {
    const int i = blockIdx.x * TPB + threadIdx.x;
    if (i >= *count) return;
    float o[3], d[3], nr, fr;
    pixel_ray(c, pix_idx[i], o, d, nr, fr);
#pragma unroll
    for (int k = 0; k < 3; ++k) { ro[3 * i + k] = o[k]; rd[3 * i + k] = d[k]; }
    near_[i] = nr;
    far_[i] = fr;
}

size_t gen_rays_temp_bytes(int n) {
    size_t bytes = 0;
    hipcub::DeviceSelect::Flagged(nullptr, bytes, hipcub::CountingInputIterator<int>(0), (const unsigned char*)nullptr, (int*)nullptr, (int*)nullptr, n);
    return bytes;
}

int launch_gen_rays(const RayCam& cam, unsigned char* mask, int* pix_idx, int* count_dev, void* temp, size_t temp_bytes,
                    float* ray_o, float* ray_d, float* near, float* far, hipStream_t s) {
    const int n = cam.H * cam.W;
    if (n <= 0) { hipMemsetAsync(count_dev, 0, sizeof(int), s); return 0; }
    hipLaunchKernelGGL(ray_mask_kernel, grid_for(n), dim3(TPB), 0, s, cam, mask);
    if (hipcub::DeviceSelect::Flagged(temp, temp_bytes, hipcub::CountingInputIterator<int>(0), mask, pix_idx, count_dev, n, s) != hipSuccess) return 1;
    hipLaunchKernelGGL(ray_emit_kernel, grid_for(n), dim3(TPB), 0, s, cam, pix_idx, count_dev, ray_o, ray_d, near, far);
    return 0;
}

size_t sort_hits_temp_bytes(int P) {
    size_t bytes = 0;
    hipcub::DeviceRadixSort::SortPairs(nullptr, bytes, (const unsigned*)nullptr, (unsigned*)nullptr, (const int*)nullptr, (int*)nullptr, P);
    return bytes;
}

int launch_sort_hits(const float* surf, const float* acc, int P, const float* bbox_min, unsigned* keys_in, unsigned* keys_out,
                     int* vals_in, int* hit_idx_out, void* temp, size_t temp_bytes, hipStream_t s) {
    if (P <= 0) return 0;
    hipLaunchKernelGGL(hit_keys_kernel, grid_for(P), dim3(TPB), 0, s, surf, acc, P, bbox_min[0], bbox_min[1], bbox_min[2], keys_in, vals_in);
    return hipcub::DeviceRadixSort::SortPairs(temp, temp_bytes, keys_in, keys_out, vals_in, hit_idx_out, P, 0, 32, s) == hipSuccess ? 0 : 1;
}

void launch_shadow_scatter(const float* occ, const int* ray_slot, const int* ray_count, int max_rays, float* lvis, hipStream_t s) {
    if (max_rays <= 0) return;
    hipLaunchKernelGGL(shadow_scatter_kernel, grid_for(max_rays), dim3(TPB), 0, s, occ, ray_slot, ray_count, max_rays, lvis);
}

void launch_shade(const ShadeIn& in, const ra_config& cfg, hipStream_t s) {
    if (in.n <= 0) return;
    hipLaunchKernelGGL(shade_kernel, grid_for((long long)in.n * 64), dim3(TPB), 0, s, in, cfg);
}

void launch_scatter_maps(const int* hit_idx, const int* hit_count, int P, int premultiply, const float* acc_full, const float* src,
                         int C, float* dst, int src_full, const int* perm, hipStream_t s) {
    if (P <= 0) return;
    hipLaunchKernelGGL(scatter_maps_kernel, grid_for((long long)P * C), dim3(TPB), 0, s, hit_idx, hit_count, premultiply, acc_full, src, C, dst, src_full, perm);
}

int launch_sort_rays(const float* ro, const float* rd, const float* nr, const float* fr, int P, const float* bbox_min, unsigned* keys_in,
                     unsigned* keys_out, int* vals_in, int* perm, void* temp, size_t temp_bytes, float* so, float* sd, float* sn, float* sf,
                     hipStream_t s, float near_min, float far_max) {
    if (P <= 0) return 0;
    float* origin_dev = nullptr;
    if (!bbox_min) {
        origin_dev = reinterpret_cast<float*>(keys_out);
        hipLaunchKernelGGL(entry_min_kernel, dim3(1), dim3(1024), 0, s, ro, rd, nr, P, origin_dev);
    }
    hipLaunchKernelGGL(ray_keys_kernel, grid_for(P), dim3(TPB), 0, s, ro, rd, nr, P, bbox_min ? bbox_min[0] : 0.f, bbox_min ? bbox_min[1] : 0.f,
                       bbox_min ? bbox_min[2] : 0.f, origin_dev, keys_in, vals_in);
    if (hipcub::DeviceRadixSort::SortPairs(temp, temp_bytes, keys_in, keys_out, vals_in, perm, P, 0, 32, s) != hipSuccess) return 1;
    hipLaunchKernelGGL(gather_rays_kernel, grid_for(P), dim3(TPB), 0, s, perm, P, ro, rd, nr, fr, so, sd, sn, sf, near_min, far_max);
    return 0;
}

void launch_gather_shard_rays(const long long* idx, int n, const float* ro, const float* rd, const float* nr, const float* fr, float* so, float* sd,
                              float* sn, float* sf, hipStream_t s) {
    if (n <= 0) return;
    hipLaunchKernelGGL(gather_shard_rays_kernel, grid_for(n), dim3(TPB), 0, s, idx, n, ro, rd, nr, fr, so, sd, sn, sf);
}

void launch_scatter_rows(const float* src, const long long* src_idx, const long long* dst_idx, long long n, int C, float* dst, hipStream_t s) {
    if (n <= 0) return;
    hipLaunchKernelGGL(scatter_rows_kernel, grid_for(n * C), dim3(TPB), 0, s, src, src_idx, dst_idx, n, C, dst);
}

void launch_accumulate(const int* count, unsigned long long* dst, hipStream_t s) {
    hipLaunchKernelGGL(accumulate_kernel, dim3(1), dim3(1), 0, s, count, dst);
}

void launch_gather_rows(const int* hit_idx, const int* hit_count, int P, const float* src, int C, float* dst, hipStream_t s) {
    if (P <= 0) return;
    hipLaunchKernelGGL(gather_rows_kernel, grid_for((long long)P * C), dim3(TPB), 0, s, hit_idx, hit_count, src, C, dst);
}

__global__ void iota_kernel(int* __restrict__ idx, int n, int* __restrict__ count) {
    const int i = blockIdx.x * TPB + threadIdx.x;
    if (i == 0 && count) *count = n;
    if (i < n) idx[i] = i;
}
void launch_iota(int* idx, int n, int* count, hipStream_t s) {
    hipLaunchKernelGGL(iota_kernel, grid_for(n > 0 ? n : 1), dim3(TPB), 0, s, idx, n, count);
}

__device__ __forceinline__ void affine_inverse4(const float* A, float* o) {
#pragma unroll
    for (int r = 0; r < 3; ++r) {
#pragma unroll
        for (int c = 0; c < 3; ++c) o[4 * r + c] = A[4 * c + r];
        o[4 * r + 3] = -(A[r] * A[3] + A[4 + r] * A[7] + A[8 + r] * A[11]);
    }
#pragma unroll
    for (int c = 0; c < 4; ++c) o[12 + c] = A[12 + c];
}
__device__ __forceinline__ void matmul4(const float* A, const float* B, float* o) {
#pragma unroll
    for (int r = 0; r < 4; ++r)
#pragma unroll
        for (int c = 0; c < 4; ++c) o[4 * r + c] = A[4 * r] * B[c] + A[4 * r + 1] * B[4 + c] + A[4 * r + 2] * B[8 + c] + A[4 * r + 3] * B[12 + c];
}
__global__ void bigpose_compose_kernel(const float* __restrict__ mats, const float* __restrict__ d2, int n, float inv2r2, const float* __restrict__ R,
                                       const float* __restrict__ Th, int invert, float* __restrict__ out) {
    const int i = blockIdx.x * TPB + threadIdx.x;
    if (i >= n) return;
    float ws = 0.f;
#pragma unroll
    for (int k = 0; k < 3; ++k) ws += expf(-d2[3 * i + k] * inv2r2);
    const float sden = ws + 1.1920928955078125e-07f;
    float sb = 0.f;
#pragma unroll
    for (int k = 0; k < 3; ++k) sb += expf(-d2[3 * i + k] * inv2r2) / sden;
    float A[16], B[16], P2W[16], t0[16], t1[16], t2[16];
#pragma unroll
    for (int e = 0; e < 12; ++e) { A[e] = mats[(size_t)i * 24 + e]; B[e] = mats[(size_t)i * 24 + 12 + e]; }
    A[12] = A[13] = A[14] = 0.f; A[15] = sb;
    B[12] = B[13] = B[14] = 0.f; B[15] = sb;
#pragma unroll
    for (int r = 0; r < 3; ++r) { P2W[4 * r] = R[3 * r]; P2W[4 * r + 1] = R[3 * r + 1]; P2W[4 * r + 2] = R[3 * r + 2]; P2W[4 * r + 3] = Th[r]; }
    P2W[12] = P2W[13] = P2W[14] = 0.f; P2W[15] = 1.f;
    affine_inverse4(P2W, t0);
    affine_inverse4(A, t1);
    matmul4(B, t1, t2);
    matmul4(t2, t0, t1);
    if (invert) { affine_inverse4(t1, t0); for (int e = 0; e < 16; ++e) out[(size_t)i * 16 + e] = t0[e]; }
    else for (int e = 0; e < 16; ++e) out[(size_t)i * 16 + e] = t1[e];
}
void launch_bigpose_compose(const float* mats, const float* d2, int n, float blend_radius, const float* R, const float* Th, int invert, float* out,
                            hipStream_t s) {
    if (n <= 0) return;
    hipLaunchKernelGGL(bigpose_compose_kernel, grid_for(n), dim3(TPB), 0, s, mats, d2, n, 1.f / (2.f * blend_radius * blend_radius), R, Th, invert, out);
}

void launch_fill(float* p, size_t n, float v, hipStream_t s) {
    if (n == 0) return;
    if (v == 0.f) { hipMemsetAsync(p, 0, n * sizeof(float), s); return; }
    hipLaunchKernelGGL(fill_kernel, grid_for((long long)n), dim3(TPB), 0, s, p, n, v);
}

void launch_volume_samples(const float* ray_o, const float* ray_d, const float* near_, const float* far_, int P, int S, float* x,
                           float* v, hipStream_t s) {
    if (P <= 0) return;
    hipLaunchKernelGGL(volume_samples_kernel, grid_for((long long)((P + 63) & ~63) * S), dim3(TPB), 0, s, ray_o, ray_d, near_, far_, P, S, x, v);
}

void launch_volume_composite(const float* raw, int C, const float* near_, const float* far_, int P, int S, float bg,
                             const ra_render_out& out, const int* perm, hipStream_t s) {
    if (P <= 0) return;
    if (C != 16) { fprintf(stderr, "relightableavatar: volume compositing expects 16 raw channels, got %d\n", C); abort(); }
    hipLaunchKernelGGL(volume_composite_kernel, dim3((P + 63) / 64), dim3(64 * VC_SEG), 0, s, raw, near_, far_, P, S, bg, out, perm);
}
```

### relightableavatar_amd/engine.py

```python
import contextlib
import ctypes as C
import weakref

import torch

from . import _lib
from ._lib import (check, ra_config, ra_counters, ra_frame, ra_ground_out, ra_ground_params, ra_lpips_weights, ra_metrics_params, ra_pose_in, ra_pose_out,
                   ra_render_out, ra_sphere_params, ra_trace_params)
from . import lpips_weights
from .base_utils import dotdict


def _ptr(t):
    return None if t is None else C.c_void_p(t.data_ptr())


def _f32(t: torch.Tensor, device) -> torch.Tensor:
    return t.detach().to(device=device, dtype=torch.float32).contiguous()


def _bbox6(bbox6):
    return (C.c_float * 6)(*[float(v) for v in bbox6])


# ... 226 lines not shown
        out = torch.empty_like(src)
        check(eng.lib.ra_topo_dilate(eng.ctx, self._handle, _ptr(src), self.V, abs(steps), _ptr(out), eng.stream), 'ra_topo_dilate')
        out = out != 0
        return ~out if steps < 0 else out

    def _rows(self, who, x, eng):
        v = _f32(x, eng.device)
        if v.shape[:1] != (self.V,) or v.ndim not in (1, 2) or (v.ndim == 2 and not 1 <= v.shape[1] <= 64):
            raise ValueError(f'Topology.{who}: rows must be ({self.V}, C) with 1 <= C <= 64, or ({self.V},)')
        return v, v.reshape(self.V, 1 if v.ndim == 1 else v.shape[1])

    def diffuse_apply(self, x, lam):
        eng = self._live_engine()
        v, v2 = self._rows('diffuse_apply', x, eng)
        out = torch.empty_like(v2)
        check(eng.lib.ra_topo_diffuse_apply(eng.ctx, self._handle, _ptr(v2) if self.V else None, self.V, max(v2.shape[1], 1), float(lam),
                                            _ptr(out) if self.V else None, eng.stream), 'ra_topo_diffuse_apply')
        return out.reshape(v.shape)

    def diffuse_solve(self, b, lam, x0=None, tol=1e-9, max_iter=256, info=False):
        eng = self._live_engine()
        v, v2 = self._rows('diffuse_solve', b, eng)
        start = None
        if x0 is not None:
            start = _f32(x0, eng.device).reshape(self.V, -1)
            if start.shape != v2.shape:
                raise ValueError('Topology.diffuse_solve: x0 must have the shape of b')
        out = torch.empty_like(v2)
        Cn = max(v2.shape[1], 1)
        rec = torch.zeros(Cn, 2, dtype=torch.float64, device=eng.device) if info else None
        check(eng.lib.ra_topo_diffuse_solve(eng.ctx, self._handle, _ptr(v2) if self.V else None, self.V, Cn, float(lam),
                                            _ptr(start) if start is not None and self.V else None, float(tol), int(max_iter),
                                            _ptr(out) if self.V else None, _ptr(rec), eng.stream), 'ra_topo_diffuse_solve')
        out = out.reshape(v.shape)
        if not info:
            return out
        words = rec[:, 0].contiguous().view(torch.int32).view(Cn, 2)
        return out, dotdict(iters=words[:, 0], stop=words[:, 1], residual=rec[:, 1])

    NORMALS = ('face_normal', 'face_area', 'vert_normal')

    def normals(self, verts, want=NORMALS):
        eng = self._live_engine()
        want = tuple(want)
        if not want or any(k not in self.NORMALS for k in want):
            raise ValueError(f'Topology.normals: want must be a non-empty subset of {self.NORMALS}')
        v = _f32(verts, eng.device)
        if v.shape != (self.V, 3):
            raise ValueError(f'Topology.normals: verts must be ({self.V}, 3)')
        out = dotdict()
        for k in want:
            out[k] = torch.zeros({'face_normal': (self.F, 3), 'face_area': (self.F,), 'vert_normal': (self.V, 3)}[k], dtype=torch.float32, device=eng.device)
        ptrs = [_ptr(out[k]) if k in out and out[k].numel() else None for k in self.NORMALS]
        if any(p is not None for p in ptrs):
            check(eng.lib.ra_mesh_normals(eng.ctx, self._handle, _ptr(v), self.V, *ptrs, eng.stream), 'ra_mesh_normals')
        return out

    def close(self):
        eng = self._engine()
        if self._handle.value and eng is not None and eng.ctx.value:
            check(eng.lib.ra_topo_destroy(eng.ctx, self._handle), 'ra_topo_destroy')
        self._handle = C.c_void_p()

    def __del__(self):
        try:
            self.close()
        except Exception:
            pass


class Cloth:

    TERMS = {'stretch': _lib.RA_CLOTH_STRETCH, 'bending': _lib.RA_CLOTH_BENDING, 'gravity': _lib.RA_CLOTH_GRAVITY}

    def __init__(self, engine, handle, topology, coeffs):
        self._engine, self._handle, self.topology, self._cache = weakref.ref(engine), handle, topology, None
        self.coeffs = coeffs

    def _live_engine(self):
        eng = self._engine()
        if eng is None or not eng.ctx.value:
            raise _lib.RaError('Cloth: the engine that built this cloth is gone')
        if not self._handle.value:
            raise _lib.RaError('Cloth: closed')
        return eng

    @property
    def arrays(self):
        if self._cache is None:
            eng, t = self._live_engine(), self.topology
            out = dotdict()
            for k, (name, n, dt) in enumerate((('f_area', t.F, torch.float32), ('Dm', 4 * t.F, torch.float32), ('Dm_inv', 4 * t.F, torch.float32),
                                               ('v_mass', t.V, torch.float32), ('inv_mass', t.V, torch.float32), ('hinge_faces', 2 * t.E, torch.int32),
                                               ('hinge_verts', 2 * t.E, torch.int32))):
                a = torch.empty(n, dtype=dt, device=eng.device)
                check(eng.lib.ra_cloth_array(eng.ctx, self._handle, k, _ptr(a) if n else None, eng.stream), 'ra_cloth_array')
                out[name] = a
            out.Dm, out.Dm_inv = out.Dm.view(-1, 2, 2), out.Dm_inv.view(-1, 2, 2)
            hf, hv = out.pop('hinge_faces').view(-1, 2).long(), out.pop('hinge_verts').view(-1, 2).long()
            keep = hf[:, 0] >= 0
            out.f_connectivity, out.f_connectivity_edges = hf[keep], hv[keep]
            self._cache = out
        return self._cache

    def energy(self, x, terms=('stretch', 'bending'), gravity=9.81, grad=True):
        eng = self._live_engine()
        v = _f32(x, eng.device)
        if v.ndim != 3 or v.shape[1:] != (self.topology.V, 3) or v.shape[0] < 1:
            raise ValueError(f'Cloth.energy: x must be (B, {self.topology.V}, 3) with B >= 1')
        bits = 0
        for k in terms:
            bits |= self.TERMS[k]
        energy = torch.empty(v.shape[0], 3, dtype=torch.float64, device=eng.device)
        g = torch.empty_like(v) if grad else None
        check(eng.lib.ra_cloth_energy(eng.ctx, self._handle, _ptr(v) if v.numel() else None, v.shape[0], bits, float(gravity), _ptr(energy),
                                      _ptr(g) if g is not None and g.numel() else None, eng.stream), 'ra_cloth_energy')
        return energy, g

    def close(self):
        eng = self._engine()
        if self._handle.value and eng is not None and eng.ctx.value:
            check(eng.lib.ra_cloth_destroy(eng.ctx, self._handle), 'ra_cloth_destroy')
        self._handle = C.c_void_p()

    def __del__(self):
        try:
            self.close()
        except Exception:
            pass


class Engine:
    def __init__(self, cfg, device=None, relight=False):
        if not torch.cuda.is_available():
            raise _lib.RaError('relightableavatar_amd needs a HIP device (MI355X); there is no CPU fallback for the render path')
        self.lib = _lib.lib()
        self.device = torch.device('cuda', torch.cuda.current_device()) if device is None else torch.device(device)
        self.cfg = cfg
        self.ctx = C.c_void_p()
        check(self.lib.ra_ctx_create(C.byref(self.ctx), self.device.index or 0), 'ra_ctx_create')
        self.relight = bool(relight)
        c = ra_config(xyz_res=cfg.xyz_res, sdf_res=cfg.sdf_res, view_res=cfg.view_res, n_bones=cfg.n_bones, relight=int(self.relight),
                      resd_limit=cfg.resd_limit, blend_radius=cfg.blend_radius, albedo_slope=cfg.albedo_slope,
                      albedo_bias=cfg.albedo_bias, roughness_slope=cfg.roughness_slope, roughness_bias=cfg.roughness_bias,
                      fresnel_f0=cfg.fresnel_f0, shading_albedo=cfg.shading_albedo, albedo_multiplier=cfg.albedo_multiplier,
                      lambert_only=int(cfg.lambert_only), glossy_only=int(cfg.glossy_only),
                      tonemapping=int(cfg.tonemapping_rendering), bg_brightness=cfg.bg_brightness,
                      mlp_f16=int(cfg.mlp_dtype == 'f16'), query_skip=int(cfg.get('query_skip', True)),
                      k4_batch_slots=int(cfg.get('k4_batch_slots', 0)), trace_precision=int(cfg.get('trace_precision', 1)),
                      clip_near=float(cfg.get('clip_near', 0.02)), clip_far=float(cfg.get('clip_far', 10.0)),
                      only_visibility=int(bool(cfg.get('only_visibility', False))),
                      vis_shade_map=2 if cfg.get('vis_ldot_map', False) else (1 if cfg.get('vis_lvis_map', False) else 0),
                      use_geodesic_filter=int(bool(cfg.get('use_geodesic_filter', True))),
                      key_light_share=float(cfg.get('key_light_share', 0.0078)))
        assert cfg.mlp_dtype in ('f16', 'bf16')
        check(self.lib.ra_set_config(self.ctx, C.byref(c)), 'ra_set_config')
        self._frame_key = None
        self._frame_refs = None
        self._keep = []

    def __del__(self):
        try:
            if getattr(self, 'ctx', None) and self.ctx.value:
                self.lib.ra_ctx_destroy(self.ctx)
                self.ctx = C.c_void_p()
        except Exception:
            pass

    @property
    def stream(self):
        return C.c_void_p(torch.cuda.current_stream(self.device).cuda_stream)

    def load_state_dict(self, sd: dict):
        for k, v in sd.items():
            if not isinstance(v, torch.Tensor) or not v.dtype.is_floating_point:
                continue
            h = v.detach().to('cpu', torch.float32).contiguous()
            check(self.lib.ra_set_weight(self.ctx, k.encode(), C.c_void_p(h.data_ptr()), h.numel()), f'ra_set_weight({k})')
        check(self.lib.ra_finalize_weights(self.ctx, self.stream), 'ra_finalize_weights')
        self._frame_key = None

    FRAME_KEYS = ('R', 'Th', 'poses', 'A', 'big_A', 'pverts', 'pnorm', 'tverts', 'weights')

    def _cond_fix_source(self, batch):
        if self.relight:
            return None
        c = self.cfg
        if c.fix_material >= 0 or c.always_fix_material:
            tm = batch.get('train_motion', None) if hasattr(batch, 'get') else None
            if tm is None or 'poses' not in tm:
                raise ValueError('cfg.fix_material / cfg.always_fix_material need batch.train_motion.poses (base_network.py:502-503)')
            return tm['poses']
        return batch['poses']

    def set_frame(self, batch, force=False):
        src = [batch[k] for k in self.FRAME_KEYS]
        cf_src = self._cond_fix_source(batch)
        refs = src + [cf_src]
        key = tuple(None if t is None else t._version for t in refs) + (int(self.cfg.fix_material), bool(self.cfg.always_fix_material))
        if (not force and self._frame_key == key and self._frame_refs is not None and len(self._frame_refs) == len(refs)
                and all(a is b for a, b in zip(self._frame_refs, refs))):
            return
        d = self.device
        t = {k: _f32(batch[k][0], d) for k in self.FRAME_KEYS}
        cond_fix = None
        if cf_src is not None:
            cond_fix = t['poses'] if cf_src is batch['poses'] else _f32(cf_src[0, self.cfg.fix_material], d)
        fr = ra_frame(R=_ptr(t['R']), Th=_ptr(t['Th']), poses=_ptr(t['poses']), cond_fix=_ptr(cond_fix), A=_ptr(t['A']),
                      big_A=_ptr(t['big_A']), pverts=_ptr(t['pverts']), pnorm=_ptr(t['pnorm']), tverts=_ptr(t['tverts']),
                      weights=_ptr(t['weights']), n_verts=int(t['pverts'].shape[0]))
        assert t['weights'].shape[-1] == self.cfg.n_bones, 'batch.weights does not match cfg.n_bones'
        check(self.lib.ra_set_frame(self.ctx, C.byref(fr), self.stream), 'ra_set_frame')
        self._keep = [t, cond_fix]
        self._frame_key, self._frame_refs = key, refs

    def hdq_sdf(self, x: torch.Tensor, dist_th: float, smooth: bool) -> torch.Tensor:
        x = _f32(x.reshape(-1, 3), self.device)
        out = torch.empty(x.shape[0], device=self.device, dtype=torch.float32)
        check(self.lib.ra_hdq_sdf(self.ctx, _ptr(x), x.shape[0], dist_th, int(smooth), _ptr(out), self.stream), 'ra_hdq_sdf')
        return out

    def observed_sdf(self, bpts: torch.Tensor) -> torch.Tensor:
        bpts = _f32(bpts.reshape(-1, 3), self.device)
        out = torch.empty(bpts.shape[0], device=self.device, dtype=torch.float32)
        check(self.lib.ra_observed_sdf(self.ctx, _ptr(bpts), bpts.shape[0], _ptr(out), self.stream), 'ra_observed_sdf')
        return out

    def bigpose_transform(self, x: torch.Tensor, R: torch.Tensor, Th: torch.Tensor, invert=False) -> torch.Tensor:
        x = _f32(x.reshape(-1, 3), self.device)
        R, Th = _f32(R.reshape(3, 3), self.device), _f32(Th.reshape(3), self.device)
        out = torch.empty(x.shape[0], 4, 4, device=self.device, dtype=torch.float32)
        check(self.lib.ra_bigpose_transform(self.ctx, _ptr(x), x.shape[0], _ptr(R), _ptr(Th), int(invert), _ptr(out), self.stream),
              'ra_bigpose_transform')
        return out

    def forward(self, x: torch.Tensor, v, dist_th: float) -> torch.Tensor:
        x = _f32(x.reshape(-1, 3), self.device)
        v = None if v is None else _f32(v.reshape(-1, 3), self.device)
        C_ = self.lib.ra_raw_channels(self.ctx)
        raw = torch.empty(x.shape[0], C_, device=self.device, dtype=torch.float32)
        check(self.lib.ra_forward(self.ctx, _ptr(x), _ptr(v), x.shape[0], dist_th, _ptr(raw), self.stream), 'ra_forward')
        return raw

    def trace_params(self, tc, dist_th, soft, iters=None) -> ra_trace_params:
        st = self.cfg.sphere_tracing
        return ra_trace_params(iters=int(tc.iter if iters is None else iters), tan_i=st.tan_i, tan_i_multiplier=st.tan_i_multiplier,
                               relax=tc.relax, offset=tc.offset, eps=st.eps, shadow_skip_iter=st.shadow_skip_iter,
                               clay_book=int(not self.cfg.no_claybook), soft_shadow=int(soft), dist_th=dist_th)

    def sphere_trace(self, ray_o, ray_d, near, far, params: ra_trace_params, tan_i=None):
        d = self.device
        ray_o, ray_d = _f32(ray_o.reshape(-1, 3), d), _f32(ray_d.reshape(-1, 3), d)
        near, far = _f32(near.reshape(-1), d), _f32(far.reshape(-1), d)
        tan_i = None if tan_i is None else _f32(tan_i.reshape(-1), d)
        n = ray_o.shape[0]
        surf = torch.empty(n, 3, device=d)
        occ, st, ot = (torch.empty(n, device=d) for _ in range(3))
        check(self.lib.ra_sphere_trace(self.ctx, _ptr(ray_o), _ptr(ray_d), _ptr(near), _ptr(far), _ptr(tan_i), n, C.byref(params),
                                       _ptr(surf), _ptr(occ), _ptr(st), _ptr(ot), self.stream), 'ra_sphere_trace')
        return surf, occ, st, ot

    def sphere_params(self) -> ra_sphere_params:
        c = self.cfg
        return ra_sphere_params(surface=self.trace_params(c.sphere_tracing, c.dist_th, False),
                                shadow=self.trace_params(c.obj_lvis, c.obj_lvis.dist_th, not c.no_dfss),
                                shadow_near_offset=c.obj_lvis.near_offset, dist_th=c.dist_th,
                                surf_sample_range=c.surf_sample_range, n_samples=c.n_samples, relighting=int(c.relighting),
                                no_visibility=int(c.no_visibility), local_visibility=int(c.local_visibility), premultiply=1)

    def render_sphere_chunk(self, ray_o, ray_d, near, far, bbox6, probe, params, outs: dict, boxes=None, box_start=None):
        P = ray_o.shape[0]
        ro = ra_render_out(**{k: _ptr(outs.get(k)) for k in _lib.RENDER_OUT_KEYS})
        bb = _bbox6(bbox6) if bbox6 is not None else None
        ph, pw = _probe_hw(probe)
        tables = _set_box_tables(params, boxes, box_start)
        check(self.lib.ra_render_sphere_chunk(self.ctx, _ptr(ray_o), _ptr(ray_d), _ptr(near), _ptr(far), P, bb, _ptr(probe), ph, pw,
                                              C.byref(params), C.byref(ro), self.stream), 'ra_render_sphere_chunk')

    def ground_params(self) -> ra_ground_params:
        c = self.cfg
        f3 = lambda v: (C.c_float * 3)(*[float(x) for x in v])
        return ra_ground_params(normal=f3(c.ground_normal), origin=f3(c.ground_origin), albedo=f3(c.ground_albedo),
                                attach_envmap=int(c.ground_attach_envmap), env_r=float(c.env_r),
                                shading_multiplier=float(c.ground_shading_multiplier),
                                shadow=self.trace_params(c.env_lvis, c.env_lvis.dist_th, not c.no_dfss),
                                shadow_near_offset=c.env_lvis.near_offset, no_visibility=int(c.no_visibility),
                                local_visibility=int(c.local_visibility))

    def render_ground_chunk(self, ray_o, ray_d, acc, bbox6, probe, params, outs: dict, boxes=None, box_start=None):
        P = ray_o.shape[0]
        go = ra_ground_out(**{k: _ptr(outs.get(k)) for k in _lib.GROUND_OUT_KEYS})
        bb = _bbox6(bbox6)
        tables = _set_box_tables(params, boxes, box_start)
        check(self.lib.ra_render_ground_chunk(self.ctx, _ptr(ray_o), _ptr(ray_d), _ptr(acc), P, bb, _ptr(probe), probe.shape[0],
                                              probe.shape[1], C.byref(params), C.byref(go), self.stream), 'ra_render_ground_chunk')

    def debug_key_lights(self, n_lights):
        key = torch.empty(n_lights, dtype=torch.uint8, device=self.device)
        share = torch.empty(n_lights, dtype=torch.float32, device=self.device)
        check(self.lib.ra_debug_key_lights(self.ctx, _ptr(key), _ptr(share), self.stream), 'ra_debug_key_lights')
        return key.bool(), share

    def begin_render(self):
        check(self.lib.ra_begin_render(self.ctx), 'ra_begin_render')

    def k3cc_enabled(self) -> bool:
        return bool(self.lib.ra_k3cc_enabled(self.ctx))
# ... 556 lines not shown
```

Baseline: 9.203 million.

## Fuse soft-shadow trace state update into the coarse distance query kernel

Moves the soft-shadow sphere-tracing step (init and per-iteration update) into the hinted BVH coarse query kernel, so each pass advances the ray from the previous SDF before querying. The final iteration's update is fused with the lvis scatter and ray-count accumulation into one finish kernel. This removes the separate trace_init, trace_update, scatter and accumulate launches and their extra global-memory round trips per iteration. In exchange the coarse kernel gains a template variant with extra state loads and stores plus shared-memory broadcast in split mode, and the update math is refactored into a shared helper with FP contraction disabled.

```diff
diff --git a/include/relightableavatar.h b/include/relightableavatar.h
--- a/include/relightableavatar.h
+++ b/include/relightableavatar.h
@@ -42,6 +42,7 @@
     int   vis_shade_map;
     int   use_geodesic_filter;
     float key_light_share;
+    int   fused_shadow_state;
 } ra_config;
 int ra_default_config(ra_config* out);
 int ra_set_config(ra_ctx* ctx, const ra_config* cfg);
diff --git a/relightableavatar_amd/_lib.py b/relightableavatar_amd/_lib.py
--- a/relightableavatar_amd/_lib.py
+++ b/relightableavatar_amd/_lib.py
@@ -27,7 +27,8 @@
                 ('shading_albedo', C.c_float), ('albedo_multiplier', C.c_float), ('lambert_only', C.c_int),
                 ('glossy_only', C.c_int), ('tonemapping', C.c_int), ('bg_brightness', C.c_float), ('mlp_f16', C.c_int), ('query_skip', C.c_int),
                 ('k4_batch_slots', C.c_int), ('trace_precision', C.c_int), ('clip_near', C.c_float), ('clip_far', C.c_float),
-                ('only_visibility', C.c_int), ('vis_shade_map', C.c_int), ('use_geodesic_filter', C.c_int), ('key_light_share', C.c_float)]
+                ('only_visibility', C.c_int), ('vis_shade_map', C.c_int), ('use_geodesic_filter', C.c_int), ('key_light_share', C.c_float),
+                ('fused_shadow_state', C.c_int)]
 
 
 class ra_frame(C.Structure):
diff --git a/relightableavatar_amd/config.py b/relightableavatar_amd/config.py
--- a/relightableavatar_amd/config.py
+++ b/relightableavatar_amd/config.py
@@ -140,6 +140,7 @@
     c.query_skip = True
     c.trace_precision = 1
     c.key_light_share = 0.0078
+    c.fused_shadow_state = True
     c.k4_batch_slots = 0
     return c
 
diff --git a/relightableavatar_amd/csrc/ra_api.cpp b/relightableavatar_amd/csrc/ra_api.cpp
--- a/relightableavatar_amd/csrc/ra_api.cpp
+++ b/relightableavatar_amd/csrc/ra_api.cpp
@@ -136,7 +136,7 @@
 }
 
 static int hdq_pass(ra_ctx* c, const RaySet& rs, int n, float th, int smooth, float* sdf, hipStream_t s, int what = Q_OTHER,
-                    const unsigned char* key = nullptr, int n_key = 0) {
+                    const unsigned char* key = nullptr, int n_key = 0, const RayStep* step = nullptr) {
     if (n <= 0) return 0;
     int err = 0;
     int* fine_idx = c->buf<int>("fine_idx", n, &err);
@@ -155,7 +155,7 @@
         hint2 = fine_hint(c, c->fc_next - 1);
     }
     out.counters = dcnt(c);
-    launch_hdq_coarse(c->fr, rs, n, th, c->cfg.blend_radius, out, s, c->cfg.use_geodesic_filter != 0);
+    launch_hdq_coarse(c->fr, rs, n, th, c->cfg.blend_radius, out, s, c->cfg.use_geodesic_filter != 0, step);
     MlpIO io{};
     io.bpts = bpts; io.idx = fine_idx; io.count = out.fine_count; io.sdf = sdf; io.dist_th = th; io.smooth = smooth;
     io.resd_limit = c->cfg.resd_limit; io.counters = dcnt(c);
@@ -409,7 +409,11 @@
     c->cnt_zero = false;
     if (traced) {
         sh.near_ = g.near_; sh.far_ = g.far_; sh.tan_i = c->light_sharp.as<float>(); sh.light = g.ray_light;
-        launch_trace_init(sh, (int)NR, g.ray_count, shadow, s);
+        const bool fused = c->cfg.fused_shadow_state && shadow.soft_shadow && shadow.iters > 0 && c->fr.bvh_leaves > 0;
+        const bool fused_first = fused && st.pix_nn != nullptr;
+        if (!fused_first) launch_trace_init(sh, (int)NR, g.ray_count, shadow, s);
+        RayStep step{};
+        step.ts = sh; step.p = shadow; step.skip = c->cfg.query_skip ? 1 : 0;
         RaySet r2{};
         r2.mode = 2; r2.o = st.surf; r2.t = sh.t; r2.pix = g.ray_pix; r2.light = g.ray_light; r2.ldir = c->light_dir.as<float>();
         r2.n_dev = g.ray_count;
@@ -420,11 +424,18 @@
             r2.hint_valid = it > 0;
             r2.hint_src = it == 0 ? st.pix_nn : nullptr;
             r2.hint_src_index = it == 0 ? g.ray_pix : nullptr;
-            if (hdq_pass(c, r2, (int)NR, shadow.dist_th, 1, ssdf, s, Q_OTHER, keyed ? c->key_mask.as<unsigned char>() : nullptr, (int)NK)) return 1;
-            launch_trace_update(sh, ssdf, (int)NR, g.ray_count, it, shadow, s);
+            step.pass = it;
+            const bool carried = fused && (it > 0 || fused_first);
+            if (hdq_pass(c, r2, (int)NR, shadow.dist_th, 1, ssdf, s, Q_OTHER, keyed ? c->key_mask.as<unsigned char>() : nullptr, (int)NK,
+                         carried ? &step : nullptr)) return 1;
+            if (!fused) launch_trace_update(sh, ssdf, (int)NR, g.ray_count, it, shadow, s);
         }
-        launch_shadow_scatter(sh.occ, g.ray_slot, g.ray_count, (int)NR, st.lvis, s);
-        launch_accumulate(g.ray_count, &dcnt(c)->n_shadow_rays, s);
+        if (fused) {
+            launch_shadow_finish(sh, ssdf, g.ray_slot, g.ray_count, (int)NR, shadow.iters - 1, shadow, st.lvis, &dcnt(c)->n_shadow_rays, s);
+        } else {
+            launch_shadow_scatter(sh.occ, g.ray_slot, g.ray_count, (int)NR, st.lvis, s);
+            launch_accumulate(g.ray_count, &dcnt(c)->n_shadow_rays, s);
+        }
     }
     if (c->gate) { RA_HIP(hipEventRecord(c->gate->done, s)); c->gate->armed = true; }
     return 0;
diff --git a/relightableavatar_amd/csrc/ra_api_ctx.cpp b/relightableavatar_amd/csrc/ra_api_ctx.cpp
--- a/relightableavatar_amd/csrc/ra_api_ctx.cpp
+++ b/relightableavatar_amd/csrc/ra_api_ctx.cpp
@@ -87,6 +87,7 @@
     o->trace_precision = 1; o->clip_near = 0.02f; o->clip_far = 10.f;
     o->only_visibility = 0; o->vis_shade_map = 0; o->use_geodesic_filter = 1;
     o->key_light_share = 0.0078f;
+    o->fused_shadow_state = 1;
     return 0;
 }
 
diff --git a/relightableavatar_amd/csrc/ra_dfss.hpp b/relightableavatar_amd/csrc/ra_dfss.hpp
--- /dev/null
+++ b/relightableavatar_amd/csrc/ra_dfss.hpp
@@ -0,0 +1,36 @@
+#pragma once
+#include "ra_common.hpp"
+
+struct DfssRay { float t, d0, occ, ot; };
+
+__device__ __forceinline__ DfssRay dfss_init(float nr, float fr) { return DfssRay{nr, 1e9f, 1.f, fr}; }
+
+__device__ __forceinline__ bool dfss_step(DfssRay& r, float d1, float nr, float fr, float ti, float off, float rlx, int iter,
+                                          const ra_trace_params& p, float& dtn) {
+#pragma clang fp contract(off)
+    const float d0 = r.d0, t = r.t;
+    float occ = r.occ, ot = r.ot;
+    const float tan_i = p.tan_i_multiplier * ti;
+    const float tan2 = (1.f / tan_i) * 2.f;
+    const float dx1 = __fmaf_rn(d1, rlx, d1) + off;
+    if (p.clay_book && iter >= p.shadow_skip_iter) {
+        const float dx0 = __fmaf_rn(d0, rlx, d0) + off;
+        const float dx1s = dx1 * dx1;
+        const float dy = dx1s / (2.f * dx0);
+        const float dx = (sqrtf(__fmaf_rn(-dy, dy, dx1s)) - off) / (1.f + rlx);
+        const float den = fmaxf(fmaxf(t - dy, nr), p.eps);
+        const float cls = fmaxf(dx, 0.f) / den / tan2;
+        const bool msk = (cls < occ) && (dy < t) && (dx1 > 0.f) && (dx0 > 0.f) && (dx > 0.f) && (dy > 0.f) && (dy < dx0);
+        if (msk) { ot = t - dy; occ = cls; }
+    }
+    if (iter >= p.shadow_skip_iter) {
+        const float cls = fmaxf(d1, 0.f) / fmaxf(fmaxf(t, nr), p.eps) / tan2;
+        if (cls < occ) { ot = t; occ = cls; }
+    }
+    dtn = dx1;
+    float tn = t + dtn;
+    tn = fminf(tn, fr);
+    tn = fmaxf(tn, nr);
+    r.t = tn; r.d0 = d1; r.occ = occ; r.ot = ot;
+    return tn == t || occ == 0.f;
+}
diff --git a/relightableavatar_amd/csrc/ra_hdq.hip b/relightableavatar_amd/csrc/ra_hdq.hip
--- a/relightableavatar_amd/csrc/ra_hdq.hip
+++ b/relightableavatar_amd/csrc/ra_hdq.hip
@@ -1,4 +1,5 @@
 #include "ra_kernels.hpp"
+#include "ra_dfss.hpp"
 #include <type_traits>
 #include <cstdlib>
 
@@ -232,6 +233,13 @@
     d1 = nd1; i1 = ni1; d2 = nd2; i2 = ni2;
 }
 
+__device__ __forceinline__ void ray_point_light(const RaySet& rs, int i, float t, float x[3]) {
+    const int p = rs.pix[i], l = rs.light[i];
+    x[0] = rs.o[3 * p] + t * rs.ldir[3 * l];
+    x[1] = rs.o[3 * p + 1] + t * rs.ldir[3 * l + 1];
+    x[2] = rs.o[3 * p + 2] + t * rs.ldir[3 * l + 2];
+}
+
 __device__ __forceinline__ void ray_point(const RaySet& rs, int i, float x[3]) {
     if (rs.mode == 0) {
         x[0] = rs.x[3 * i]; x[1] = rs.x[3 * i + 1]; x[2] = rs.x[3 * i + 2];
@@ -241,18 +249,17 @@
         x[1] = rs.o[3 * i + 1] + t * rs.d[3 * i + 1];
         x[2] = rs.o[3 * i + 2] + t * rs.d[3 * i + 2];
     } else {
-        const float t = rs.t[i];
-        const int p = rs.pix[i], l = rs.light[i];
-        x[0] = rs.o[3 * p] + t * rs.ldir[3 * l];
-        x[1] = rs.o[3 * p + 1] + t * rs.ldir[3 * l + 1];
-        x[2] = rs.o[3 * p + 2] + t * rs.ldir[3 * l + 2];
-    }
-}
-
-template <bool BVH, int SPLIT, bool HINT = false>
+        ray_point_light(rs, i, rs.t[i], x);
+    }
+}
+
+struct NoStep {};
+
+template <bool BVH, int SPLIT, bool HINT = false, bool STATE = false>
 __global__ __launch_bounds__(SPLIT == 1 ? KNN_THREADS : 64 * SPLIT) void hdq_coarse_kernel(FrameState fr, RaySet rs, int n_launch, float th, float inv2r2,
-                                                                  HdqOut out, int dbg) {
+                                                                  HdqOut out, int dbg, std::conditional_t<STATE, RayStep, NoStep> step) {
     static_assert(SPLIT == 1 || (BVH && SPLIT >= 2 && SPLIT <= 16), "SPLIT > 1: the workgroup is SPLIT waves on the same 64 queries");
+    static_assert(!STATE || (BVH && HINT), "STATE: hinted passes on the box structure only");
     constexpr int NT = SPLIT == 1 ? KNN_THREADS : 64 * SPLIT;
     __shared__ __attribute__((aligned(16))) unsigned char smem[BVH ? 16 : VT * 16];
 #ifdef RA_COARSE_TS
@@ -266,11 +273,43 @@
     if (base >= n) return;
     if (blockIdx.x == 0 && threadIdx.x == 0 && out.counters) atomicAdd(&out.counters->n_coarse, (unsigned long long)n);
     const int i = base + (SPLIT == 1 ? threadIdx.x : (threadIdx.x & 63));
-    const bool live_q = i < n && !(rs.skip && rs.skip[i < n ? i : 0]);
+    float t_ray = 0.f;
+    bool skip_ray = false;
+    if constexpr (STATE) {
+        if (SPLIT == 1 || threadIdx.x < 64) {
+            if (i < n) {
+                const TraceState& ts = step.ts;
+                const float nr = ts.near_[i], far_i = ts.far_[i];
+                DfssRay r = dfss_init(nr, far_i);
+                bool stuck = false;
+                if (step.pass > 0) {
+                    r = DfssRay{ts.t[i], ts.d0[i], ts.occ[i], ts.ot[i]};
+                    float dtn;
+                    stuck = dfss_step(r, out.sdf[i], nr, far_i, ts.tan_i[ts.light[i]], step.p.offset, step.p.relax, step.pass - 1, step.p, dtn);
+                }
+                ts.t[i] = r.t; ts.d0[i] = r.d0; ts.occ[i] = r.occ; ts.ot[i] = r.ot;
+                ts.stuck[i] = stuck ? 1 : 0;
+                t_ray = r.t;
+                skip_ray = stuck && step.skip != 0;
+            }
+        }
+        if constexpr (SPLIT > 1) {
+            __shared__ float st_t[64];
+            __shared__ int st_skip[64];
+            if (threadIdx.x < 64) { st_t[threadIdx.x] = t_ray; st_skip[threadIdx.x] = skip_ray ? 1 : 0; }
+            __syncthreads();
+            t_ray = st_t[threadIdx.x & 63];
+            skip_ray = st_skip[threadIdx.x & 63] != 0;
+        }
+    }
+    const bool live_q = STATE ? (i < n && !skip_ray) : (i < n && !(rs.skip && rs.skip[i < n ? i : 0]));
     bool live = live_q;
     if (__syncthreads_count(live_q) == 0) return;
     float x[3] = {0.f, 0.f, 0.f};
-    if (live) ray_point(rs, i, x);
+    if (live) {
+        if constexpr (STATE) ray_point_light(rs, i, t_ray, x);
+        else ray_point(rs, i, x);
+    }
     const float xt[3] = {x[0] - fr.Th[0], x[1] - fr.Th[1], x[2] - fr.Th[2]};
     float p[3];
 #pragma unroll
@@ -579,7 +618,7 @@
 }
 
 void launch_hdq_coarse(const FrameState& fr, const RaySet& rs, int n, float th, float blend_radius, const HdqOut& out,
-                       hipStream_t s, bool geodesic) {
+                       hipStream_t s, bool geodesic, const RayStep* step) {
     if (n <= 0) return;
     const float inv2r2 = 1.f / (2.f * blend_radius * blend_radius);
     const dim3 grid((n + KNN_THREADS - 1) / KNN_THREADS);
@@ -596,24 +635,33 @@
     dbg |= (launch_no++ & 63) << 8;
 #endif
     const bool hint = (rs.nn_hint != nullptr && rs.hint_valid != 0) || rs.hint_src != nullptr;
+    if (step) {
+        const int d = dbg;
+        const int groups = (n + 63) / 64;
+        if (n > split_max) hipLaunchKernelGGL((hdq_coarse_kernel<true, 1, true, true>), grid, dim3(KNN_THREADS), 0, s, fr, rs, n, th, inv2r2, out, d, *step);
+        else if (n <= split_max / 8) hipLaunchKernelGGL((hdq_coarse_kernel<true, 16, true, true>), dim3(groups), dim3(1024), 0, s, fr, rs, n, th, inv2r2, out, d, *step);
+        else if (n <= split_max / 2) hipLaunchKernelGGL((hdq_coarse_kernel<true, 8, true, true>), dim3(groups), dim3(512), 0, s, fr, rs, n, th, inv2r2, out, d, *step);
+        else hipLaunchKernelGGL((hdq_coarse_kernel<true, 4, true, true>), dim3(groups), dim3(256), 0, s, fr, rs, n, th, inv2r2, out, d, *step);
+        return;
+    }
     for (int pass = probe ? 0 : 1; pass < 2; ++pass) {
         const int d = pass == 0 ? probe : dbg;
         if (fr.bvh_leaves > 0 && n <= split_max)
         {
             const int groups = (n + 63) / 64;
             if (hint) {
-                if (n <= split_max / 8) hipLaunchKernelGGL((hdq_coarse_kernel<true, 16, true>), dim3(groups), dim3(1024), 0, s, fr, rs, n, th, inv2r2, out, d);
-                else if (n <= split_max / 2) hipLaunchKernelGGL((hdq_coarse_kernel<true, 8, true>), dim3(groups), dim3(512), 0, s, fr, rs, n, th, inv2r2, out, d);
-                else hipLaunchKernelGGL((hdq_coarse_kernel<true, 4, true>), dim3(groups), dim3(256), 0, s, fr, rs, n, th, inv2r2, out, d);
+                if (n <= split_max / 8) hipLaunchKernelGGL((hdq_coarse_kernel<true, 16, true>), dim3(groups), dim3(1024), 0, s, fr, rs, n, th, inv2r2, out, d, NoStep{});
+                else if (n <= split_max / 2) hipLaunchKernelGGL((hdq_coarse_kernel<true, 8, true>), dim3(groups), dim3(512), 0, s, fr, rs, n, th, inv2r2, out, d, NoStep{});
+                else hipLaunchKernelGGL((hdq_coarse_kernel<true, 4, true>), dim3(groups), dim3(256), 0, s, fr, rs, n, th, inv2r2, out, d, NoStep{});
             } else {
-                if (n <= split_max / 8) hipLaunchKernelGGL((hdq_coarse_kernel<true, 16>), dim3(groups), dim3(1024), 0, s, fr, rs, n, th, inv2r2, out, d);
-                else if (n <= split_max / 2) hipLaunchKernelGGL((hdq_coarse_kernel<true, 8>), dim3(groups), dim3(512), 0, s, fr, rs, n, th, inv2r2, out, d);
-                else hipLaunchKernelGGL((hdq_coarse_kernel<true, 4>), dim3(groups), dim3(256), 0, s, fr, rs, n, th, inv2r2, out, d);
-            }
-        }
-        else if (fr.bvh_leaves > 0 && hint) hipLaunchKernelGGL((hdq_coarse_kernel<true, 1, true>), grid, dim3(KNN_THREADS), 0, s, fr, rs, n, th, inv2r2, out, d);
-        else if (fr.bvh_leaves > 0) hipLaunchKernelGGL((hdq_coarse_kernel<true, 1>), grid, dim3(KNN_THREADS), 0, s, fr, rs, n, th, inv2r2, out, d);
-        else hipLaunchKernelGGL((hdq_coarse_kernel<false, 1>), grid, dim3(KNN_THREADS), 0, s, fr, rs, n, th, inv2r2, out, d);
+                if (n <= split_max / 8) hipLaunchKernelGGL((hdq_coarse_kernel<true, 16>), dim3(groups), dim3(1024), 0, s, fr, rs, n, th, inv2r2, out, d, NoStep{});
+                else if (n <= split_max / 2) hipLaunchKernelGGL((hdq_coarse_kernel<true, 8>), dim3(groups), dim3(512), 0, s, fr, rs, n, th, inv2r2, out, d, NoStep{});
+                else hipLaunchKernelGGL((hdq_coarse_kernel<true, 4>), dim3(groups), dim3(256), 0, s, fr, rs, n, th, inv2r2, out, d, NoStep{});
+            }
+        }
+        else if (fr.bvh_leaves > 0 && hint) hipLaunchKernelGGL((hdq_coarse_kernel<true, 1, true>), grid, dim3(KNN_THREADS), 0, s, fr, rs, n, th, inv2r2, out, d, NoStep{});
+        else if (fr.bvh_leaves > 0) hipLaunchKernelGGL((hdq_coarse_kernel<true, 1>), grid, dim3(KNN_THREADS), 0, s, fr, rs, n, th, inv2r2, out, d, NoStep{});
+        else hipLaunchKernelGGL((hdq_coarse_kernel<false, 1>), grid, dim3(KNN_THREADS), 0, s, fr, rs, n, th, inv2r2, out, d, NoStep{});
         if (pass == 0) hipMemsetAsync(out.fine_count, 0, sizeof(int), s);
     }
 }
diff --git a/relightableavatar_amd/csrc/ra_kernels.hpp b/relightableavatar_amd/csrc/ra_kernels.hpp
--- a/relightableavatar_amd/csrc/ra_kernels.hpp
+++ b/relightableavatar_amd/csrc/ra_kernels.hpp
@@ -48,9 +48,6 @@
 void launch_bvh_build(const float4* pverts4, int n_verts, int* order, float* leaves, float4* sbox, int n_leaves, int n_supers, hipStream_t s);
 int bvh_leaf_count(int n_verts);
 int bvh_super_count(int n_leaves);
-void launch_hdq_coarse(const FrameState& fr, const RaySet& rs, int n, float th, float blend_radius, const HdqOut& out,
-                       hipStream_t s, bool geodesic = true);
-
 struct TraceState {
     float *t, *d0, *dt, *st, *ot, *cd, *occ, *off, *rlx;
     const float *near_, *far_;
@@ -58,6 +55,14 @@
     const int* light;
     unsigned char* stuck;
 };
+struct RayStep {
+    TraceState ts;
+    ra_trace_params p;
+    int pass;
+    int skip;
+};
+void launch_hdq_coarse(const FrameState& fr, const RaySet& rs, int n, float th, float blend_radius, const HdqOut& out,
+                       hipStream_t s, bool geodesic = true, const RayStep* step = nullptr);
 void launch_trace_init(const TraceState& ts, int n, const int* n_dev, const ra_trace_params& p, hipStream_t s);
 
 void launch_trace_update(const TraceState& ts, const float* sdf, int n, const int* n_dev, int iter,
@@ -118,6 +123,8 @@
 int launch_sort_hits(const float* surf, const float* acc, int P, const float* bbox_min, unsigned* keys_in, unsigned* keys_out,
                      int* vals_in, int* hit_idx_out, void* temp, size_t temp_bytes, hipStream_t s);
 void launch_shadow_scatter(const float* occ, const int* ray_slot, const int* ray_count, int max_rays, float* lvis, hipStream_t s);
+void launch_shadow_finish(const TraceState& ts, const float* sdf, const int* ray_slot, const int* ray_count, int max_rays, int iter,
+                          const ra_trace_params& p, float* lvis, unsigned long long* n_rays_total, hipStream_t s);
 
 struct ShadeIn {
     const float* ray_o;
diff --git a/relightableavatar_amd/csrc/ra_trace.hip b/relightableavatar_amd/csrc/ra_trace.hip
--- a/relightableavatar_amd/csrc/ra_trace.hip
+++ b/relightableavatar_amd/csrc/ra_trace.hip
@@ -1,4 +1,5 @@
 #include "ra_kernels.hpp"
+#include "ra_dfss.hpp"
 #include "ra_shade_dev.hpp"
 #include <hipcub/hipcub.hpp>
 
@@ -18,13 +19,14 @@
     const int i = blockIdx.x * TPB + threadIdx.x;
     if (i >= live_count(n_dev, n_launch)) return;
     const float nr = ts.near_[i], fr = ts.far_[i];
-    ts.t[i] = nr;
-    ts.d0[i] = 1e9f;
-    ts.occ[i] = 1.f;
+    const DfssRay r = dfss_init(nr, fr);
+    ts.t[i] = r.t;
+    ts.d0[i] = r.d0;
+    ts.occ[i] = r.occ;
     if (ts.stuck) ts.stuck[i] = 0;
     if (ts.dt) ts.dt[i] = 1e9f;
     if (ts.st) ts.st[i] = fr;
-    if (ts.ot) ts.ot[i] = fr;
+    if (ts.ot) ts.ot[i] = r.ot;
     if (ts.cd) ts.cd[i] = 1e9f;
     if (ts.off) ts.off[i] = offset;
     if (ts.rlx) ts.rlx[i] = relax;
@@ -36,35 +38,34 @@
     const int i = blockIdx.x * TPB + threadIdx.x;
     if (i >= live_count(n_dev, n_launch)) return;
     const float d1 = sdf[i];
+    const float nr = ts.near_[i], fr = ts.far_[i];
+    if constexpr (SOFT) {
+        DfssRay r{ts.t[i], ts.d0[i], ts.occ[i], ts.ot ? ts.ot[i] : 0.f};
+        const float ti = ts.tan_i ? (ts.light ? ts.tan_i[ts.light[i]] : ts.tan_i[i]) : p.tan_i;
+        float dtn;
+        const bool stuck = dfss_step(r, d1, nr, fr, ti, ts.off ? ts.off[i] : p.offset, ts.rlx ? ts.rlx[i] : p.relax, iter, p, dtn);
+        if (ts.dt) ts.dt[i] = dtn;
+        ts.t[i] = r.t;
+        if (ts.stuck) ts.stuck[i] = stuck ? 1 : 0;
+        ts.d0[i] = r.d0;
+        ts.occ[i] = r.occ;
+        if (ts.ot) ts.ot[i] = r.ot;
+        return;
+    }
     const float d0 = ts.d0[i];
     float t = ts.t[i];
     const float t_prev = t;
     float occ = ts.occ[i];
-    const float nr = ts.near_[i], fr = ts.far_[i];
-    float tan_i = p.tan_i;
-    if (SOFT) {
-        const float ti = ts.tan_i ? (ts.light ? ts.tan_i[ts.light[i]] : ts.tan_i[i]) : p.tan_i;
-        tan_i = p.tan_i_multiplier * ti;
-    }
+    const float tan_i = p.tan_i;
     const float tan2 = (1.f / tan_i) * 2.f;
     float off = ts.off ? ts.off[i] : p.offset;
     float rlx = ts.rlx ? ts.rlx[i] : p.relax;
     float ot = ts.ot ? ts.ot[i] : 0.f;
-    if (SOFT && p.clay_book && iter >= p.shadow_skip_iter) {
-        const float dx0 = d0 + rlx * d0 + off;
-        const float dx1 = d1 + rlx * d1 + off;
-        const float dy = (dx1 * dx1) / (2.f * dx0);
-        const float dx = (sqrtf(dx1 * dx1 - dy * dy) - off) / (1.f + rlx);
-        const float den = fmaxf(fmaxf(t - dy, nr), p.eps);
-        const float cls = fmaxf(dx, 0.f) / den / tan2;
-        const bool msk = (cls < occ) && (dy < t) && (dx1 > 0.f) && (dx0 > 0.f) && (dx > 0.f) && (dy > 0.f) && (dy < dx0);
-        if (msk) { ot = t - dy; occ = cls; }
-    }
     if (iter >= p.shadow_skip_iter) {
         const float cls = fmaxf(d1, 0.f) / fmaxf(fmaxf(t, nr), p.eps) / tan2;
         if (cls < occ) { ot = t; occ = cls; }
     }
-    if (!SOFT) {
+    {
         const float d1u = fabsf(d1), d0u = fabsf(d0);
         float st = ts.st[i], cd = ts.cd[i];
         const float dt = ts.dt[i];
@@ -87,7 +88,7 @@
     t = fmaxf(t, nr);
     if (ts.dt) ts.dt[i] = dtn;
     ts.t[i] = t;
-    if (ts.stuck) ts.stuck[i] = (t == t_prev || (SOFT && occ == 0.f)) ? 1 : 0;
+    if (ts.stuck) ts.stuck[i] = (t == t_prev) ? 1 : 0;
     ts.d0[i] = d1;
     ts.occ[i] = occ;
     if (ts.ot) ts.ot[i] = ot;
@@ -425,6 +426,18 @@
     const int i = blockIdx.x * TPB + threadIdx.x;
     if (i >= min(*ray_count, max_rays)) return;
     lvis[ray_slot[i]] = occ[i];
+}
+
+__global__ void shadow_finish_kernel(TraceState ts, const float* __restrict__ sdf, const int* __restrict__ ray_slot,
+                                     const int* __restrict__ ray_count, int max_rays, int iter, ra_trace_params p, float* __restrict__ lvis,
+                                     unsigned long long* __restrict__ n_rays_total) {
+    const int i = blockIdx.x * TPB + threadIdx.x;
+    if (i == 0) atomicAdd(n_rays_total, (unsigned long long)*ray_count);
+    if (i >= min(*ray_count, max_rays)) return;
+    DfssRay r{ts.t[i], ts.d0[i], ts.occ[i], ts.ot[i]};
+    float dtn;
+    dfss_step(r, sdf[i], ts.near_[i], ts.far_[i], ts.tan_i[ts.light[i]], p.offset, p.relax, iter, p, dtn);
+    lvis[ray_slot[i]] = r.occ;
 }
 
 __global__ __launch_bounds__(TPB) void key_lights_kernel(const float* __restrict__ probes, int n, int ph, int pw, const float* __restrict__ ldir,
@@ -1276,6 +1289,12 @@
     hipLaunchKernelGGL(scatter_rows_kernel, grid_for(n * C), dim3(TPB), 0, s, src, src_idx, dst_idx, n, C, dst);
 }
 
+void launch_shadow_finish(const TraceState& ts, const float* sdf, const int* ray_slot, const int* ray_count, int max_rays, int iter,
+                          const ra_trace_params& p, float* lvis, unsigned long long* n_rays_total, hipStream_t s) {
+    hipLaunchKernelGGL(shadow_finish_kernel, grid_for(max_rays > 0 ? max_rays : 1), dim3(TPB), 0, s, ts, sdf, ray_slot, ray_count, max_rays, iter, p, lvis,
+                       n_rays_total);
+}
+
 void launch_accumulate(const int* count, unsigned long long* dst, hipStream_t s) {
     hipLaunchKernelGGL(accumulate_kernel, dim3(1), dim3(1), 0, s, count, dst);
 }
diff --git a/relightableavatar_amd/engine.py b/relightableavatar_amd/engine.py
--- a/relightableavatar_amd/engine.py
+++ b/relightableavatar_amd/engine.py
@@ -402,7 +402,8 @@
                       only_visibility=int(bool(cfg.get('only_visibility', False))),
                       vis_shade_map=2 if cfg.get('vis_ldot_map', False) else (1 if cfg.get('vis_lvis_map', False) else 0),
                       use_geodesic_filter=int(bool(cfg.get('use_geodesic_filter', True))),
-                      key_light_share=float(cfg.get('key_light_share', 0.0078)))
+                      key_light_share=float(cfg.get('key_light_share', 0.0078)),
+                      fused_shadow_state=int(cfg.get('fused_shadow_state', True)))
         assert cfg.mlp_dtype in ('f16', 'bf16')
         check(self.lib.ra_set_config(self.ctx, C.byref(c)), 'ra_set_config')
         self._frame_key = None
```

Measured after the change: 9.146 million. No clear change (-0.6%).
